# GDMCF/GDMCF

Measured on AMD Instinct MI355X. Metric: training users/sec, higher is better.
Workload: dtype f32; 1 GPU; yelp-shape synthetic rows, batch=400/GPU, dims=[1000], T=5, noise_scale=0.01, linear-var, mean_type=x0, reweight, AdamW lr=1e-5 (BASELINE configs[1]); n_items=34395, global_batch=400, parallelism=dp1, batch_rows=device CSR rows (CsrBatch)

## Files before the change

### gdmcf_amd/_lib.py

```python
import ctypes
import os
import re
from ctypes import c_char_p, c_double, c_float, c_int, c_int64, c_size_t, c_uint64, c_void_p

_HERE = os.path.dirname(os.path.abspath(__file__))
LIB_PATH = os.path.join(_HERE, "csrc", "libgdmcf_hip.so")
HEADER_PATH = os.path.normpath(os.path.join(_HERE, "..", "include", "gdmcf_hip.h"))

P = c_void_p
_CTYPES = {"int": c_int, "int64_t": c_int64, "uint64_t": c_uint64, "size_t": c_size_t, "float": c_float, "double": c_double}


def _uncomment(text):
    return re.sub(r"/\*.*?\*/", " ", text, flags=re.S)


def _code(text):
    return re.sub(r'^[ \t]*(#.*|extern\s+"C"\s*\{|\})[ \t]*$', "", _uncomment(text), flags=re.M)


def _ctype(ctype, where):
    words = re.sub(r"\bconst\b", " ", ctype).replace("*", " * ").split()
    if "*" in words:
        return c_char_p if words == ["char", "*"] else c_void_p
    if " ".join(words) not in _CTYPES:
        raise ImportError(f"gdmcf_hip.h: no ctypes type for '{' '.join(ctype.split())}' in the declaration of {where}")
    return _CTYPES[" ".join(words)]


def _declarator(decl, where):
    m = re.fullmatch(r"\s*(.*[\s*])(\w+)\s*", decl, flags=re.S)
    if not m:
        raise ImportError(f"gdmcf_hip.h: cannot read '{decl.strip()}' in the declaration of {where}")
    return m.groups()


def parse_functions(text):
    code = _code(text)
    out = {}
    for ret, name, params in re.findall(r"([\w\s*]+?)\b(gdmcf_\w+)\s*\(([^()]*)\)\s*;", code):
        params = [] if params.strip() in ("", "void") else params.split(",")
        out[name] = (_ctype(ret, name), [_ctype(_declarator(p, name)[0], name) for p in params])
    mentioned = re.findall(r"(gdmcf_\w+)\s*\(", code)
    if len(mentioned) != len(out):
        raise ImportError(f"gdmcf_hip.h: {len(mentioned)} gdmcf_*( but {len(out)} declarations read; unreadable: "
                          f"{sorted(set(mentioned) - set(out)) or 'none, a name is repeated'}")
    return out


def parse_constants(text):
    text = _uncomment(text)
    out = {n: int(v) for n, v in re.findall(r"^\s*#\s*define\s+(GDMCF_\w+)\s+\(?\s*(-?\d+)\s*\)?\s*$", text, flags=re.M)}
    for body in re.findall(r"\benum\s*\{([^}]*)\}", text):
        for member in filter(str.strip, body.split(",")):
            m = re.fullmatch(r"\s*(\w+)\s*=\s*(-?\d+)\s*", member)
            if not m:
                raise ImportError(f"gdmcf_hip.h: enum member '{member.strip()}' is not `NAME = integer`")
            out[m.group(1)] = int(m.group(2))
    return out


def parse_structs(text):
    out = {}
    for name, body in re.findall(r"\btypedef\s+struct\s+(\w+)\s*\{([^}]*)\}\s*\1\s*;", _code(text)):
        out[name] = []
        for line in filter(str.strip, body.split(";")):
            first, *more = line.split(",")
            ctype, member = _declarator(first, "struct " + name)
            if more and "*" in line:
                raise ImportError(f"gdmcf_hip.h: struct {name}: '{line.strip()}' must declare one pointer member per line")
            out[name] += [(m.strip(), _ctype(ctype, "struct " + name)) for m in [member] + more]
    return out


try:
    with open(HEADER_PATH) as _f:
        _HEADER = _f.read()
except OSError as e:
    raise ImportError(f"{HEADER_PATH} is missing: gdmcf_amd._lib derives its ctypes binding from the C header, which sits "
                      "beside the package in the source tree.") from e
_SIGNATURES = parse_functions(_HEADER)
EXPORTED_SYMBOLS = tuple(_SIGNATURES)
CONSTANTS = parse_constants(_HEADER)
GDMCF_OK, E_SHAPE, E_ARG, E_UNSUPPORTED, E_HIP, E_WORKSPACE, N_TABLES = (
    CONSTANTS["GDMCF_" + n] for n in ("OK", "E_SHAPE", "E_ARG", "E_UNSUPPORTED", "E_HIP", "E_WORKSPACE", "N_TABLES"))
TABLE_NAMES = (
    "betas", "alphas_cumprod", "alphas_cumprod_prev", "alphas_cumprod_next", "sqrt_alphas_cumprod",
    "sqrt_one_minus_alphas_cumprod", "log_one_minus_alphas_cumprod", "sqrt_recip_alphas_cumprod",
    "sqrt_recipm1_alphas_cumprod", "posterior_variance", "posterior_log_variance_clipped",
    "posterior_mean_coef1", "posterior_mean_coef2",
)


class GdDwAdamw(ctypes.Structure):
    _fields_ = parse_structs(_HEADER)["GdDwAdamw"]


_lib = None


def load():
    global _lib
    if _lib is not None:
        return _lib
    if not os.path.exists(LIB_PATH):
        raise ImportError(
            f"{LIB_PATH} is missing: build it with `python -m gdmcf_amd.build` (hipcc, gfx950). "
            "gdmcf_amd has no CPU / PyTorch fallback.")
    lib = ctypes.CDLL(LIB_PATH)
    for name, (res, args) in _SIGNATURES.items():
        fn = getattr(lib, name)
        fn.restype = res
        fn.argtypes = args
    if lib.gdmcf_version() != 1:
        raise ImportError("libgdmcf_hip.so ABI version mismatch; rebuild with `python -m gdmcf_amd.build --force`")
    _lib = lib
    return lib


_EXC = {E_SHAPE: AssertionError, E_ARG: ValueError, E_UNSUPPORTED: NotImplementedError, E_HIP: RuntimeError,
        E_WORKSPACE: RuntimeError}


def check(rc):
    if rc != GDMCF_OK:
        msg = load().gdmcf_last_error().decode(errors="replace")
        raise _EXC.get(rc, RuntimeError)(msg or f"gdmcf error {rc}")


def ptr(t):
    return None if t is None else t.data_ptr()


def require_gpu(t, what):
    if not t.is_cuda:
        raise RuntimeError(f"gdmcf_amd: {what} must live on the MI355X (got device '{t.device}'); "
                           "the HIP path has no CPU fallback")


def shadow_info(data_ptr):
    p16 = ctypes.c_void_p()
    rows, cols, ld = ctypes.c_int64(), ctypes.c_int64(), ctypes.c_int64()
    if not load().gdmcf_bf16_shadow_info(data_ptr, ctypes.byref(p16), ctypes.byref(rows), ctypes.byref(cols), ctypes.byref(ld)):
        return None
    return int(p16.value), int(rows.value), int(cols.value), int(ld.value)


def stream_ptr():
    import torch
    return torch.cuda.current_stream().cuda_stream


def philox_randn(shape, device, seed, offset, stream_id=4, out=None):
    import torch
    rows, cols = int(shape[0]), int(shape[1])
    if out is None:
        out = torch.empty(rows, cols, dtype=torch.float32, device=device)
    require_gpu(out, "philox_randn output")
    check(load().gdmcf_randn_f32(out.data_ptr(), out.stride(0), rows, cols, int(stream_id), int(seed) & (2 ** 64 - 1),
                                 int(offset) & (2 ** 64 - 1), stream_ptr()))
    return out


def schedule_tables(kind, noise_scale, noise_min, noise_max, steps, beta_fixed=True):
    import numpy as np
    out = np.zeros((N_TABLES, steps), dtype=np.float64)
    rc = load().gdmcf_schedule_build(kind, float(noise_scale), float(noise_min), float(noise_max), int(steps),
                                     int(bool(beta_fixed)), out.ctypes.data_as(c_void_p))
    check(rc)
    return out


class Bf16Shadow:

    def __init__(self, t, sync=True):
        import weakref

        import torch
        require_gpu(t, "bf16 shadow source")
        if t.dim() != 2 or t.dtype != torch.float32 or t.stride(1) != 1:
            raise RuntimeError("gdmcf_amd: a bf16 shadow needs a 2-D float32 tensor with unit column stride")
        self.rows, self.cols = t.shape
        self.ptr = t.data_ptr()
        self.ld = t.stride(0)
        self.buf = torch.zeros((self.rows + 63) // 64 * 64, (self.cols + 63) // 64 * 64, dtype=torch.bfloat16,
                               device=t.device)
        self._lib = load()
        self._fin = weakref.finalize(self, self._lib.gdmcf_bf16_shadow_clear, self.ptr)
        self.register()
        if sync:
            self.sync()

    def register(self):
        check(self._lib.gdmcf_bf16_shadow_set(self.ptr, self.buf.data_ptr(), self.rows, self.cols, self.buf.stride(0)))

    def unregister(self):
        self._lib.gdmcf_bf16_shadow_clear(self.ptr)

    def sync(self):
        check(self._lib.gdmcf_bf16_shadow_sync(self.ptr, self.ld, stream_ptr()))

    def close(self):
        self._fin()
```

### gdmcf_amd/build.py

```python
import concurrent.futures
import hashlib
import os
import re
import subprocess
import sys

CSRC = os.path.join(os.path.dirname(os.path.abspath(__file__)), "csrc")
SOURCES = ["capi.hip", "dp_exchange.hip", "gemm_f32.hip", "gemm_bf16.hip", "gemm_split.hip", "gemm_small.hip", "gemm_dr.hip", "gemm_dr_tn.hip", "gemm_dr_fat.hip", "gemm_dr_kn.hip", "prep_input.hip", "noise.hip", "loss_tail.hip", "adamw.hip", "rows.hip", "reduce.hip", "linear.hip", "topk.hip", "spmm_csr.hip", "rank_metrics.hip", "spmm_bundle.hip", "score_topk.hip", "score_rank.hip", "bpr.hip", "cat.hip", "gather_fwd.hip", "ntxent.hip", "latent_step.hip", "cand_scores.hip", "rank.hip"]
HEADERS = ["common.h", "draws.h", "rank_order.h", "score_product.h", "spmm.h", "gemm_dr.h", "gemm_epilogue.h", os.path.join("..", "..", "include", "gdmcf_hip.h")]
LIB = os.path.join(CSRC, "libgdmcf_hip.so")
ASM_LINT = ("gemm_dr_tn.hip", "gemm_split.hip")
STORE_LINT = ("gemm_f32.hip", "gemm_bf16.hip", "gemm_dr_fat.hip", "gemm_dr_kn.hip", "score_topk.hip", "score_rank.hip", "latent_step.hip", "bpr.hip")
NO_SPILL = ("gemm_f32.hip", "gemm_bf16.hip", "gemm_split.hip", "gemm_dr_tn.hip", "score_topk.hip", "score_rank.hip", "cat.hip", "gather_fwd.hip", "ntxent.hip", "latent_step.hip", "cand_scores.hip", "bpr.hip")
FLAGS = ["--offload-arch=gfx950", "-O3", "-std=c++17", "-fPIC", "-Wall", "-Wno-unused-function"]


def _hipcc():
    for c in (os.environ.get("HIPCC"), "/opt/rocm/bin/hipcc", "hipcc"):
        if c and (os.path.isabs(c) and os.path.exists(c) or not os.path.isabs(c)):
            return c
    raise RuntimeError("hipcc not found")


def _digest():
    h = hashlib.sha256()
    for f in SOURCES + HEADERS:
        with open(os.path.join(CSRC, f), "rb") as fh:
            h.update(fh.read())
    h.update(" ".join(FLAGS).encode())
    return h.hexdigest()


_REG = re.compile(r"\bv(\d+)\b|\bv\[(\d+):(\d+)\]")


def _regs(text):
    out = set()
    for m in _REG.finditer(text):
        if m.group(1) is not None:
            out.add(int(m.group(1)))
        else:
            out.update(range(int(m.group(2)), int(m.group(3)) + 1))
    return out


_SREG = re.compile(r"\bs(\d+)\b|\bs\[(\d+):(\d+)\]")


def _sregs(text):
    out = set()
    for m in _SREG.finditer(text):
        if m.group(1) is not None:
            out.add(int(m.group(1)))
        else:
            out.update(range(int(m.group(2)), int(m.group(3)) + 1))
    return out


def lint_ring_registers(asm_text, kernel_prefix="dr_tn_kernel"):
    bad, seen = [], 0
    for m in re.finditer(r"^(\S*%s\S*):[^\n]*\n(.*?)\n\s*s_endpgm" % kernel_prefix, asm_text, flags=re.S | re.M):
        name, body = m.group(1), m.group(2)
        seen += 1
        lines = [ln.split(";")[0].strip() for ln in body.splitlines()]
        lines = [ln for ln in lines if ln and not ln.endswith(":") and not ln.startswith(".")]
        ring = set()
        for ln in lines:
            if ln.startswith("buffer_load_dwordx4"):
                ring |= _regs(ln.split(",")[0])
        if not ring:
            bad.append(f"{name}: no asm ring loads found (lint out of date?)")
            continue
        first = next(i for i, ln in enumerate(lines) if ln.startswith("buffer_load_dwordx4"))
        drains = [i for i, ln in enumerate(lines) if ln.startswith("s_waitcnt") and "vmcnt(0)" in ln]
        last = drains[-1] if drains and drains[-1] > first else len(lines)
        for ln in lines[first:last]:
            mnem, _, ops = ln.partition(" ")
            parts = [o.strip() for o in ops.split(",")]
            if mnem.startswith("buffer_load_dwordx4"):
                if _regs(",".join(parts[1:])) & ring:
                    bad.append(f"{name}: ring register used as an address: {ln}")
            elif mnem.startswith("v_mfma"):
                if (_regs(parts[0]) | _regs(parts[3] if len(parts) > 3 else "")) & ring:
                    bad.append(f"{name}: MFMA accumulator inside the operand ring: {ln}")
            elif mnem.startswith(("v_mov", "v_pk_mov", "v_accvgpr", "scratch_", "v_swap")):
                if _regs(ops) & ring:
                    bad.append(f"{name}: copy or spill of a ring register: {ln}")
    if not seen:
        bad.append(f"no function named *{kernel_prefix}* in the assembly (lint out of date?)")
    return bad


_COPY = ("v_mov", "v_pk_mov", "v_accvgpr", "scratch_", "v_swap")
_VMEM = ("buffer_", "global_", "flat_", "scratch_")


def lint_vmcnt(asm_text, only=None):
    bad, nk = [], 0
    for m in re.finditer(r"^(_Z\S+):[^\n]*\n(.*?)\n\s*s_endpgm", asm_text, flags=re.S | re.M):
        name, body = m.group(1), m.group(2)
        if only and only not in name:
            continue
        ins, in_asm = [], False
        for ln in body.splitlines():
            t = ln.strip()
            if t.startswith(";;#ASMSTART"):
                in_asm = True
                continue
            if t.startswith(";;#ASMEND"):
                in_asm = False
                continue
            c = t.split(";")[0].strip()
            if not c or (c.startswith(".") and not c.endswith(":")):
                continue
            ins.append((c, in_asm))
        if not any(a and "load_dword" in c.split()[0] for c, a in ins):
            continue
        nk += 1
        leaders, labels = {0}, {}
        for k, (c, a) in enumerate(ins):
            if c.endswith(":"):
                labels[c[:-1]] = k
                leaders.add(k)
            elif c.startswith(("s_cbranch", "s_branch")):
                leaders.add(k + 1)
        starts = sorted(x for x in leaders if x < len(ins))
        blocks = [(st, starts[i + 1] if i + 1 < len(starts) else len(ins)) for i, st in enumerate(starts)]
        blk_of = {st: i for i, (st, en) in enumerate(blocks)}
        succ = []
        for bi, (st, en) in enumerate(blocks):
            mn, _, ops = ins[en - 1][0].partition(" ")
            nxt = []
            if mn.startswith(("s_cbranch", "s_branch")) and labels.get(ops.strip()) is not None:
                nxt.append(blk_of[labels[ops.strip()]])
            if not mn.startswith("s_branch") and bi + 1 < len(blocks):
                nxt.append(bi + 1)
            succ.append(nxt)
        found = {}

        def transfer(bi, st_in, report):
            st = dict(st_in)
            fresh = {}
            for k in range(*blocks[bi]):
                ln, a = ins[k]
                if ln.endswith(":"):
                    continue
                mnem, _, ops = ln.partition(" ")
                parts = [o.strip() for o in ops.split(",")]
                if a and mnem.startswith(_VMEM):
                    hot = _sregs(ops) & fresh.keys()
                    if hot and report:
                        found.setdefault(f"s{min(hot)} written by a VALU instruction < 5 wait states before this asm load reads it: {ln}", k)
                step = int(ops) + 1 if mnem == "s_nop" and ops.strip().isdigit() else 1
                fresh = {r: w - step for r, w in fresh.items() if w - step > 0}
                if mnem.startswith("v_") and parts and re.fullmatch(r"s\d+|s\[\d+:\d+\]", parts[0]):
                    for r in _sregs(parts[0]):
                        fresh[r] = 5
                if mnem == "s_waitcnt":
                    mm = re.search(r"vmcnt\((\d+)\)", ops)
                    if mm:
                        st = {r: rk for r, rk in st.items() if rk < int(mm.group(1))}
                    continue
                asm_load = a and "load_dword" in mnem
                touched = _regs(",".join(parts[1:]) if asm_load else ops) & st.keys()
                if touched and report:
                    what = "used as an address" if asm_load else ("copied / spilled" if mnem.startswith(_COPY) else "used")
                    found.setdefault(f"register v{min(touched)} {what} before a counted wait covers its load: {ln}", k)
                if mnem.startswith(_VMEM):
                    st = {r: min(rk + 1, 64) for r, rk in st.items()}
                    if asm_load:
                        for r in _regs(parts[0]):
                            st[r] = 0
            return st

        state = [None] * len(blocks)
        state[0] = {}
        work = [0]
        while work:
            bi = work.pop()
            out = transfer(bi, state[bi], False)
            for sj in succ[bi]:
                if state[sj] is None:
                    state[sj] = dict(out)
                    work.append(sj)
                else:
                    changed = False
                    for r, rk in out.items():
                        if state[sj].get(r, 65) > rk:
                            state[sj][r] = rk
                            changed = True
                    if changed:
                        work.append(sj)
        for bi in range(len(blocks)):
            if state[bi] is not None:
                transfer(bi, state[bi], True)
        bad += [f"{name}: {msg}" for msg, k in sorted(found.items(), key=lambda kv: kv[1])]
    if not nk:
        bad.append("no kernel with inline-asm loads in the assembly (lint out of date?)")
    return bad


def lint_store_data(asm_text):
    bad = []
    for m in re.finditer(r"^(_Z\S+):[^\n]*\n(.*?)\n\s*s_endpgm", asm_text, flags=re.S | re.M):
        name, body = m.group(1), m.group(2)
        lines = [ln.split(";")[0].strip() for ln in body.splitlines()]
        lines = [ln for ln in lines if ln and not ln.startswith(".") and not ln.endswith(":")]
        for k, ln in enumerate(lines):
            mnem, _, ops = ln.partition(" ")
            if not re.match(r"(buffer|global|flat|scratch)_store_dwordx[34]$", mnem):
                continue
            parts = [o.strip() for o in ops.split(",")]
            data = _regs(parts[1] if mnem.startswith(("global", "flat", "scratch")) else parts[0])
            left = 2
            for nxt in lines[k + 1:k + 8]:
                nm, _, nops = nxt.partition(" ")
                if nm == "s_nop":
                    left -= int(nops.strip() or 0) + 1
                else:
                    nparts = [o.strip() for o in nops.split(",")]
                    if nm.startswith("v_") and nparts and _regs(nparts[0]) & data and left > 0:
                        bad.append(f"{name}: data register of `{ln}` rewritten {2 - left} wait state(s) later by `{nxt}`")
                        break
                    left -= 1
                if left <= 0:
                    break
    return bad


def lint_fat_dma(asm_text, kernel="dr_fat_kernel"):
    bad, n_dma = [], 0
    for m in re.finditer(r"^(_Z\S*%s\S*):[^\n]*\n(.*?)\n\s*s_endpgm" % kernel, asm_text, flags=re.S | re.M):
        name, body = m.group(1), m.group(2)
        lines = [ln.split(";")[0].strip() for ln in body.splitlines()]
        lines = [ln for ln in lines if ln and (not ln.startswith(".") or ln.endswith(":"))]
        if not any(ln.startswith("buffer_load_dwordx4") and ln.endswith(" lds") for ln in lines):
            continue
        n_dma += 1
        pending = None
        for ln in lines:
            if ln.startswith("buffer_load_dwordx4") and ln.endswith(" lds"):
                pending = ln
            elif ln.startswith("s_waitcnt") and re.search(r"vmcnt\(0\)", ln):
                pending = None
            elif ln.startswith("ds_read_b128") and pending:
                bad.append(f"{name}: `{ln}` follows `{pending}` with no s_waitcnt vmcnt(0) in between")
                break
        loops, label, blk = 0, None, []
        for ln in lines + ["end:"]:
            if not ln.endswith(":"):
                blk.append(ln)
                continue
            if label and any(i.startswith("v_mfma") for i in blk) and any(
                    i.startswith(("s_cbranch", "s_branch")) and i.split()[-1] == label for i in blk):
                loops += 1
                moved = [i for i in blk if i.startswith(("scratch_", "v_accvgpr", "v_mov"))]
                if moved:
                    bad.append(f"{name}: {len(moved)} spill / move instruction(s) in the k loop, e.g. `{moved[0]}`")
            label, blk = ln[:-1], []
        if not loops:
            bad.append(f"{name}: no k loop found (lint out of date?)")
    if not n_dma:
        bad.append(f"no *{kernel}* with `buffer_load_dwordx4 ... lds` in the assembly (lint out of date?)")
    return bad


def build(force=False, verbose=True):
    stamp = os.path.join(CSRC, ".build_stamp")
    dig = _digest()
    if not force and os.path.exists(LIB) and os.path.exists(stamp) and open(stamp).read() == dig:
        return LIB
    hipcc = _hipcc()
    objs = []

    def compile_one(src):
        obj = os.path.join(CSRC, src.replace(".hip", ".o"))
        cmd = [hipcc] + FLAGS + ["-c", os.path.join(CSRC, src), "-o", obj]
        guarded = src in NO_SPILL
        if guarded:
            cmd.append("-Rpass-analysis=kernel-resource-usage")
        r = subprocess.run(cmd, capture_output=True, text=True)
        if r.returncode != 0:
            raise RuntimeError(f"hipcc failed for {src}:\n{r.stderr}")
        err = r.stderr
        if guarded:
            name, bad = None, []
            for line in err.splitlines():
                if "Function Name:" in line:
                    name = line.split("Function Name:")[1].split()[0]
                elif "VGPRs Spill:" in line and int(line.split("VGPRs Spill:")[1].split()[0]) > 0:
                    bad.append(name)
            if bad:
                raise RuntimeError(f"{src}: register spills in {len(bad)} kernel(s) with uncounted asm loads, e.g. {bad[0]}")
            err = err if ("warning:" in err or "error:" in err) else ""
        if verbose and err.strip():
            print(err, file=sys.stderr)
        if src in ASM_LINT or src in STORE_LINT:
            asm = os.path.join(CSRC, src.replace(".hip", ".lint.s"))
            r2 = subprocess.run([hipcc] + FLAGS + ["-S", "--cuda-device-only", os.path.join(CSRC, src), "-o", asm],
                                capture_output=True, text=True)
            if r2.returncode != 0:
                raise RuntimeError(f"hipcc -S failed for {src}:\n{r2.stderr}")
            text = open(asm).read()
            os.remove(asm)
            bad = lint_store_data(text)
            if src in ASM_LINT:
                bad += lint_vmcnt(text)
            if src == "gemm_dr_tn.hip":
                bad += lint_ring_registers(text)
            if src == "gemm_dr_fat.hip":
                bad += lint_fat_dma(text)
            if bad:
                raise RuntimeError(f"{src}: ISA lint failed (lint_store_data / lint_vmcnt / lint_ring_registers / lint_fat_dma):\n  " + "\n  ".join(bad[:12]))
        return obj

    with concurrent.futures.ThreadPoolExecutor(max_workers=min(8, len(SOURCES))) as ex:
        objs = list(ex.map(compile_one, SOURCES))
    cmd = [hipcc, "--offload-arch=gfx950", "-shared", "-fPIC", "-o", LIB] + objs
    r = subprocess.run(cmd, capture_output=True, text=True)
    if r.returncode != 0:
        raise RuntimeError(f"link failed:\n{r.stderr}")
    with open(stamp, "w") as fh:
        fh.write(dig)
    if verbose:
        print(f"built {LIB}")
    return LIB


if __name__ == "__main__":
    build(force="--force" in sys.argv)
```

### gdmcf_amd/csrc/gemm_dr_kn.hip

```cpp
#include "gemm_dr.h"

namespace {

#ifndef GD_KN_EVERY
#define GD_KN_EVERY 4
#endif
template <int NL>
__global__ __launch_bounds__(256, 1) void dr_kn_kernel(const DrArgs d) {
    constexpr int TMB = 5;
    const GdGemm& g = d.g;
    const int lane = threadIdx.x & 63;
    const int wave = __builtin_amdgcn_readfirstlane(threadIdx.x >> 6);
    const int r = lane & 15, q = lane >> 4;
    const int nblk = gridDim.x, per = nblk >> 3;
    const int wl = ((nblk & 7) == 0 ? ((int)(blockIdx.x & 7) * per + (int)(blockIdx.x >> 3)) : (int)blockIdx.x) * 4 + wave;
    const int n_waves = nblk * 4;
    const int ntiles = d.tiles_m * d.tiles_n;
    const int CPS = d.ksp;
    const int total_chunks = (g.K + 15) >> 4;
    const int ntasks = ntiles * g.splits;
    const __amdgpu_buffer_rsrc_t srdA = __builtin_amdgcn_make_buffer_rsrc(const_cast<float*>(g.A), 0, (int)(((int64_t)(g.M - 1) * g.lda + g.K) * 4), 0x00020000);
    const __amdgpu_buffer_rsrc_t srdB = __builtin_amdgcn_make_buffer_rsrc(const_cast<float*>(g.B), 0, (int)(((int64_t)(g.K - 1) * g.ldb + g.N) * 4), 0x00020000);
    const uint32_t ldb16 = (uint32_t)g.ldb * 64u;
    for (int task = wl; task < ntasks; task += n_waves) {
        const int split = task / ntiles, tile = task - split * ntiles;
        const int tm = tile % d.tiles_m, tn = tile / d.tiles_m;
        const int m0 = tm * (16 * TMB), n0 = tn * (64 * NL);
        const int c_lo = split * CPS;
        uint32_t offA[TMB], offB[4][NL];
#pragma unroll
        for (int a = 0; a < TMB; ++a) offA[a] = (uint32_t)(((int64_t)min(m0 + 16 * a + r, g.M - 1) * g.lda + 4 * q) * 4);
#pragma unroll
        for (int s = 0; s < 4; ++s)
#pragma unroll
            for (int l = 0; l < NL; ++l) {
                const int n = n0 + 64 * l + 4 * r;
                offB[s][l] = n < g.N ? (uint32_t)(((int64_t)(4 * q + s) * g.ldb + n) * 4) : 0x80000000u;
            }
        f32x4 acc[TMB][NL][4];
#pragma unroll
        for (int a = 0; a < TMB; ++a)
#pragma unroll
            for (int l = 0; l < NL; ++l)
#pragma unroll
                for (int e = 0; e < 4; ++e) acc[a][l][e] = f32x4{0.f, 0.f, 0.f, 0.f};
        f32x4 xa[2][TMB], xb[2][4][NL];
        {
            const uint32_t ka = (uint32_t)c_lo * 64u, kb = (uint32_t)c_lo * ldb16;
#pragma unroll
            for (int a = 0; a < TMB; ++a) xa[0][a] = __builtin_bit_cast(f32x4, __builtin_amdgcn_raw_buffer_load_b128(srdA, offA[a], ka, 0));
#pragma unroll
            for (int s = 0; s < 4; ++s)
#pragma unroll
                for (int l = 0; l < NL; ++l)
                    xb[0][s][l] = __builtin_bit_cast(f32x4, __builtin_amdgcn_raw_buffer_load_b128(srdB, offB[s][l], kb, 0));
        }
#define GD_KN_CHUNK(PAR, c)                                                                                            \
        {                                                                                                              \
            const bool more = (c) + 1 < c_lo + CPS && (c) + 1 < total_chunks;                                          \
            const uint32_t ka = more ? (uint32_t)((c) + 1) * 64u : 0x80000000u;                                        \
            const uint32_t kb = more ? (uint32_t)((c) + 1) * ldb16 : 0x80000000u;                                      \
            if ((c) * 16 + 15 >= g.K) {  \
                _Pragma("unroll") for (int e = 0; e < 4; ++e) {                                                        \
                    const bool keep = (c) * 16 + 4 * q + e < g.K;                                                      \
                    _Pragma("unroll") for (int a = 0; a < TMB; ++a) xa[PAR][a][e] = keep ? xa[PAR][a][e] : 0.f;        \
                }                                                                                                      \
            }                                                                                                          \
                    \
            _Pragma("unroll") for (int a = 0; a < TMB; ++a) asm volatile("" : "+v"(xa[PAR][a]));                       \
            _Pragma("unroll") for (int s = 0; s < 4; ++s)                                                              \
                _Pragma("unroll") for (int l = 0; l < NL; ++l) asm volatile("" : "+v"(xb[PAR][s][l]));                 \
            __builtin_amdgcn_sched_barrier(0);                                                                         \
            _Pragma("unroll") for (int s = 0; s < 4; ++s) {                                                            \
                _Pragma("unroll") for (int n = 0; n < TMB * NL * 4; ++n) {                                             \
                    const int a = n / (NL * 4), l = (n / 4) % NL, e = n % 4;                                           \
                    acc[a][l][e] = __builtin_amdgcn_mfma_f32_16x16x4f32(xa[PAR][a][s], xb[PAR][s][l][e], acc[a][l][e], 0, 0, 0); \
                    const int idx = s * (TMB * NL * 4) + n;                                                            \
                    if (idx % GD_KN_EVERY == 2 && idx / GD_KN_EVERY < TMB + 4 * NL) {                                  \
                        const int ld = idx / GD_KN_EVERY;                                                              \
                        __builtin_amdgcn_sched_barrier(0);                                                             \
                        if (ld < TMB)                                                                                  \
                            xa[(PAR) ^ 1][ld] = __builtin_bit_cast(f32x4, __builtin_amdgcn_raw_buffer_load_b128(srdA, offA[ld], ka, 0)); \
                        else                                                                                           \
                            xb[(PAR) ^ 1][(ld - TMB) / NL][(ld - TMB) % NL] = __builtin_bit_cast(                      \
                                f32x4, __builtin_amdgcn_raw_buffer_load_b128(srdB, offB[(ld - TMB) / NL][(ld - TMB) % NL], kb, 0)); \
                        __builtin_amdgcn_sched_barrier(0);                                                             \
                    }                                                                                                  \
                }                                                                                                      \
                __builtin_amdgcn_sched_barrier(0);                                                                     \
            }                                                                                                          \
        }
        for (int c = c_lo; c < c_lo + CPS && c < total_chunks; c += 2) {
            GD_KN_CHUNK(0, c);
            GD_KN_CHUNK(1, c + 1);
        }
#undef GD_KN_CHUNK
        float* __restrict__ slab = g.C + (int64_t)split * g.slab_stride;
#pragma unroll
        for (int a = 0; a < TMB; ++a)
#pragma unroll
            for (int t = 0; t < 4; ++t) {
                const int m = m0 + 16 * a + 4 * q + t;
                if (m >= g.M) continue;
#pragma unroll
                for (int l = 0; l < NL; ++l) {
                    const int n = n0 + 64 * l + 4 * r;
                    const f32x4 v = {acc[a][l][0][t], acc[a][l][1][t], acc[a][l][2][t], acc[a][l][3][t]};
                    if (n + 3 < g.ldc) {
                        *reinterpret_cast<f32x4*>(slab + (int64_t)m * g.ldc + n) = v;
                    } else {
                        for (int e = 0; e < 4; ++e)
                            if (n + e < g.N) slab[(int64_t)m * g.ldc + n + e] = v[e];
                    }
                }
            }
    }
}

}

int gd_dr_kn_splits(int M, int N, int K) {
    if (!dr_routes().kn || M < 16 || N < 64 || K < 4096) return 0;
    const long tiles = (long)gd_cdiv(M, 80) * gd_cdiv(N, 128);
    if ((long)gd_cdiv(M, 80) * 80 * 100 > (long)M * 112) return 0;
    if ((long)gd_cdiv(N, 128) * 128 * 100 > (long)N * 112) return 0;
    const long slots = 4L * dr_cu_count();
    if (tiles > slots) return 0;
    int splits = (int)(slots / tiles);
    const int total_chunks = gd_cdiv(K, 16);
    if (splits > total_chunks / 8) splits = total_chunks / 8;
    if (splits < 2 || splits > 64) return splits > 64 ? 64 : 0;
    return splits;
}

int gd_dr_kn_launch(GdGemm& g, hipStream_t s) {
    if (!dr_routes().kn) return GD_DR_NOT_TAKEN;
    const int splits = gd_dr_kn_splits(g.M, g.N, g.K);
    const size_t need = (size_t)splits * g.M * g.ldc * sizeof(float);
    const bool ok = splits > 0 && g.ldc >= g.N && (g.ldc & 3) == 0 && g.ws_cap >= need && g.slab_stride >= (int64_t)g.M * g.ldc &&
                (int64_t)g.M * g.lda * 4 < ((int64_t)1 << 31) && (int64_t)g.K * g.ldb * 4 < ((int64_t)1 << 31) && g.lda >= g.K && g.ldb >= g.N &&
                (reinterpret_cast<uintptr_t>(g.B) & 15) == 0 && (g.ldb & 3) == 0 && (reinterpret_cast<uintptr_t>(g.C) & 15) == 0;
    if (!ok) return GD_DR_NOT_TAKEN;
    DrArgs d = {};
    const int n_cu = dr_cu_count();
    const int total_chunks = gd_cdiv(g.K, 16);
    const int cps = (gd_cdiv(total_chunks, splits) + 1) & ~1;
    d.tiles_m = gd_cdiv(g.M, 80);
    d.tiles_n = gd_cdiv(g.N, 128);
    d.ksp = cps;
    g.splits = gd_cdiv(total_chunks, cps);
    g.kchunk = cps * 16;
    g.tiles_m = d.tiles_m;
    g.tiles_n = d.tiles_n;
    d.g = g;
    {
        GdProfScope prof(g.prof_tag, 2.0 * g.M * g.N * g.K, s);
        hipLaunchKernelGGL((dr_kn_kernel<2>), dim3(n_cu), dim3(256), 0, s, d);
    }
    t_gd_last_gemm = 5;
    return gd_launch_status("gemm_dr_kn");
}
```

### gdmcf_amd/csrc/linear.hip

```cpp
#include <stdlib.h>

#include "common.h"

int gd_splitk_reduce(const float* slabs, int64_t slab_stride, int splits, int64_t ld_slab, int M, int N, int mode,
                     const float* bias, const float* rowscale, const float* aact, int64_t ldact, int act, float* out,
                     int64_t ldo, hipStream_t s);
int gd_colsum(const float* dZ, int64_t ld, const float* rs, int M, int N, float* db, hipStream_t s);
int gd_rowpart_reduce(const float* rowpart, int ld, int M, int nt, float* rowsum, hipStream_t s);

namespace {

static const int TARGET_WGS = getenv("GDMCF_TARGET_WGS") ? atoi(getenv("GDMCF_TARGET_WGS")) : 760;

thread_local int t_gemm_prec = GDMCF_GEMM_F32;

int pick_class(int M, int N, bool fused, int prec) {
    if (prec == GDMCF_GEMM_BF16 && M > 128) {
        const long pad = (long)gd_cdiv(M, 208) * 208;
        const long tiles = (pad / 208) * gd_cdiv(N, 256);
        const long rounds = (tiles + 255) / 256;
        if (pad * 10 <= (long)M * 11 && pad / 208 <= 2 && (!fused || tiles * 100 >= rounds * 256 * 85)) return 3;
    }
    if (prec == GDMCF_GEMM_F32X3 && M > 128 && N >= 128) {
        const long pad = (long)gd_cdiv(M, 208) * 208;
        if (pad * 10 <= (long)M * 11) return 4;
    }
    return gd_pick_shape_class(M, N);
}

int pick_class_dw(int M, int N, int prec, bool fused_adamw = false) {
    static const int forced = getenv("GDMCF_BF16_DW_CLASS") ? atoi(getenv("GDMCF_BF16_DW_CLASS")) : -1;
    if (prec == GDMCF_GEMM_BF16 && forced >= 0) return forced;
    if (prec == GDMCF_GEMM_BF16 && fused_adamw && M >= 160 && N >= 256) return 0;
    if (prec == GDMCF_GEMM_BF16 && M >= 416 && N >= 512) {
        const long tiles = (long)gd_cdiv(M, 208) * gd_cdiv(N, 256);
        const long rounds = (tiles + 255) / 256;
        if (tiles * 100 >= rounds * 256 * 85) return 3;
    }
    return gd_pick_shape_class(M, N);
}

void attach_result_shadow(GdGemm& g) {
    GdShadow c;
    if (g.bf16 == 1 && gd_shadow_lookup(g.C, &c) && c.rows == g.M && c.cols >= g.N) {
        g.C16 = c.p16;
        g.ldc16 = c.ld16;
    }
}

void attach_shadows(GdGemm& g, int layA, int layB) {
    if (g.bf16 != 1) return;
    GdShadow a, b;
    if (!gd_shadow_lookup(g.A, &a) || !gd_shadow_lookup(g.B, &b)) return;
    const bool okA = layA == GD_LAY_KC ? (a.rows == g.M && a.cols == g.K) : (a.rows == g.K && a.cols == g.M);
    const bool okB = layB == GD_LAY_KC ? (b.rows == g.N && b.cols == g.K) : (b.rows == g.K && b.cols == g.N);
    if (!okA || !okB) return;
    g.A16 = a.p16; g.lda16 = a.ld16;
    g.B16 = b.p16; g.ldb16 = b.ld16;
}

int pick_splits(int M, int N, int K, int cls, int prec) {
    const int bk = prec == GDMCF_GEMM_BF16 ? 64 : 32;
    const int tiles = gd_cdiv(M, gd_gemm_tile_m(cls)) * gd_cdiv(N, gd_gemm_tile_n(cls));
    int s = (cls >= 3 ? 256 : TARGET_WGS) / tiles;
    const int max_by_k = K / (8 * bk);
    if (s > max_by_k) s = max_by_k;
    if (s < 1) s = 1;
    if (s > 64) s = 64;
    return s;
}

inline int64_t round4(int64_t x) { return (x + 3) & ~(int64_t)3; }

float* bias_col_request(int a_scale_col, int64_t lda, const float* rowscale, int K, float* db) {
    static const int on = getenv("GDMCF_BIAS_COL") ? atoi(getenv("GDMCF_BIAS_COL")) : 1;
    if (!on || !a_scale_col || db == nullptr || t_gemm_prec != GDMCF_GEMM_F32 || lda <= K) return nullptr;
    return db;
}

int dw_adamw_setup(const GdDwAdamw& e, GdGemm& g, int& cls) {
    GD_CHECK_SHAPE(e.M > 0 && e.N > 0 && e.K > 0 && e.lddz >= e.N && e.lda >= e.K && e.ldw >= e.K, "linear_bwd_weight_adamw: bad shape");
    GD_CHECK_ARG(e.W && e.exp_avg && e.exp_avg_sq && e.step >= 1, "linear_bwd_weight_adamw: optimizer state missing");
    const int M = e.M, N = e.N, K = e.K;
    cls = pick_class_dw(N, K, t_gemm_prec, true);
    g = GdGemm{};
    g.bf16 = t_gemm_prec;
    g.A = e.dZ; g.lda = e.lddz; g.B = e.A; g.ldb = e.lda; g.M = N; g.N = K; g.K = M; g.splits = 1;
    g.m_fastest = gd_cdiv(N, gd_gemm_tile_m(cls)) <= gd_cdiv(K, gd_gemm_tile_n(cls));
    g.C = e.W; g.ldc = e.ldw; g.aux = e.exp_avg; g.aux2 = e.exp_avg_sq; g.prof_tag = 5;
    g.adam = gd_adam_hyper(e.lr, e.beta1, e.beta2, e.eps, e.weight_decay, e.step, e.grad_scale);
    g.adam_dev = t_gd_step_state ? &t_gd_step_state->hyper : nullptr;
    attach_result_shadow(g);
    attach_shadows(g, GD_LAY_MC, GD_LAY_MC);
    g.out2 = bias_col_request(e.a_scale_col, e.lda, e.rowscale, K, e.db);
    return GDMCF_OK;
}

int dw_adamw_finish(const GdDwAdamw& e, bool asked, const GdGemm& g, hipStream_t s) {
    if (asked && g.out2 == nullptr) return GDMCF_OK;
    if (e.db) return gd_colsum(e.dZ, e.lddz, e.rowscale, e.M, e.N, e.db, s);
    return GDMCF_OK;
}

}

extern "C" {

int gdmcf_gemm_precision(int mode) {
    const int prev = t_gemm_prec;
    if (mode == GDMCF_GEMM_F32 || mode == GDMCF_GEMM_BF16 || mode == GDMCF_GEMM_F32X3) t_gemm_prec = mode;
    return prev;
}

size_t gdmcf_linear_ws_bytes(int M, int N, int K) {
    if (M <= 0 || N <= 0 || K <= 0) return 0;
    size_t need = 0;
    for (int prec = GDMCF_GEMM_F32; prec <= GDMCF_GEMM_F32X3; ++prec) {
        const int cf = pick_class(M, N, false, prec), cb = pick_class(M, K, false, prec);
        size_t f = (size_t)pick_splits(M, N, K, cf, prec) * M * round4(N);
        if (prec == GDMCF_GEMM_F32) {
            const size_t fk = (size_t)gd_dr_kn_splits(M, N, K) * M * round4(N);
            f = f > fk ? f : fk;
            const size_t ff = (size_t)gd_dr_fat_slab_plan(M, N, K, nullptr, nullptr) * M * round4(N);
            f = f > ff ? f : ff;
        }
        size_t b = (size_t)pick_splits(M, K, N, cb, prec) * M * round4(K);
        if (prec == GDMCF_GEMM_F32) {
            const size_t bk = (size_t)gd_dr_kn_splits(M, K, N) * M * round4(K);
            b = b > bk ? b : bk;
        }
        need = need > f ? need : f;
        need = need > b ? need : b;
    }
    return need * sizeof(float) + 256;
}

int gdmcf_debug_fat_slab_plan(int M, int N, int K, int* nb, int* splits, int* cps) {
    int nb_ = 0, cps_ = 0;
    const int sp = (t_gemm_prec == GDMCF_GEMM_F32 && M > 0 && N > 0 && K > 0) ? gd_dr_fat_slab_plan(M, N, K, &nb_, &cps_) : 0;
    if (nb) *nb = nb_;
    if (splits) *splits = sp;
    if (cps) *cps = cps_;
    return sp > 0;
}

int gdmcf_loss_tiles(int N) { return gd_cdiv(N, 16); }

int gdmcf_linear_fwd_f32(const float* A, int64_t lda, const float* W, int64_t ldw, const float* bias, int act, int M,
                         int N, int K, float* C, int64_t ldc, void* ws, size_t ws_bytes, void* stream) {
    GD_CHECK_SHAPE(M > 0 && N > 0 && K > 0 && lda >= K && ldw >= K && ldc >= N, "linear_fwd: bad shape");
    GD_CHECK_ARG(act == 0 || act == 1, "linear_fwd: bad activation");
    hipStream_t s = (hipStream_t)stream;
    const int cls = pick_class(M, N, false, t_gemm_prec);
    const int splits = pick_splits(M, N, K, cls, t_gemm_prec);
    GdGemm g = {};
    g.bf16 = t_gemm_prec;
    g.A = A; g.lda = lda; g.B = W; g.ldb = ldw; g.M = M; g.N = N; g.K = K;
    g.m_fastest = gd_cdiv(M, gd_gemm_tile_m(cls)) <= gd_cdiv(N, gd_gemm_tile_n(cls));
    g.bias = bias; g.act = act; g.prof_tag = 1;
    if (splits == 1) {
        g.splits = 1; g.C = C; g.ldc = ldc;
        attach_result_shadow(g);
        attach_shadows(g, GD_LAY_KC, GD_LAY_KC);
        return gd_gemm_launch(GD_LAY_KC, GD_LAY_KC, GD_EPI_BIAS_ACT, cls, g, s);
    }
    const int64_t lds_ = round4(N);
    const size_t need = (size_t)splits * M * lds_ * sizeof(float);
    if (ws == nullptr || ws_bytes < need) {
        gdmcf_set_error("linear_fwd: workspace %zu < %zu bytes", ws_bytes, need);
        return GDMCF_E_WORKSPACE;
    }
    g.splits = splits; g.C = (float*)ws; g.ldc = lds_; g.slab_stride = (int64_t)M * lds_;
    g.ws_cap = ws_bytes;
    attach_shadows(g, GD_LAY_KC, GD_LAY_KC);
    int rc = gd_gemm_launch(GD_LAY_KC, GD_LAY_KC, GD_EPI_SLAB, cls, g, s);
    if (rc) return rc;
    const int real_splits = gd_cdiv(K, g.kchunk);
    return gd_splitk_reduce((const float*)ws, g.slab_stride, real_splits, lds_, M, N, 0, bias, nullptr, nullptr, 0,
                            act, C, ldc, s);
}

int gdmcf_linear_fwd_wt_f32(const float* A, int64_t lda, const float* Wt, int64_t ldwt, const float* bias, int act, int M, int N,
                            int K, float* C, int64_t ldc, void* ws, size_t ws_bytes, void* stream) {
    GD_CHECK_SHAPE(M > 0 && N > 0 && K > 0 && lda >= K && ldwt >= N && ldc >= N, "linear_fwd_wt: bad shape");
    GD_CHECK_ARG(act == 0 || act == 1, "linear_fwd_wt: bad activation");
    if (t_gemm_prec != GDMCF_GEMM_F32) {
        gdmcf_set_error("linear_fwd_wt: float32 GEMM mode only (the bf16 / f32x3 modes keep the weight in its own orientation)");
        return GDMCF_E_UNSUPPORTED;
    }
    hipStream_t s = (hipStream_t)stream;
    const int cls = pick_class(M, N, false, t_gemm_prec);
    const int splits = pick_splits(M, N, K, cls, t_gemm_prec);
    const int64_t lds_ = round4(N);
    const size_t need = (size_t)splits * M * lds_ * sizeof(float);
    if (ws == nullptr || ws_bytes < need) {
        gdmcf_set_error("linear_fwd_wt: workspace %zu < %zu bytes", ws_bytes, need);
        return GDMCF_E_WORKSPACE;
    }
    GdGemm g = {};
    g.A = A; g.lda = lda; g.B = Wt; g.ldb = ldwt; g.M = M; g.N = N; g.K = K;
    g.m_fastest = gd_cdiv(M, gd_gemm_tile_m(cls)) <= gd_cdiv(N, gd_gemm_tile_n(cls));
    g.splits = splits; g.C = (float*)ws; g.ldc = lds_; g.slab_stride = (int64_t)M * lds_; g.prof_tag = 1;
    g.ws_cap = ws_bytes;
    int rc = gd_gemm_launch(GD_LAY_KC, GD_LAY_MC, GD_EPI_SLAB, cls, g, s);
    if (rc) return rc;
    const int real_splits = gd_cdiv(K, g.kchunk);
    return gd_splitk_reduce((const float*)ws, g.slab_stride, real_splits, lds_, M, N, 0, bias, nullptr, nullptr, 0, act, C, ldc, s);
}

int gdmcf_linear_loss_fwd_f32(const float* A, int64_t lda, const float* W, int64_t ldw, const float* bias,
                              const float* target, int64_t ldt, const float* alpha, int M, int N, int K, float* out,
                              int64_t ldo, float* diff, int64_t ldd, float* rowpart, float* rowsum, void* stream) {
    GD_CHECK_SHAPE(M > 0 && N > 0 && K > 0 && lda >= K && ldw >= K && ldt >= N && ldd >= N, "linear_loss_fwd: bad shape");
    GD_CHECK_SHAPE(out == nullptr || ldo >= N, "linear_loss_fwd: ldo < N");
    hipStream_t s = (hipStream_t)stream;
    const int cls = pick_class(M, N, true, t_gemm_prec);
    GdGemm g = {};
    g.bf16 = t_gemm_prec;
    g.A = A; g.lda = lda; g.B = W; g.ldb = ldw; g.M = M; g.N = N; g.K = K; g.splits = 1;
    g.m_fastest = gd_cdiv(M, gd_gemm_tile_m(cls)) <= gd_cdiv(N, gd_gemm_tile_n(cls));
    g.bias = bias; g.aux = target; g.ldaux = ldt; g.r0 = alpha; g.out2 = out; g.ldout2 = ldo;
    g.prof_tag = 2;
    g.C = diff; g.ldc = ldd; g.rowpart = rowpart; g.ld_rowpart = gdmcf_loss_tiles(N);
    attach_result_shadow(g);
    attach_shadows(g, GD_LAY_KC, GD_LAY_KC);
    int rc = gd_gemm_launch(GD_LAY_KC, GD_LAY_KC, GD_EPI_LOSS, cls, g, s);
    if (rc) return rc;
    return gd_rowpart_reduce(rowpart, g.ld_rowpart, M, g.tiles_n, rowsum, s);
}

int gdmcf_linear_loss_fwd_bits_f32(const float* A, int64_t lda, const float* W, int64_t ldw, const float* bias,
                                   const uint32_t* target_bits, int64_t ldbits, const float* alpha, int M, int N, int K,
                                   float* out, int64_t ldo, float* diff, int64_t ldd, float* rowpart, float* rowsum,
                                   void* stream) {
    GD_CHECK_SHAPE(M > 0 && N > 0 && K > 0 && lda >= K && ldw >= K && ldd >= N, "linear_loss_fwd_bits: bad shape");
    GD_CHECK_SHAPE(out == nullptr || ldo >= N, "linear_loss_fwd_bits: ldo < N");
    GD_CHECK_ARG(target_bits && ldbits >= (N + 31) / 32, "linear_loss_fwd_bits: target bitmap missing / ldbits < ceil(N/32)");
    hipStream_t s = (hipStream_t)stream;
    const int cls = pick_class(M, N, true, t_gemm_prec);
    GdGemm g = {};
    g.bf16 = t_gemm_prec;
    g.A = A; g.lda = lda; g.B = W; g.ldb = ldw; g.M = M; g.N = N; g.K = K; g.splits = 1;
    g.m_fastest = gd_cdiv(M, gd_gemm_tile_m(cls)) <= gd_cdiv(N, gd_gemm_tile_n(cls));
    g.bias = bias; g.aux = nullptr; g.ldaux = 0; g.aux_bits = target_bits; g.ldbits = ldbits; g.r0 = alpha; g.out2 = out;
    g.ldout2 = ldo; g.prof_tag = 2;
    g.C = diff; g.ldc = ldd; g.rowpart = rowpart; g.ld_rowpart = gdmcf_loss_tiles(N);
    attach_result_shadow(g);
    attach_shadows(g, GD_LAY_KC, GD_LAY_KC);
    int rc = gd_gemm_launch(GD_LAY_KC, GD_LAY_KC, GD_EPI_LOSS, cls, g, s);
    if (rc) return rc;
    return gd_rowpart_reduce(rowpart, g.ld_rowpart, M, g.tiles_n, rowsum, s);
}

int gdmcf_linear_posterior_fwd_f32(const float* A, int64_t lda, const float* W, int64_t ldw, const float* bias,
                                   const float* x_t, int64_t ldxt, const float* c1, const float* c2, const float* r1,
                                   const float* r2, const float* sigma, const float* z, int64_t ldz, int M, int N,
                                   int K, float* x_next, int64_t ldxn, float* pred_out, int64_t ldp, void* stream) {
    GD_CHECK_SHAPE(M > 0 && N > 0 && K > 0 && lda >= K && ldw >= K && ldxt >= N && ldxn >= N, "linear_posterior_fwd: bad shape");
    GD_CHECK_ARG(c1 && c2, "linear_posterior_fwd: c1/c2 missing");
    GD_CHECK_ARG((r1 == nullptr) == (r2 == nullptr), "linear_posterior_fwd: r1/r2 must both be set or both NULL");
    GD_CHECK_ARG(z == nullptr || (sigma != nullptr && ldz >= N), "linear_posterior_fwd: sigma missing");
    hipStream_t s = (hipStream_t)stream;
    const int cls = pick_class(M, N, true, t_gemm_prec);
    GdGemm g = {};
    g.bf16 = t_gemm_prec;
    g.A = A; g.lda = lda; g.B = W; g.ldb = ldw; g.M = M; g.N = N; g.K = K; g.splits = 1;
    g.m_fastest = gd_cdiv(M, gd_gemm_tile_m(cls)) <= gd_cdiv(N, gd_gemm_tile_n(cls));
    g.bias = bias; g.aux = x_t; g.ldaux = ldxt; g.aux2 = z; g.ldaux2 = ldz;
    g.r0 = c1; g.r1 = c2; g.r2 = r1; g.r3 = r2; g.r4 = sigma;
    g.out2 = pred_out; g.ldout2 = ldp; g.C = x_next; g.ldc = ldxn; g.prof_tag = 3;
    attach_result_shadow(g);
    attach_shadows(g, GD_LAY_KC, GD_LAY_KC);
    return gd_gemm_launch(GD_LAY_KC, GD_LAY_KC, GD_EPI_POST, cls, g, s);
}

int gdmcf_linear_bwd_input_f32(const float* dZ, int64_t lddz, const float* W, int64_t ldw, const float* rowscale,
                               const float* Aact, int64_t ldact, int act, int M, int N, int K, float* dA,
                               int64_t ldda, void* ws, size_t ws_bytes, void* stream) {
    GD_CHECK_SHAPE(M > 0 && N > 0 && K > 0 && lddz >= N && ldw >= K && ldda >= K, "linear_bwd_input: bad shape");
    GD_CHECK_ARG(act == 0 || (act == 1 && Aact && ldact >= K), "linear_bwd_input: activation output missing");
    hipStream_t s = (hipStream_t)stream;
    const int cls = pick_class(M, K, false, t_gemm_prec);
    const int splits = pick_splits(M, K, N, cls, t_gemm_prec);
    const int64_t lds_ = round4(K);
    const size_t need = (size_t)splits * M * lds_ * sizeof(float);
    if (ws == nullptr || ws_bytes < need) {
        gdmcf_set_error("linear_bwd_input: workspace %zu < %zu bytes", ws_bytes, need);
        return GDMCF_E_WORKSPACE;
    }
    GdGemm g = {};
    g.bf16 = t_gemm_prec;
    g.A = dZ; g.lda = lddz; g.B = W; g.ldb = ldw; g.M = M; g.N = K; g.K = N;
    g.m_fastest = gd_cdiv(M, gd_gemm_tile_m(cls)) <= gd_cdiv(K, gd_gemm_tile_n(cls));
    g.splits = splits; g.C = (float*)ws; g.ldc = lds_; g.slab_stride = (int64_t)M * lds_; g.prof_tag = 4;
    g.ws_cap = ws_bytes;
    attach_shadows(g, GD_LAY_KC, GD_LAY_MC);
    int rc = gd_gemm_launch(GD_LAY_KC, GD_LAY_MC, GD_EPI_SLAB, cls, g, s);
    if (rc) return rc;
    const int real_splits = gd_cdiv(N, g.kchunk);
    return gd_splitk_reduce((const float*)ws, g.slab_stride, real_splits, lds_, M, K, 1, nullptr, rowscale, Aact,
                            ldact, act, dA, ldda, s);
}

int gdmcf_linear_bwd_weight_f32(const float* dZ, int64_t lddz, const float* A, int64_t lda, const float* rowscale,
                                int a_scale_col, int M, int N, int K, float* dW, int64_t lddw, float* db, int accumulate,
                                void* stream) {
    GD_CHECK_SHAPE(M > 0 && N > 0 && K > 0 && lddz >= N && lda >= K && lddw >= K, "linear_bwd_weight: bad shape");
    hipStream_t s = (hipStream_t)stream;
    const int cls = pick_class_dw(N, K, t_gemm_prec);
    GdGemm g = {};
    g.bf16 = t_gemm_prec;
    g.A = dZ; g.lda = lddz; g.B = A; g.ldb = lda; g.M = N; g.N = K; g.K = M; g.splits = 1;
    g.m_fastest = gd_cdiv(N, gd_gemm_tile_m(cls)) <= gd_cdiv(K, gd_gemm_tile_n(cls));
    g.C = dW; g.ldc = lddw; g.accumulate = accumulate; g.prof_tag = 5;
    attach_shadows(g, GD_LAY_MC, GD_LAY_MC);
    g.out2 = bias_col_request(a_scale_col, lda, rowscale, K, db);
    const bool asked = g.out2 != nullptr;
    int rc = gd_gemm_launch(GD_LAY_MC, GD_LAY_MC, GD_EPI_STORE, cls, g, s);
    if (rc) return rc;
    if (asked && g.out2 == nullptr) return GDMCF_OK;
    if (db) return gd_colsum(dZ, lddz, rowscale, M, N, db, s);
    return GDMCF_OK;
}

int gdmcf_linear_bwd_weight_adamw_f32(const float* dZ, int64_t lddz, const float* A, int64_t lda, const float* rowscale,
                                      int a_scale_col, int M, int N, int K, float* W, int64_t ldw, float* exp_avg, float* exp_avg_sq,
                                      float* db, float lr, float beta1, float beta2, float eps, float weight_decay,
                                      int step, float grad_scale, void* stream) {
    const GdDwAdamw e = {dZ, lddz, A, lda, rowscale, a_scale_col, M, N, K, W, ldw, exp_avg, exp_avg_sq, db,
                         lr, beta1, beta2, eps, weight_decay, step, grad_scale};
    GdGemm g;
    int cls;
    int rc = dw_adamw_setup(e, g, cls);
    if (rc) return rc;
    const bool asked = g.out2 != nullptr;
    rc = gd_gemm_launch(GD_LAY_MC, GD_LAY_MC, GD_EPI_ADAMW, cls, g, (hipStream_t)stream);
    if (rc) return rc;
    return dw_adamw_finish(e, asked, g, (hipStream_t)stream);
}

int gdmcf_linear_bwd_weight_adamw_multi_f32(const GdDwAdamw* list, int n, void* stream) {
    GD_CHECK_ARG(n >= 0 && (n == 0 || list), "linear_bwd_weight_adamw_multi: bad list");
    hipStream_t s = (hipStream_t)stream;
    constexpr int MAXN = 4;
    for (int i0 = 0; i0 < n; i0 += MAXN) {
        const int k = n - i0 < MAXN ? n - i0 : MAXN;
        GdGemm g[MAXN];
        bool asked[MAXN];
        int cls;
        for (int j = 0; j < k; ++j) {
            const int rc = dw_adamw_setup(list[i0 + j], g[j], cls);
            if (rc) return rc;
            asked[j] = g[j].out2 != nullptr;
        }
        int rc = gd_gemm_dr_adamw_multi(g, k, s);
        if (rc == GD_DR_NOT_TAKEN) {
            for (int j = 0; j < k; ++j) {
                const GdDwAdamw& e = list[i0 + j];
                rc = gdmcf_linear_bwd_weight_adamw_f32(e.dZ, e.lddz, e.A, e.lda, e.rowscale, e.a_scale_col, e.M, e.N, e.K, e.W,
                                                       e.ldw, e.exp_avg, e.exp_avg_sq, e.db, e.lr, e.beta1, e.beta2, e.eps,
                                                       e.weight_decay, e.step, e.grad_scale, stream);
                if (rc) return rc;
            }
            continue;
        }
        if (rc) return rc;
        for (int j = 0; j < k; ++j) {
            rc = dw_adamw_finish(list[i0 + j], asked[j], g[j], s);
            if (rc) return rc;
        }
    }
    return GDMCF_OK;
}

}
```

### gdmcf_amd/csrc/loss_tail.hip

```cpp
#include "draws.h"

namespace {

__device__ void lt_history_parallel(const int64_t* __restrict__ ts, const double* __restrict__ lu, int B, int T, int H,
                                    double* hist, int64_t* cnt, unsigned char* lds_raw) {
    double* old = reinterpret_cast<double*>(lds_raw);
    int* n_t = reinterpret_cast<int*>(old + (size_t)T * H);
    int* c0 = n_t + T;
    int* tsl = c0 + T;
    const int tid = threadIdx.x, nth = blockDim.x;
    for (int i = tid; i < T * H; i += nth) old[i] = hist[i];
    for (int t = tid; t < T; t += nth) {
        n_t[t] = 0;
        c0[t] = (int)cnt[t];
    }
    for (int b = tid; b < B; b += nth) tsl[b] = (int)ts[b];
    __syncthreads();
    for (int b = tid; b < B; b += nth) atomicAdd(&n_t[tsl[b]], 1);
    __syncthreads();
    for (int i = tid; i < T * H; i += nth) {
        const int t = i / H, j = i % H;
        const int drop = max(0, c0[t] + n_t[t] - H);
        if (j < c0[t] && j - drop >= 0) hist[(int64_t)t * H + (j - drop)] = old[i];
    }
    for (int b = tid; b < B; b += nth) {
        const int t = tsl[b];
        int rank = 0;
        for (int p = 0; p < b; ++p) rank += (tsl[p] == t);
        const int drop = max(0, c0[t] + n_t[t] - H);
        const int pos = c0[t] + rank - drop;
        if (pos >= 0) hist[(int64_t)t * H + pos] = lu[b];
    }
    for (int t = tid; t < T; t += nth) cnt[t] = (int64_t)min(H, c0[t] + n_t[t]);
}

__global__ __launch_bounds__(256) void row_loss_finish_kernel(const float* __restrict__ rowsum,
                                                              const float* __restrict__ rowdiv,
                                                              const float* __restrict__ alpha,
                                                              float* __restrict__ gradcoef,
                                                              const int64_t* __restrict__ ts,
                                                              const double* __restrict__ weight_t,
                                                              const double* __restrict__ pt, int B, int T, int H,
                                                              double* hist, int64_t* cnt, int update,
                                                              double* __restrict__ lu, double* __restrict__ loss,
                                                              double* __restrict__ loss_mean, float* __restrict__ rowscale_mean,
                                                              float inv_b) {
    extern __shared__ __attribute__((aligned(16))) unsigned char fin_lds[];
    double part = 0.0;
    for (int b = threadIdx.x; b < B; b += 256) {
        const float mse = rowsum[b] / rowdiv[b];
        const double l = weight_t[ts[b]] * (double)mse;
        lu[b] = l;
        const double lb = l / pt[b];
        loss[b] = lb;
        part += lb;
        if (gradcoef) {
            const float gc = (float)(2.0 * (alpha ? (double)alpha[b] : 1.0) * weight_t[ts[b]] / (pt[b] * (double)rowdiv[b]));
            gradcoef[b] = gc;
            if (rowscale_mean) rowscale_mean[b] = gc * inv_b;
        }
    }
    if (loss_mean) {
        double* s_part = reinterpret_cast<double*>(fin_lds);
        for (int o = 32; o > 0; o >>= 1) part += __shfl_xor(part, o);
        if ((threadIdx.x & 63) == 0) s_part[threadIdx.x >> 6] = part;
        __syncthreads();
        if (threadIdx.x == 0) *loss_mean = (((s_part[0] + s_part[1]) + s_part[2]) + s_part[3]) / (double)B;
    }
    __syncthreads();
    if (update) lt_history_parallel(ts, lu, B, T, H, hist, cnt, fin_lds);
}

__global__ __launch_bounds__(256) void lt_history_update_kernel(const int64_t* ts, const double* lu, int B, int T,
                                                                int H, double* hist, int64_t* cnt) {
    extern __shared__ __attribute__((aligned(16))) unsigned char fin_lds[];
    lt_history_parallel(ts, lu, B, T, H, hist, cnt, fin_lds);
}

__global__ __launch_bounds__(256) void sample_timesteps_kernel(const double* __restrict__ hist,
                                                               const int64_t* __restrict__ cnt, int T, int H, int B,
                                                               double uniform_prob, uint64_t seed, uint64_t offset,
                                                               int64_t* __restrict__ ts, double* __restrict__ pt,
                                                               double* __restrict__ p_out, const GdStepState* step_state) {
    if (step_state) offset = step_state->ts_offset;
    extern __shared__ __attribute__((aligned(16))) unsigned char st_lds[];
    double* p = reinterpret_cast<double*>(st_lds);
    double* cdf = p + T;
    __shared__ int full;
    __shared__ double total;
    const int tid = threadIdx.x;
    if (tid == 0) full = 1;
    __syncthreads();
    for (int t = tid; t < T; t += 256)
        if (cnt[t] != H) full = 0;
    __syncthreads();
    const bool imp = (full != 0);
    if (imp) {
        for (int t = tid; t < T; t += 256) {
            double s = 0.0;
            for (int j = 0; j < H; ++j) {
                const double v = hist[(int64_t)t * H + j];
                s += v * v;
            }
            p[t] = sqrt(s / (double)H);
        }
        __syncthreads();
        if (tid == 0) {
            double s = 0.0;
            for (int t = 0; t < T; ++t) s += p[t];
            total = s;
        }
        __syncthreads();
        for (int t = tid; t < T; t += 256) {
            double v = p[t] / total;
            v *= 1.0 - uniform_prob;
            v += uniform_prob / (double)T;
            p[t] = v;
            if (p_out) p_out[t] = v;
        }
        __syncthreads();
        if (tid == 0) {
            double s = 0.0;
            for (int t = 0; t < T; ++t) {
                s += p[t];
                cdf[t] = s;
            }
        }
        __syncthreads();
    }
    for (int b = tid; b < B; b += 256) {
        const uint4 r = gd_philox_block((uint32_t)b, 0, GD_STREAM_TIMESTEPS, offset, gd_philox_key(seed));
        const double u = ((double)r.x * 4294967296.0 + (double)r.y) * (1.0 / 18446744073709551616.0);
        int t;
        if (imp) {
            const double x = u * cdf[T - 1];
            int lo = 0, hi = T - 1;
            while (lo < hi) {
                const int mid = (lo + hi) >> 1;
                if (cdf[mid] > x) hi = mid; else lo = mid + 1;
            }
            t = lo;
            pt[b] = p[t] * (double)T;
        } else {
            t = min((int)(u * (double)T), T - 1);
            pt[b] = 1.0;
        }
        ts[b] = t;
    }
}

size_t lt_lds_bytes(int T, int H, int B) { return (size_t)T * H * 8 + (size_t)T * 8 + (size_t)B * 4 + 16; }

template <class K>
bool gd_allow_big_lds(K* kernel, size_t lds, bool* done, const char* who) {
    if (*done || lds <= 48 * 1024) return true;
    *done = hipFuncSetAttribute(reinterpret_cast<const void*>(kernel), hipFuncAttributeMaxDynamicSharedMemorySize, 160 * 1024) == hipSuccess;
    if (!*done) gdmcf_set_error("%s: hipFuncSetAttribute failed", who);
    return *done;
}

}

extern "C" {

int gdmcf_row_loss_finish_f64(const float* rowsum, const float* rowdiv, const float* alpha, const int64_t* ts,
                              const double* weight_t, const double* pt, int B, int T, int H, double* Lt_history,
                              int64_t* Lt_count, int update_history, double* loss_unscaled, double* loss,
                              float* gradcoef, void* stream) {
    return gdmcf_row_loss_finish_mean_f64(rowsum, rowdiv, alpha, ts, weight_t, pt, B, T, H, Lt_history, Lt_count, update_history,
                                          loss_unscaled, loss, gradcoef, nullptr, nullptr, stream);
}

int gdmcf_row_loss_finish_mean_f64(const float* rowsum, const float* rowdiv, const float* alpha, const int64_t* ts,
                                   const double* weight_t, const double* pt, int B, int T, int H, double* Lt_history,
                                   int64_t* Lt_count, int update_history, double* loss_unscaled, double* loss,
                                   float* gradcoef, double* loss_mean, float* rowscale_mean, void* stream) {
    GD_CHECK_SHAPE(B > 0 && T > 0 && H > 0, "row_loss_finish: bad shape");
    GD_CHECK_ARG(rowsum && rowdiv && ts && weight_t && pt && loss_unscaled && loss, "row_loss_finish: null pointer");
    GD_CHECK_ARG(!update_history || (Lt_history && Lt_count), "row_loss_finish: update_history without the history");
    GD_CHECK_ARG(!rowscale_mean || gradcoef, "row_loss_finish: rowscale_mean needs gradcoef");
    const size_t lds = lt_lds_bytes(T, H, B);
    GD_CHECK_ARG(lds <= 150 * 1024, "row_loss_finish: T*H and B too large for the LDS-resident FIFO update (150 KiB)");
    static bool attr_set = false;
    if (!gd_allow_big_lds(row_loss_finish_kernel, lds, &attr_set, "row_loss_finish")) return GDMCF_E_HIP;
    hipLaunchKernelGGL(row_loss_finish_kernel, dim3(1), dim3(256), lds, (hipStream_t)stream, rowsum, rowdiv, alpha,
                       gradcoef, ts, weight_t, pt, B, T, H, Lt_history, Lt_count, update_history, loss_unscaled, loss,
                       loss_mean, rowscale_mean, 1.0f / (float)B);
    return gd_launch_status("row_loss_finish");
}

int gdmcf_lt_history_update(const int64_t* ts, const double* loss_unscaled, int B, int T, int H, double* Lt_history,
                            int64_t* Lt_count, void* stream) {
    GD_CHECK_SHAPE(B > 0 && T > 0 && H > 0, "lt_history_update: bad shape");
    GD_CHECK_ARG(ts && loss_unscaled && Lt_history && Lt_count, "lt_history_update: null pointer");
    const size_t lds = lt_lds_bytes(T, H, B);
    GD_CHECK_ARG(lds <= 150 * 1024, "lt_history_update: T*H and B too large for the LDS-resident FIFO update (150 KiB)");
    static bool attr_set = false;
    if (!gd_allow_big_lds(lt_history_update_kernel, lds, &attr_set, "lt_history_update")) return GDMCF_E_HIP;
    hipLaunchKernelGGL(lt_history_update_kernel, dim3(1), dim3(256), lds, (hipStream_t)stream, ts, loss_unscaled, B, T,
                       H, Lt_history, Lt_count);
    return gd_launch_status("lt_history_update");
}

int gdmcf_sample_timesteps(const double* Lt_history, const int64_t* Lt_count, int T, int H, int B,
                           double uniform_prob, uint64_t seed, uint64_t offset, int64_t* ts, double* pt, double* p_out,
                           void* stream) {
    GD_CHECK_SHAPE(B > 0 && T > 0 && H > 0, "sample_timesteps: bad shape");
    GD_CHECK_OFFSET(offset, "sample_timesteps");
    GD_CHECK_ARG(T <= 4096, "sample_timesteps: T > 4096 unsupported");
    hipLaunchKernelGGL(sample_timesteps_kernel, dim3(1), dim3(256), (size_t)T * 16, (hipStream_t)stream, Lt_history,
                       Lt_count, T, H, B, uniform_prob, seed, offset, ts, pt, p_out, t_gd_step_state);
    return gd_launch_status("sample_timesteps");
}

}
```

### gdmcf_amd/csrc/reduce.hip

```cpp
#include "common.h"

namespace {

__global__ __launch_bounds__(256) void splitk_reduce_kernel(const float* __restrict__ slabs, int64_t slab_stride,
                                                            int splits, int64_t ld_slab, int M, int N, int mode,
                                                            const float* __restrict__ bias,
                                                            const float* __restrict__ rowscale,
                                                            const float* __restrict__ aact, int64_t ldact, int act,
                                                            float* __restrict__ out, int64_t ldo,
                                                            unsigned short* __restrict__ out16, int64_t ldo16, int vec) {
    const int m = blockIdx.y;
    const int n0 = (blockIdx.x * 256 + threadIdx.x) * 4;
    if (n0 >= N) return;
    float sv[4] = {0.f, 0.f, 0.f, 0.f};
    const float* p = slabs + (int64_t)m * ld_slab + n0;
    if (vec && n0 + 3 < N) {
        for (int k0 = 0; k0 < splits; k0 += 8) {
            f32x4 t[8];
#pragma unroll
            for (int u = 0; u < 8; ++u)
                t[u] = (k0 + u < splits) ? *reinterpret_cast<const f32x4*>(p + (int64_t)(k0 + u) * slab_stride)
                                         : f32x4{0.f, 0.f, 0.f, 0.f};
#pragma unroll
            for (int u = 0; u < 8; ++u)
                if (k0 + u < splits) { sv[0] += t[u].x; sv[1] += t[u].y; sv[2] += t[u].z; sv[3] += t[u].w; }
        }
    } else {
        for (int k = 0; k < splits; ++k)
            for (int j = 0; j < 4; ++j)
                if (n0 + j < N) sv[j] += p[(int64_t)k * slab_stride + j];
    }
    const float rs = (mode != 0 && rowscale) ? rowscale[m] : 1.f;
#pragma unroll
    for (int j = 0; j < 4; ++j) {
        const int n = n0 + j;
        if (n >= N) break;
        float s = sv[j];
        if (mode == 0) {
            if (bias) s += bias[n];
            if (act == 1) s = tanhf(s);
        } else {
            if (rowscale) s *= rs;
            if (act == 1) {
                const float h = aact[(int64_t)m * ldact + n];
                s *= (1.f - h * h);
            }
        }
        out[(int64_t)m * ldo + n] = s;
        if (out16) out16[(int64_t)m * ldo16 + n] = gd_bf16_bits(s);
    }
}

__global__ __launch_bounds__(256) void rowscale_kernel(const float* __restrict__ A, int64_t lda,
                                                       const float* __restrict__ rs, int M, int K,
                                                       float* __restrict__ out, int64_t ldo,
                                                       unsigned short* __restrict__ out16, int64_t ldo16, int bias_col) {
    const int m = blockIdx.y, k = (blockIdx.x * 256 + threadIdx.x) * 4;
    if (bias_col && blockIdx.x == 0 && threadIdx.x == 0) out[(int64_t)m * ldo + K] = rs[m];
    if (k >= K) return;
    const float r = rs[m];
    const float* a = A + (int64_t)m * lda + k;
    float* o = out + (int64_t)m * ldo + k;
    float v[4];
    if (k + 3 < K) {
        const f32x4 t = *reinterpret_cast<const f32x4_u4*>(a);
        v[0] = t.x * r; v[1] = t.y * r; v[2] = t.z * r; v[3] = t.w * r;
        *reinterpret_cast<f32x4_u4*>(o) = f32x4{v[0], v[1], v[2], v[3]};
    } else {
        for (int j = 0; j < 4; ++j)
            if (k + j < K) o[j] = v[j] = a[j] * r;
    }
    if (out16)
        for (int j = 0; j < 4; ++j)
            if (k + j < K) out16[(int64_t)m * ldo16 + k + j] = gd_bf16_bits(v[j]);
}

__global__ __launch_bounds__(256) void colsum_kernel(const float* __restrict__ dZ, int64_t ld,
                                                     const float* __restrict__ rs, int M, int N,
                                                     float* __restrict__ db) {
    __shared__ float part[4][64];
    const int lane = threadIdx.x & 63, wave = threadIdx.x >> 6;
    const int n = blockIdx.x * 64 + lane;
    const int nc = min(n, N - 1);
    float s = 0.f;
    int m = wave;
    for (; m + 28 < M; m += 32) {
        float v[8];
#pragma unroll
        for (int j = 0; j < 8; ++j) v[j] = dZ[(int64_t)(m + 4 * j) * ld + nc] * (rs ? rs[m + 4 * j] : 1.f);
#pragma unroll
        for (int j = 0; j < 8; ++j) s += v[j];
    }
    for (; m < M; m += 4) s += dZ[(int64_t)m * ld + nc] * (rs ? rs[m] : 1.f);
    part[wave][lane] = s;
    __syncthreads();
    if (wave == 0 && n < N) db[n] = ((part[0][lane] + part[1][lane]) + part[2][lane]) + part[3][lane];
}

__global__ __launch_bounds__(256) void rowpart_reduce_kernel(const float* __restrict__ rowpart, int ld, int M, int nt,
                                                             float* __restrict__ rowsum) {
    const int m = blockIdx.x * 4 + (threadIdx.x >> 6), lane = threadIdx.x & 63;
    if (m >= M) return;
    float s = 0.f;
    for (int j = lane; j < nt; j += 64) s += rowpart[(int64_t)m * ld + j];
    for (int o = 32; o > 0; o >>= 1) s += __shfl_xor(s, o);
    if (lane == 0) rowsum[m] = s;
}

typedef __bf16 gd_bf16x2 __attribute__((ext_vector_type(2)));
__device__ __forceinline__ unsigned gd_pack_bf16(float lo, float hi) {
    gd_bf16x2 v;
    v[0] = (__bf16)lo;
    v[1] = (__bf16)hi;
    return __builtin_bit_cast(unsigned, v);
}
typedef unsigned int gd_u32x4 __attribute__((ext_vector_type(4)));

__global__ __launch_bounds__(256) void cast_bf16_kernel(const float* __restrict__ src, int64_t ld, unsigned short* __restrict__ dst,
                                                        int64_t ld16, int64_t rows, int64_t cols) {
    const int64_t groups = (cols + 7) / 8;
    const int64_t total = rows * groups;
    for (int64_t u = (int64_t)blockIdx.x * blockDim.x + threadIdx.x; u < total; u += (int64_t)gridDim.x * blockDim.x) {
        const int64_t r = u / groups, c = (u - r * groups) * 8;
        const float* p = src + r * ld + c;
        float e[8];
#pragma unroll
        for (int i = 0; i < 8; ++i) e[i] = (c + i < cols) ? p[i] : 0.f;
        gd_u32x4 w;
        w.x = gd_pack_bf16(e[0], e[1]);
        w.y = gd_pack_bf16(e[2], e[3]);
        w.z = gd_pack_bf16(e[4], e[5]);
        w.w = gd_pack_bf16(e[6], e[7]);
        *reinterpret_cast<gd_u32x4*>(dst + r * ld16 + c) = w;
    }
}
}

extern "C" {

int gdmcf_rowscale_f32(const float* A, int64_t lda, const float* rowscale, int M, int K, float* out, int64_t ldo,
                       void* stream) {
    GD_CHECK_SHAPE(M > 0 && K > 0 && lda >= K && ldo >= K, "rowscale: bad shape");
    GdShadow sh;
    const bool has16 = gd_shadow_lookup(out, &sh) && sh.rows == M && sh.cols == K;
    const int bias_col = ldo > K;
    hipLaunchKernelGGL(rowscale_kernel, dim3(gd_cdiv(K, 1024), M), dim3(256), 0, (hipStream_t)stream, A, lda,
                       rowscale, M, K, out, ldo, has16 ? (unsigned short*)sh.p16 : nullptr, has16 ? sh.ld16 : 0, bias_col);
    return gd_launch_status("rowscale");
}

}

int gd_splitk_reduce(const float* slabs, int64_t slab_stride, int splits, int64_t ld_slab, int M, int N, int mode,
                     const float* bias, const float* rowscale, const float* aact, int64_t ldact, int act, float* out,
                     int64_t ldo, hipStream_t s) {
    GdShadow sh;
    const bool has16 = gd_shadow_lookup(out, &sh) && sh.rows == M && sh.cols == N;
    const int vec = (ld_slab % 4 == 0) && (slab_stride % 4 == 0) && gd_aligned16(slabs);
    hipLaunchKernelGGL(splitk_reduce_kernel, dim3(gd_cdiv(N, 1024), M), dim3(256), 0, s, slabs, slab_stride,
                       splits, ld_slab, M, N, mode, bias, rowscale, aact, ldact, act, out, ldo,
                       has16 ? (unsigned short*)sh.p16 : nullptr, has16 ? sh.ld16 : 0, vec);
    return gd_launch_status("splitk_reduce");
}

int gd_colsum(const float* dZ, int64_t ld, const float* rs, int M, int N, float* db, hipStream_t s) {
    hipLaunchKernelGGL(colsum_kernel, dim3(gd_cdiv(N, 64)), dim3(256), 0, s, dZ, ld, rs, M, N, db);
    return gd_launch_status("colsum");
}

int gd_rowpart_reduce(const float* rowpart, int ld, int M, int nt, float* rowsum, hipStream_t s) {
    hipLaunchKernelGGL(rowpart_reduce_kernel, dim3(gd_cdiv(M, 4)), dim3(256), 0, s, rowpart, ld, M, nt, rowsum);
    return gd_launch_status("rowpart_reduce");
}

int gd_cast_bf16(const float* src, int64_t ld, void* dst, int64_t ld16, int64_t rows, int64_t cols, hipStream_t s) {
    const int64_t total = rows * ((cols + 7) / 8);
    const int64_t blocks = (total + 255) / 256;
    hipLaunchKernelGGL(cast_bf16_kernel, dim3((unsigned)(blocks < 16384 ? blocks : 16384)), dim3(256), 0, s, src, ld,
                       (unsigned short*)dst, ld16, rows, cols);
    return gd_launch_status("cast_bf16");
}
```

### gdmcf_amd/engine.py

```python

import ctypes
import os

import torch

from . import _lib
from . import engine_core as core
from .engine_core import EngineBase, _Bufs, _ceil64, with_precision


class DenoiserEngine(EngineBase):
    def __init__(self, model):
        super().__init__(model)
        self._wshadow = {}
        self.input_grad_first = False
        self.weight_waiters = {}
        self.static_grads = False
        self._grad_bufs = {}
        self._gemm_side = os.environ.get("GDMCF_GEMM_SIDE", "0") == "1"
        self._side2 = None
        self._side2_used = False
        self._wt_on = os.environ.get("GDMCF_FWD_WT", "1") == "1"

    def _grad_like(self, p):
        if not self.static_grads:
            return torch.empty_like(p)
        g = self._grad_bufs.get(id(p))
        if g is None or g.shape != p.shape or g.device != p.device:
            g = self._grad_bufs[id(p)] = torch.empty_like(p)
        return g

    def _use_weight(self, w):
        fn = self.weight_waiters.pop(id(w), None) if self.weight_waiters else None
        if fn is not None:
            fn()
            rec = self._wshadow.get(id(w))
            if rec is not None and rec[1] != w._version:
                rec[0].sync()
                rec[1] = w._version

    def flush_weight_waiters(self):
        while self.weight_waiters:
            self.weight_waiters.popitem()[1]()

    def _shadows_on(self, bufs, layers):
        if self.gemm_dtype != "bf16":
            if bufs.shadows is not None:
                for sh in bufs.shadows:
                    sh.close()
                bufs.shadows = None
                bufs.sh_xin2 = None
            for sh, _ in self._wshadow.values():
                sh.close()
            self._wshadow = {}
            return
        if bufs.shadows is None:
            I, E = self.I, self.E
            mk = lambda t, cols: _lib.Bf16Shadow(t[:, :cols], sync=False)
            sh = [mk(bufs.xin, I + E), mk(bufs.diff, I)]
            for (w, _, _), a, d in zip(layers[:-1], bufs.acts, bufs.dzs):
                sh += [mk(a, w.shape[0]), mk(d, w.shape[0])]
            sh.append(mk(bufs.hs, layers[-1][0].shape[1]))
            bufs.shadows = sh
            bufs.sh_xin = sh[0]
        live = {id(w) for w, _, _ in layers}
        for key in [k for k in self._wshadow if k not in live]:
            self._wshadow.pop(key)[0].close()
        for w, _, _ in layers:
            rec = self._wshadow.get(id(w))
            if rec is None or rec[0].ptr != w.data_ptr():
                self._use_weight(w)
                if rec is not None:
                    rec[0].close()
                self._wshadow[id(w)] = [_lib.Bf16Shadow(w.detach()), w._version]
            elif id(w) in self.weight_waiters:
                continue
            elif rec[1] != w._version:
                rec[0].sync()
                rec[1] = w._version

    def _layers(self):
        layers = self.model.layer_list()
        self._check_params(layers)
        return layers

    def buffers(self, B, device):
        key = (B, str(device))
        b = self._bufs.get(key)
        if b is not None:
            return b
        layers = self.model.layer_list()
        f32 = dict(dtype=torch.float32, device=device)
        b = _Bufs()
        b.ldk = _ceil64(self.I + self.E)
        b.xin = torch.zeros(B, b.ldk, **f32)
        b.xin2 = None
        b.acts = [torch.zeros(B, _ceil64(w.shape[0]), **f32) for (w, _, _) in layers[:-1]]
        b.dzs = [torch.zeros(B, _ceil64(w.shape[0]), **f32) for (w, _, _) in layers[:-1]]
        b.hs = torch.zeros(B, _ceil64(layers[-1][0].shape[1]), **f32)
        b.shadows = None
        self._shared_buffers(b, B, device, layers[-1][0].shape[0], layers[0][0].shape[0], [w for w, _, _ in layers])
        self._bufs[key] = b
        return b

    def _prep(self, bufs, x, ts, ca, cb, noise, drop_mask, training, xt_out=None, xin=None):
        xin = bufs.xin if xin is None else xin
        keepalive = self._prep_input(bufs, x, self.I, xin, ts, ca, cb, noise, drop_mask, training, xt_out=xt_out)
        if xin is bufs.xin:
            bufs.xin_ones = True
        return keepalive

    def _train_input(self, bufs, spec, xt_out):
        return self._prep(bufs, spec["x_start"], spec["ts"], spec["ca"], spec["cb"], spec["noise"], spec["drop_mask"],
                          self.model.training, xt_out=xt_out)

    def _prep_csr(self, bufs, batch, ts, ca, cb, noise, drop_mask, training):
        m = self.model
        B, I = batch.shape
        if getattr(bufs, "x0bits", None) is None:
            bufs.x0bits = torch.zeros(B, (I + 31) // 32, dtype=torch.int32, device=batch.device)
        self.offset += 1
        keepalive = core.prep_input_csr(self.lib, batch, ts, ca, cb, noise, drop_mask, float(m.drop.p), training, self.seed,
                                        self.offset, m.emb_layer, self.E, bufs.xin, bufs.temb, bufs.x0bits, _lib.stream_ptr())
        bufs.xin_ones = True
        return keepalive

    def _train_input_csr(self, bufs, spec):
        return self._prep_csr(bufs, spec["csr"], spec["ts"], spec["ca"], spec["cb"], spec["noise"], spec["drop_mask"],
                              self.model.training)

    def _hidden_forward(self, bufs, layers, B, xin=None, frozen=False, csr=None):
        lib, st = self.lib, _lib.stream_ptr()
        A = bufs.xin if xin is None else xin
        for li, (w, bias, act) in enumerate(layers[:-1]):
            N, K = w.shape
            out = bufs.acts[li]
            self._use_weight(w)
            if li == 0 and csr is not None:
                self._gather_first_layer(bufs, csr, w, bias, act, A, B, out, st)
            elif frozen and self._wt_on and self.gemm_dtype == "f32" and K >= 4096 and w.numel() >= (1 << 20):
                wt = self._transposed(w)
                _lib.check(lib.gdmcf_linear_fwd_wt_f32(A.data_ptr(), A.stride(0), wt.data_ptr(), wt.stride(0), bias.data_ptr(), act, B, N, K,
                                                       out.data_ptr(), out.stride(0), bufs.ws.data_ptr(), bufs.ws_bytes, st))
            else:
                core.linear_fwd(lib, bufs, A, w, bias, act, B, N, K, out, st)
            A = out
        return A

    @with_precision
    def train_forward(self, spec):
        x0, ts = spec["x_start"], spec["ts"]
        csr = spec.get("csr")
        B, dev = (csr.shape[0], csr.device) if csr is not None else (x0.shape[0], x0.device)
        layers = self._layers()
        bufs = self.buffers(B, dev)
        self._shadows_on(bufs, layers)
        lib, st = self.lib, _lib.stream_ptr()
        self.version += 1
        eps_mode = spec["eps_mode"]
        xt_out = None
        if eps_mode:
            if bufs.xt is None:
                bufs.xt = torch.zeros(B, bufs.ldi, dtype=torch.float32, device=dev)
            xt_out = bufs.xt
        if csr is not None:
            keepalive = self._train_input_csr(bufs, spec)
        else:
            keepalive = self._train_input(bufs, spec, xt_out)
        x0c = keepalive[0]
        alpha = None
        if eps_mode:
            target, alpha, rowdiv = self._eps_target(bufs, spec, ts, x0c, keepalive[1])
        else:
            target = x0c
            rowdiv = bufs.rowdiv_mse
        A = self._hidden_forward(bufs, layers, B)
        w, bias, _ = layers[-1]
        N, K = w.shape
        self._use_weight(w)
        if csr is not None:
            core.loss_layer_bits(lib, bufs, A, w, bias, bufs.x0bits, None, B, N, K, st)
        else:
            core.loss_layer(lib, bufs, A, w, bias, target, alpha, B, N, K, st)
        loss, self.last_loss_mean = core.loss_tail(lib, bufs, spec, B, rowdiv, alpha, st, mean=True)
        self._saved = dict(kind="train", B=B, bufs=bufs, layers=layers, keepalive=(keepalive, target, alpha, rowdiv, spec["pt"]))
        return loss

    @with_precision
    def train_backward(self, gloss):
        sv = self._saved
        if sv is None or sv.get("kind") != "train":
            raise RuntimeError("gdmcf_amd: train_backward without a preceding training_losses")
        bufs = sv["bufs"]
        if isinstance(gloss, float) and gloss == 1.0 / sv["B"] and getattr(bufs, "rowscale_mean", None) is not None:
            rowscale = bufs.rowscale_mean
        else:
            rowscale = self._rowscale_of(bufs, gloss)
        return self._backward(sv, bufs.diff, rowscale)

    @with_precision
    def forward_plain(self, x, timesteps, training, drop_mask=None):
        self.flush_weight_waiters()
        B, dev = x.shape[0], x.device
        layers = self._layers()
        bufs = self.buffers(B, dev)
        self._shadows_on(bufs, layers)
        lib, st = self.lib, _lib.stream_ptr()
        self.version += 1
        ts = timesteps.to(device=dev, dtype=torch.int64).contiguous()
        keepalive = self._prep(bufs, x, ts, None, None, None, drop_mask, training)
        A = self._hidden_forward(bufs, layers, B)
        w, bias, act = layers[-1]
        N, K = w.shape
        out = torch.empty(B, N, dtype=torch.float32, device=dev)
        core.linear_fwd(lib, bufs, A, w, bias, act, B, N, K, out, st)
        self._saved = dict(kind="plain", B=B, bufs=bufs, layers=layers, keepalive=(keepalive, ts))
        return out

    @with_precision
    def backward_plain(self, gout):
        sv = self._saved
        g = gout.to(torch.float32)
        if g.stride(-1) != 1:
            g = g.contiguous()
        return self._backward(sv, g, None)

    def _backward(self, sv, dz_last, rowscale):
        lib, st = self.lib, _lib.stream_ptr()
        bufs, layers, B = sv["bufs"], sv["layers"], sv["B"]
        m = self.model
        L = len(layers)
        grads_w = [None] * L
        grads_b = [None] * L
        dWe = dbe = None
        fused = self.fused_opt if self.grad_sink is None else None
        dz, rs = dz_last, rowscale
        dw_queue = [] if (fused is not None and self.gemm_dtype == "f32" and os.environ.get("GDMCF_DW_MULTI", "1") != "0") else None

        def input_grad(li, w, A_prev):
            nonlocal dWe, dbe
            N, K = w.shape
            if li > 0:
                dprev = bufs.dzs[li - 1]
                self._input_grad(bufs, B, w, N, K, dz, rs, A_prev, layers[li - 1][2], dprev, st)
                return dprev
            dWe = self._grad_like(m.emb_layer.weight)
            dbe = self._grad_like(m.emb_layer.bias)
            core.emb_bwd(lib, bufs, dz, w, self.I, self.E, B, N, dWe, dbe, st)
            return None

        def weight_grad(li, w, bias, A_prev):
            db = self._grad_like(bias)
            scol = int(rs is None and li == 0 and getattr(bufs, "xin_ones", False) and A_prev.stride(0) > w.shape[1])
            A_use, scol = self._row_scaled(bufs, B, w.shape[1], A_prev, rs, scol, st)
            fs = fused.fused_state(w) if fused is not None else None
            dW = self._grad_like(w) if fs is None else None
            if fs is None and self._gemm_side and self.grad_sink is None and li == L - 1 and L > 1:
                if self._side2 is None:
                    self._side2 = torch.cuda.Stream()
                self._side2.wait_stream(torch.cuda.current_stream())
                with torch.cuda.stream(self._side2):
                    self._weight_grad(bufs, B, w, dz, rs, A_use, scol, dW, db, None, _lib.stream_ptr())
                self._side2_used = True
            else:
                self._weight_grad(bufs, B, w, dz, rs, A_use, scol, dW, db, fs, st, queue=dw_queue)
            grads_w[li], grads_b[li] = dW, db
            if self.grad_sink is not None:
                self.grad_sink(w, dW)
                self.grad_sink(bias, db)
                grads_w[li] = grads_b[li] = None

        for li in range(L - 1, -1, -1):
            w, bias, _ = layers[li]
            A_prev = bufs.acts[li - 1] if li > 0 else bufs.xin
            if fused is not None or self.input_grad_first:
                nxt = input_grad(li, w, A_prev)
                weight_grad(li, w, bias, A_prev)
            else:
                weight_grad(li, w, bias, A_prev)
                nxt = input_grad(li, w, A_prev)
            dz, rs = nxt, None
        if dw_queue:
            arr = (_lib.GdDwAdamw * len(dw_queue))(*[e for e, _ in dw_queue])
            _lib.check(lib.gdmcf_linear_bwd_weight_adamw_multi_f32(ctypes.addressof(arr), len(dw_queue), st))
            for _, w in dw_queue:
                torch.autograd.graph.increment_version(w)
        if self._side2_used:
            torch.cuda.current_stream().wait_stream(self._side2)
            self._side2_used = False
        if self.grad_sink is not None:
            self.grad_sink(m.emb_layer.weight, dWe)
            self.grad_sink(m.emb_layer.bias, dbe)
            dWe = dbe = None
        out = [dWe, dbe]
        for li in range(L):
            out += [grads_w[li], grads_b[li]]
        return out

    @with_precision
    def p_sample_loop(self, x_start, steps, T, tabs32, eps_mode, sampling_noise, noise0=None, step_noise=None,
                      capture=None, draw_noise=None, latent=False, stop=False, eps=None):
        m, lib = self.model, self.lib
        if draw_noise is None:
            def draw_noise(like):
                self.offset += 1
                return _lib.philox_randn(like.shape, like.device, self.seed, self.offset, 7)
        self.flush_weight_waiters()
        B, dev, I = x_start.shape[0], x_start.device, self.I
        from .data_utils import CsrBatch
        csr = x_start if isinstance(x_start, CsrBatch) else None
        if csr is not None and (steps != 0 or m.norm or self.gemm_dtype != "f32" or csr.csr.values is not None):
            raise RuntimeError("gdmcf_amd: the reverse loop takes CSR rows only for steps == 0, binary rows, norm=False and "
                               "float32 products (GaussianDiffusion.p_sample densifies the rest)")
        layers = self._layers()
        bufs = self.buffers(B, dev)
        self._shadows_on(bufs, layers)
        st = _lib.stream_ptr()
        self.version += 1
        if latent:
            if (eps_mode and eps is None) or sampling_noise or capture is not None or m.norm or self.gemm_dtype != "f32":
                raise RuntimeError("gdmcf_amd: the latent reverse loop takes the x0 target without sampling noise, capture or "
                                   "F.normalize, in float32 products (GaussianDiffusion._latent_reverse_ok)")
            return self._latent_loop(bufs, layers, x_start, csr, steps, T, tabs32, noise0, stop=stop, eps=eps if eps_mode else None)
        if bufs.xin2 is None:
            bufs.xin2 = torch.zeros_like(bufs.xin)
        if self.gemm_dtype == "bf16" and getattr(bufs, "sh_xin2", None) is None:
            bufs.sh_xin2 = _lib.Bf16Shadow(bufs.xin2[:, : I + self.E], sync=False)
            bufs.shadows.append(bufs.sh_xin2)
        norm = bool(m.norm)
        keep = []
        t_vec = torch.full((B,), max(steps - 1, 0), dtype=torch.int64, device=dev)
        ca = cb = None
        if steps > 0:
            ca, cb = tabs32["sqrt_ab"], tabs32["sqrt_1mab"]
        w, bias, _ = layers[-1]
        N, K = w.shape
        out = None

        stabs = core.step_tables(tabs32, T, B, ("c1", "c2", "r1", "r2", "sigma"), bufs.tab_cache)
        if getattr(bufs, "step_ts", None) is None or bufs.step_ts.shape[0] != T:
            bufs.step_ts = torch.arange(T, dtype=torch.int64, device=dev)[:, None].expand(T, B).contiguous()
        step_ts = bufs.step_ts

        def posterior(i, n, A, xt, xn):
            c1, c2 = stabs["c1"][i], stabs["c2"][i]
            r1 = r2 = sg = z = None
            if eps_mode:
                r1, r2 = stabs["r1"][i], stabs["r2"][i]
            if sampling_noise and i != 0:
                sg = stabs["sigma"][i]
                z = step_noise[n] if step_noise is not None else draw_noise(xt[:, :I])
                z = z.contiguous()
            pred = torch.empty(B, I, dtype=torch.float32, device=dev) if capture is not None else None
            core.posterior_fwd(lib, A, w, bias, xt, c1, c2, r1, r2, sg, z, B, N, K, xn, pred, st)
            keep.append((c1, c2, r1, r2, sg, z))
            if capture is not None:
                capture.setdefault("pred_xstart", []).append(pred)
                capture.setdefault("mean", []).append(xn[:, :I].clone())

        if not norm:
            cur, nxt = bufs.xin, bufs.xin2
            if csr is not None:
                keep.append(self._prep_csr(bufs, csr, t_vec, None, None, None, None, False))
            else:
                keep.append(self._prep(bufs, x_start, t_vec, ca, cb, noise0, None, False, xin=cur))
            bufs.xin_ones = False
            for n, i in enumerate(range(T - 1, -1, -1)):
                ts = step_ts[i]
                _lib.check(lib.gdmcf_dnn_emb_cols_f32(ts.data_ptr(), m.emb_layer.weight.data_ptr(),
                                                      m.emb_layer.bias.data_ptr(), self.E, B, I, cur.data_ptr(),
                                                      cur.stride(0), bufs.temb.data_ptr(), st))
                keep.append(ts)
                A = self._hidden_forward(bufs, layers, B, xin=cur, frozen=True, csr=csr if n == 0 else None)
                out = torch.empty(B, I, dtype=torch.float32, device=dev) if i == 0 else None
                posterior(i, n, A, cur, out if out is not None else nxt)
                cur, nxt = nxt, cur
        else:
            if bufs.xt is None:
                bufs.xt = torch.zeros(B, bufs.ldi, dtype=torch.float32, device=dev)
            xt = bufs.xt
            keep.append(self._prep(bufs, x_start, t_vec, ca, cb, noise0, None, False, xt_out=xt, xin=bufs.xin2))
            for n, i in enumerate(range(T - 1, -1, -1)):
                ts = step_ts[i]
                keep.append(self._prep(bufs, xt[:, :I], ts, None, None, None, None, False, xin=bufs.xin))
                A = self._hidden_forward(bufs, layers, B, xin=bufs.xin, frozen=True)
                out = torch.empty(B, I, dtype=torch.float32, device=dev) if i == 0 else None
                xn = out if out is not None else (bufs.diff if xt is bufs.xt else bufs.xt)
                posterior(i, n, A, xt, xn)
                xt = xn
        self._saved = None
        del keep
        return out

    def _latent_begin(self, bufs, layers, T, B, tabs32):
        for wl, _, _ in layers:
            self._use_weight(wl)
        (w1, b1, _), (w, bias, _), emb = layers[0], layers[-1], self.model.emb_layer
        ops = self._latent_operands(w1, b1, w, w.shape[1], bias, T, (w1, b1, w, bias, emb.weight, emb.bias))
        ld = _ceil64(w1.shape[0])
        if getattr(bufs, "lat_p", None) is None:
            bufs.lat_p = torch.zeros(B, ld, dtype=torch.float32, device=w1.device)
            bufs.lat_h = torch.zeros_like(bufs.lat_p)
        return ops, core.step_tables(tabs32, T, B, ("c1", "c2"), bufs.tab_cache), bufs.lat_p, ld

    def _latent_run(self, bufs, layers, ops, tabs, T, B, pre, p, e, x_T, **kw):
        (_, _, act1), (w, bias, _), lib, st = layers[0], layers[-1], self.lib, _lib.stream_ptr()

        def middle(n, i, A):
            for li in range(1, len(layers) - 1):
                wl, bl, al = layers[li]
                core.linear_fwd(lib, bufs, A, wl, bl, al, B, wl.shape[0], wl.shape[1], bufs.acts[li], st)
                A = bufs.acts[li]
            return A

        return self._latent_reverse(bufs, ops, T, B, w.shape[1], act1, pre, p, (bufs.acts[0], bufs.lat_h),
                                    middle if len(layers) > 2 else None, e, tabs["c1"], tabs["c2"], w, bias, x_T, **kw)

    def _latent_loop(self, bufs, layers, x_start, csr, steps, T, tabs32, noise0, stop=False, eps=None):
        lib, st, I = self.lib, _lib.stream_ptr(), self.I
        B, dev = x_start.shape[0], x_start.device
        w1 = layers[0][0]
        h1 = w1.shape[0]
        ops, tabs, p, _ = self._latent_begin(bufs, layers, T, B, tabs32)
        t_vec = torch.full((B,), max(steps - 1, 0), dtype=torch.int64, device=dev)
        if csr is not None:
            if stop:
                keep, self.offset = None, self.offset + 1
            else:
                keep = self._prep_csr(bufs, csr, t_vec, None, None, None, None, False)
            wt = self._transposed(w1)
            core.gather_fwd(lib, None, None, csr, wt, I, None, None, 0, None, 0, B, h1, p, st)
        else:
            ca, cb = (tabs32["sqrt_ab"], tabs32["sqrt_1mab"]) if steps > 0 else (None, None)
            keep = self._prep(bufs, x_start, t_vec, ca, cb, noise0, None, False, xin=bufs.xin)
            core.linear_fwd(lib, bufs, (bufs.xin.data_ptr(), bufs.xin.stride(0)), w1, None, 0, B, h1, I, p, st)
        bufs.xin_ones = False
        x0 = self._latent_run(bufs, layers, ops, tabs, T, B, p, p, ops.e, bufs.xin, stop=stop, eps=eps)
        self._saved = None
        del keep
        return x0
```

### gdmcf_amd/engine_core.py

```python
import collections
import functools

import torch

from . import _lib


def _ceil64(n):
    return (int(n) + 63) // 64 * 64


class _Bufs:
    pass


_GEMM_MODES = {k: _lib.CONSTANTS["GDMCF_GEMM_" + k.upper()] for k in ("f32", "bf16", "f32x3")}


def with_precision(fn):
    @functools.wraps(fn)
    def wrapped(self, *a, **kw):
        prev = self.lib.gdmcf_gemm_precision(_GEMM_MODES[self.gemm_dtype])
        try:
            return fn(self, *a, **kw)
        finally:
            self.lib.gdmcf_gemm_precision(prev)
    return wrapped


def _pl(a):
    if type(a) is tuple:
        return a
    return (None, 0) if a is None else (a.data_ptr(), a.stride(0))


def _f32_rows(t):
    return t if t.dtype == torch.float32 and t.stride(-1) == 1 else t.float().contiguous()


def _prep_modes(B, ca, noise, drop_mask, drop_p, training):
    noise_mode = 0
    if ca is not None:
        noise_mode = 1 if noise is not None else 2
        if noise is not None:
            noise = _f32_rows(noise)
    drop_mode, keep = 0, None
    if drop_mask is not None:
        drop_mode = 1
        keep = drop_mask.reshape(B, -1)
        keep = (keep if keep.dtype == torch.uint8 else (keep != 0).to(torch.uint8)).contiguous()
    elif training and drop_p > 0.0:
        drop_mode = 2
    return noise_mode, noise, drop_mode, keep


def prep_input(lib, x, I, ts, ca, cb, noise, drop_mask, drop_p, training, seed, offset, norm, emb, E, xin, xt_out, temb,
               rownorm, st):
    B = x.shape[0]
    x = _f32_rows(x)
    noise_mode, noise, drop_mode, keep = _prep_modes(B, ca, noise, drop_mask, drop_p, training)
    (nz, ldn), (kp, ldkp), (xi, ldx), (xo, ldxo) = _pl(noise), _pl(keep), _pl(xin), _pl(xt_out)
    _lib.check(lib.gdmcf_dnn_prep_input_f32(
        x.data_ptr(), x.stride(0), _lib.ptr(ts), _lib.ptr(ca), _lib.ptr(cb), noise_mode, nz, ldn, drop_mode, kp, ldkp, drop_p,
        seed, offset, int(bool(norm)), emb.weight.data_ptr() if emb is not None else None,
        emb.bias.data_ptr() if emb is not None else None, E, B, I, xi, ldx, xo, ldxo, _lib.ptr(temb), _lib.ptr(rownorm), st))
    return x, noise, keep


def prep_input_csr(lib, batch, ts, ca, cb, noise, drop_mask, drop_p, training, seed, offset, emb, E, xin, temb, x0bits, st):
    B, I = batch.shape
    noise_mode, noise, drop_mode, keep = _prep_modes(B, ca, noise, drop_mask, drop_p, training)
    (nz, ldn), (kp, ldkp) = _pl(noise), _pl(keep)
    c = batch.csr
    _lib.check(lib.gdmcf_dnn_prep_input_csr_f32(
        c.indptr.data_ptr(), c.indices.data_ptr(), batch.row_ids.data_ptr(), _lib.ptr(ts), _lib.ptr(ca), _lib.ptr(cb),
        noise_mode, nz, ldn, drop_mode, kp, ldkp, drop_p, seed, offset, emb.weight.data_ptr(), emb.bias.data_ptr(), E, B, I,
        xin.data_ptr(), xin.stride(0), temb.data_ptr(), x0bits.data_ptr(), x0bits.stride(0), st))
    return batch, noise, keep


def onehot_prep_input_csr(lib, batch, ts_U, discrete, sampled, seed, offset_noise, ts, drop_mask, drop_p, training,
                          offset_prep, emb, E, xin, temb, st, sampled_out=None, x0bits=None):
    B, I = batch.shape
    _, _, drop_mode, keep = _prep_modes(B, None, None, drop_mask, drop_p, training)
    (sp, lds), (kp, ldkp), (so, ldso), (xb, ldb) = _pl(sampled), _pl(keep), _pl(sampled_out), _pl(x0bits)
    c = batch.csr
    _lib.check(lib.gdmcf_onehot_prep_input_csr_f32(
        c.indptr.data_ptr(), c.indices.data_ptr(), batch.row_ids.data_ptr(), _lib.ptr(ts_U), float(discrete), sp, lds, seed,
        offset_noise, so, ldso, _lib.ptr(ts), drop_mode, kp, ldkp, drop_p, offset_prep,
        emb.weight.data_ptr() if emb is not None else None, emb.bias.data_ptr() if emb is not None else None, E, B, I,
        xin.data_ptr(), xin.stride(0), _lib.ptr(temb), xb, ldb, st))
    return batch, sampled, keep


def cat_prep_input_csr(lib, batch, ts_U, discrete, sampled, seed, offset_noise, ts, ca, cb, noise, drop_mask, drop_p, training,
                       offset_prep, cat, emb, E, xin, xt, temb, x0bits, clsbits, st):
    B, I = batch.shape
    noise_mode, noise, drop_mode, keep = _prep_modes(B, ca, noise, drop_mask, drop_p, training)
    (sp, lds), (nz, ldn), (kp, ldkp) = _pl(sampled), _pl(noise), _pl(keep)
    c = batch.csr
    _lib.check(lib.gdmcf_cat_prep_input_csr_f32(
        c.indptr.data_ptr(), c.indices.data_ptr(), batch.row_ids.data_ptr(), _lib.ptr(ts_U), float(discrete), sp, lds,
        offset_noise, ts.data_ptr(), _lib.ptr(ca), _lib.ptr(cb), noise_mode, nz, ldn, drop_mode, kp, ldkp, drop_p, seed,
        offset_prep, cat.weight.data_ptr(), cat.bias.data_ptr(), emb.weight.data_ptr(), emb.bias.data_ptr(), E, B, I,
        xin.data_ptr(), xin.stride(0), xt.data_ptr(), xt.stride(0), temb.data_ptr(), x0bits.data_ptr(), x0bits.stride(0),
        clsbits.data_ptr(), clsbits.stride(0), st))
    return batch, noise, keep, drop_mode


def cat_grad_bits(lib, dxin, xt, x0bits, clsbits, drop_mode, keep, drop_p, seed, offset, B, I, ws, ws_bytes, gw, gb, st):
    (kp, ldkp) = _pl(keep)
    _lib.check(lib.gdmcf_cat_grad_bits_f32(
        dxin.data_ptr(), dxin.stride(0), xt.data_ptr(), xt.stride(0), x0bits.data_ptr(), x0bits.stride(0), clsbits.data_ptr(),
        clsbits.stride(0), drop_mode, kp, ldkp, drop_p, seed, offset, B, I, ws.data_ptr(), ws_bytes, gw.data_ptr(), gb.data_ptr(),
        st))


def linear_fwd(lib, bufs, A, W, bias, act, B, N, K, out, st):
    (a, lda), (w, ldw), (o, ldo) = _pl(A), _pl(W), _pl(out)
    _lib.check(lib.gdmcf_linear_fwd_f32(a, lda, w, ldw, _lib.ptr(bias), act, B, N, K, o, ldo, bufs.ws.data_ptr(),
                                        bufs.ws_bytes, st))


def gather_fwd(lib, pre, base, batch, table, I, a, tblE, E, bias, act, B, N, out, st):
    (p, ldp), (tb, ldt), (ap, lda), (te, ldte), (o, ldo) = _pl(pre), _pl(table), _pl(a), _pl(tblE), _pl(out)
    c = batch.csr if batch is not None else None
    if c is None:
        tb, ldt = None, 0
    if E == 0:
        ap, lda, te, ldte = None, 0, None, 0
    _lib.check(lib.gdmcf_gather_fwd_f32(
        p, ldp, _lib.ptr(base), c.indptr.data_ptr() if c is not None else None, c.indices.data_ptr() if c is not None else None,
        batch.row_ids.data_ptr() if c is not None else None, tb, ldt, I, ap, lda, te, ldte, E, _lib.ptr(bias), act, B, N, o, ldo, st))


def latent_step(lib, A, M, v, p_cur, c1, c2, e, act, B, N, K, p_next, h_next, st):
    (a, lda), (m, ldm), (pc, ldpc), (pn, ldpn), (h, ldh) = _pl(A), _pl(M), _pl(p_cur), _pl(p_next), _pl(h_next)
    _lib.check(lib.gdmcf_latent_step_f32(a, lda, m, ldm, _lib.ptr(v), pc, ldpc, c1.data_ptr(), c2.data_ptr(), _lib.ptr(e), act,
                                         B, N, K, pn, ldpn, h, ldh, None, 0, st))


def latent_step_ex(lib, A, M, v, p_cur, c1, c2, r, e, act, B, N, K, p_next, h_next, acc, st):
    (a, lda), (m, ldm), (pc, ldpc), (pn, ldpn), (h, ldh), (rp, ldr) = _pl(A), _pl(M), _pl(p_cur), _pl(p_next), _pl(h_next), _pl(r)
    (qc, ldqc), (qn, ldqn) = (_pl(acc[0]), _pl(acc[3])) if acc is not None else ((None, 0), (None, 0))
    qa, qb = (acc[1].data_ptr(), acc[2].data_ptr()) if acc is not None else (None, None)
    _lib.check(lib.gdmcf_latent_step_ex_f32(a, lda, m, ldm, _lib.ptr(v), pc, ldpc, c1.data_ptr(), c2.data_ptr(), rp, ldr, _lib.ptr(e),
                                            act, B, N, K, pn, ldpn, h, ldh, qc, ldqc, qa, qb, qn, ldqn, None, 0, st))


def latent_acc(lib, q_cur, qa, A, qb, B, K, q_next, st):
    (qc, ldqc), (a, lda), (qn, ldqn) = _pl(q_cur), _pl(A), _pl(q_next)
    _lib.check(lib.gdmcf_latent_acc_f32(qc, ldqc, qa.data_ptr(), a, lda, qb.data_ptr(), B, K, qn, ldqn, st))


def cand_scores(lib, A, W, I, K, bias, scale, cand, ldcand, B, C, mask_ptrs, rows, out, st):
    (a, lda), (w, ldw), (o, ldo) = _pl(A), _pl(W), _pl(out)
    _lib.check(lib.gdmcf_cand_scores_f32(a, lda, w, ldw, I, K, _lib.ptr(bias), _lib.ptr(scale), cand.data_ptr(), ldcand, B, C,
                                         *mask_ptrs, _lib.ptr(rows), o, ldo, st))


def cand_pick(lib, dense, B, I, scale, cand, ldcand, C, mask_ptrs, rows, out, st):
    (d, ldd), (o, ldo) = _pl(dense), _pl(out)
    _lib.check(lib.gdmcf_cand_pick_f32(d, ldd, B, I, _lib.ptr(scale), cand.data_ptr(), ldcand, C, *mask_ptrs, _lib.ptr(rows), o,
                                       ldo, st))


def step_tables(tabs32, T, B, names, cache=None):
    key = (id(tabs32), int(T), int(B))
    rec = cache.get(names) if cache is not None else None
    if rec is None or rec[0] != key:
        rec = (key, {k: tabs32[k][:T, None].expand(T, B).contiguous() for k in names if k in tabs32})
        if cache is not None:
            cache[names] = rec
    return rec[1]


LatentProduct = collections.namedtuple("LatentProduct", "A second K bias scale")


class EpsTables:

    def __init__(self, c1, c2, r1, r2, T):
        import numpy as np
        c1, c2, r1, r2 = (np.asarray(t, dtype=np.float64)[:T] for t in (c1, c2, r1, r2))
        g, d = c1 * r1 + c2, c1 * r2
        G, D = 1.0, 0.0
        with np.errstate(all="ignore"):
            for t in range(T - 1, -1, -1):
                G, D = g[t] * G, g[t] * D + d[t]
            qa, qb = g.copy(), d.copy()
            qa[T - 1] = 0.0
            qa[0], qb[0] = qa[0] / D, qb[0] / D
        self.g, self.d, self.qa, self.qb = (t.astype(np.float32) for t in (g, d, qa, qb))
        self.G, self.D = float(np.float32(G)), float(np.float32(D))
        self.ok = bool(all(np.isfinite(t).all() for t in (self.g, self.d, self.qa, self.qb)) and np.isfinite(self.G)
                       and np.isfinite(self.D) and self.D > 0)
        self._dev = {}

    def on(self, device, B):
        rec, key = self._dev, (str(device), int(B))
        if key not in rec:
            def tab(a):
                return torch.from_numpy(a).to(device)[:, None].expand(len(a), B).contiguous()
            f = dict(dtype=torch.float32, device=device)
            rec[key] = dict(neg_d=tab(-self.d), g=tab(self.g), qa=tab(self.qa), qb=tab(self.qb), G=torch.full((B,), self.G, **f),
                            D=torch.full((B,), self.D, **f), one=torch.ones(B, **f), zero=torch.zeros(B, **f))
            rec[key]["qa0_neg"], rec[key]["qb0_neg"] = -rec[key]["qa"][0], -rec[key]["qb"][0]
        return rec[key]


def linear_bwd_input(lib, bufs, dz, W, rs, A_prev, act_prev, B, N, K, d_prev, st):
    (z, ldz), (w, ldw), (a, lda), (d, ldd) = _pl(dz), _pl(W), _pl(A_prev), _pl(d_prev)
    _lib.check(lib.gdmcf_linear_bwd_input_f32(z, ldz, w, ldw, _lib.ptr(rs), a, lda, act_prev, B, N, K, d, ldd,
                                              bufs.ws.data_ptr(), bufs.ws_bytes, st))


def linear_bwd_weight(lib, dz, A, rs, scol, B, N, K, dW, db, st):
    (z, ldz), (a, lda) = _pl(dz), _pl(A)
    _lib.check(lib.gdmcf_linear_bwd_weight_f32(z, ldz, a, lda, _lib.ptr(rs), scol, B, N, K, dW.data_ptr(), dW.stride(0),
                                               _lib.ptr(db), 0, st))


def adamw_args(fs, w):
    if fs["exp_avg"].stride() != w.stride() or fs["exp_avg_sq"].stride() != w.stride():
        raise RuntimeError("gdmcf_amd: the moments of a fused weight must share its leading dimension")
    return (fs["exp_avg"].data_ptr(), fs["exp_avg_sq"].data_ptr(), fs["lr"], fs["beta1"], fs["beta2"], fs["eps"],
            fs["weight_decay"], fs["step"], fs["grad_scale"])


def dw_adamw_args(dz, A, rs, scol, B, N, K, w, db, fs):
    (z, ldz), (a, lda) = _pl(dz), _pl(A)
    ad = adamw_args(fs, w)
    return (z, ldz, a, lda, _lib.ptr(rs), scol, B, N, K, w.data_ptr(), w.stride(0), ad[0], ad[1], _lib.ptr(db)) + ad[2:]


def linear_bwd_weight_adamw(lib, args, st):
    _lib.check(lib.gdmcf_linear_bwd_weight_adamw_f32(*args, st))


def rowscale(lib, A, rs, B, K, out, st):
    (a, lda), (o, ldo) = _pl(A), _pl(out)
    _lib.check(lib.gdmcf_rowscale_f32(a, lda, rs.data_ptr(), B, K, o, ldo, st))


def emb_bwd(lib, bufs, dz, W, I_cols, E, B, N, dWe, dbe, st):
    (z, ldz), (w, ldw) = _pl(dz), _pl(W)
    _lib.check(lib.gdmcf_emb_bwd_f32(z, ldz, w, ldw, I_cols, E, bufs.temb.data_ptr(), B, N, bufs.demb.data_ptr(),
                                     dWe.data_ptr(), dbe.data_ptr(), st))


def loss_layer(lib, bufs, A, W, bias, target, alpha, B, N, K, st):
    (a, lda), (w, ldw) = _pl(A), _pl(W)
    _lib.check(lib.gdmcf_linear_loss_fwd_f32(a, lda, w, ldw, _lib.ptr(bias), target.data_ptr(), target.stride(0),
                                             _lib.ptr(alpha), B, N, K, None, 0, bufs.diff.data_ptr(), bufs.ldi,
                                             bufs.rowpart.data_ptr(), bufs.rowsum.data_ptr(), st))


def loss_layer_bits(lib, bufs, A, W, bias, x0bits, alpha, B, N, K, st):
    (a, lda), (w, ldw) = _pl(A), _pl(W)
    _lib.check(lib.gdmcf_linear_loss_fwd_bits_f32(a, lda, w, ldw, _lib.ptr(bias), x0bits.data_ptr(), x0bits.stride(0),
                                                  _lib.ptr(alpha), B, N, K, None, 0, bufs.diff.data_ptr(), bufs.ldi,
                                                  bufs.rowpart.data_ptr(), bufs.rowsum.data_ptr(), st))


def loss_tail(lib, bufs, spec, B, rowdiv, alpha, st, mean=False):
    ts = spec["ts"]
    loss = torch.empty(B, dtype=torch.float64, device=ts.device)
    args = (bufs.rowsum.data_ptr(), rowdiv.data_ptr(), _lib.ptr(alpha), ts.data_ptr(), spec["weight_t"].data_ptr(),
            spec["pt"].data_ptr(), B, spec["T"], spec["H"], spec["Lt_history"].data_ptr(), spec["Lt_count"].data_ptr(),
            int(spec["update_history"]), bufs.lu.data_ptr(), loss.data_ptr(), bufs.gradcoef.data_ptr())
    if not mean:
        _lib.check(lib.gdmcf_row_loss_finish_f64(*args, st))
        return loss
    loss_mean = torch.empty((), dtype=torch.float64, device=ts.device)
    if getattr(bufs, "rowscale_mean", None) is None:
        bufs.rowscale_mean = torch.zeros(B, dtype=torch.float32, device=ts.device)
    _lib.check(lib.gdmcf_row_loss_finish_mean_f64(*args, loss_mean.data_ptr(), bufs.rowscale_mean.data_ptr(), st))
    return loss, loss_mean


def posterior_fwd(lib, A, W, bias, x_t, c1, c2, r1, r2, sigma, z, B, N, K, x_next, pred, st):
    (a, lda), (w, ldw), (zp, ldz), (pp, ldp) = _pl(A), _pl(W), _pl(z), _pl(pred)
    _lib.check(lib.gdmcf_linear_posterior_fwd_f32(
        a, lda, w, ldw, _lib.ptr(bias), x_t.data_ptr(), x_t.stride(0), c1.data_ptr(), c2.data_ptr(), _lib.ptr(r1),
        _lib.ptr(r2), _lib.ptr(sigma), zp, ldz, B, N, K, x_next.data_ptr(), x_next.stride(0), pp, ldp, st))


class TrainLoss(torch.autograd.Function):

    @staticmethod
    def forward(ctx, eng, spec, *params):
        loss = eng.train_forward(spec)
        ctx.eng, ctx.version = eng, eng.version
        return loss

    @staticmethod
    def backward(ctx, gloss):
        eng = ctx.eng
        if ctx.version != eng.version:
            raise RuntimeError("gdmcf_amd: activations were overwritten by a later forward; "
                               "call backward before the next training_losses/forward")
        return (None, None, *eng.train_backward(gloss))


class EngineBase:
    supports_grad_sink = True

    def __init__(self, model):
        self.model = model
        self.lib = _lib.load()
        self.E = int(model.time_emb_dim)
        self.I = int(model.in_dims[0])
        self.version = 0
        self.seed = int(torch.initial_seed()) & 0xFFFFFFFFFFFFFFFF
        self.offset = 0
        self._bufs = {}
        self._saved = None
        self._wt = {}
        self._latent = None
        self.grad_sink = None
        self.fused_opt = None

    @property
    def gemm_dtype(self):
        return getattr(self.model, "gemm_dtype", "f32")

    def manual_seed(self, seed):
        self.seed = int(seed) & 0xFFFFFFFFFFFFFFFF
        self.offset = 0

    def _check_params(self, layers):
        what = type(self.model).__name__ + " parameters"
        for w, b, _ in layers:
            _lib.require_gpu(w, what)
            if not (w.stride(1) == 1 and w.stride(0) >= w.shape[1] and b.is_contiguous() and w.dtype == torch.float32):
                raise RuntimeError(f"gdmcf_amd: {what} must be float32 with unit column stride")

    def _transposed(self, w):
        rec = self._wt.get(id(w))
        if rec is None or rec[0] is not w or rec[1] != w._version or rec[2].device != w.device:
            n, k = w.shape
            buf = torch.zeros(k, (n + 31) // 32 * 32, dtype=torch.float32, device=w.device)
            buf[:, :n].copy_(w.detach().t())
            rec = self._wt[id(w)] = (w, w._version, buf)
        return rec[2]

    def _emb_table(self, w, bias, I_cols, T, st):
        m, lib, E, h, dev = self.model, self.lib, self.E, w.shape[0], w.device
        f32 = dict(dtype=torch.float32, device=dev)
        e = torch.zeros(T, _ceil64(h), **f32)
        if E == 0:
            e[:, :h].copy_(bias.detach()[None, :].expand(T, h))
            return e, None
        ew, eb = m.emb_layer.weight, m.emb_layer.bias
        xs = torch.zeros(T, _ceil64(4 + E), **f32)
        ts = torch.arange(T, dtype=torch.int64, device=dev)
        temb = torch.zeros(T, E, **f32)
        _lib.check(lib.gdmcf_dnn_emb_cols_f32(ts.data_ptr(), ew.data_ptr(), eb.data_ptr(), E, T, 4, xs.data_ptr(), xs.stride(0),
                                              temb.data_ptr(), st))
        we_t = torch.zeros(E, (h + 3) // 4 * 4, **f32)
        we_t[:, :h].copy_(w.detach()[:, I_cols:I_cols + E].t())
        gather_fwd(lib, None, None, None, None, I_cols, (xs.data_ptr() + 16, xs.stride(0)), we_t, E, bias, 0, T, h, e, st)
        return e, (xs, ts, temb, we_t)

    def _latent_operands(self, w1, bias1, second, K, b_out, T, entering, tables=()):
        lib, st = self.lib, _lib.stream_ptr()
        key = tuple((t.data_ptr(), t._version, str(t.device)) for t in entering) + (int(T), int(K), b_out is None)
        if self._latent is not None and self._latent[0] == key:
            return self._latent[1]
        h, I, dev = w1.shape[0], self.I, w1.device
        f32 = dict(dtype=torch.float32, device=dev)
        o, ws = _Bufs(), _Bufs()
        ws.ws_bytes = int(max(lib.gdmcf_linear_ws_bytes(h, I, K), lib.gdmcf_linear_ws_bytes(1, h, I)))
        ws.ws = torch.empty(max(ws.ws_bytes, 256), dtype=torch.uint8, device=dev)
        w1x = (w1.data_ptr(), w1.stride(0))
        o.M = torch.zeros(h, _ceil64(K), **f32)
        linear_bwd_input(lib, ws, w1x, second, None, None, 0, h, I, K, o.M, st)
        o.v = o.neg_b = None
        if b_out is not None:
            o.v = torch.zeros(h, **f32)
            linear_fwd(lib, ws, (b_out.data_ptr(), I), w1x, None, 0, 1, h, I, (o.v.data_ptr(), h), st)
            o.neg_b = -b_out.detach()
        ones = torch.ones(I, **f32)
        o.S = torch.zeros(h, **f32)
        linear_fwd(lib, ws, (ones.data_ptr(), I), w1x, None, 0, 1, h, I, (o.S.data_ptr(), h), st)
        o.keep_S = ones
        o.e, o.keep = self._emb_table(w1, bias1, I, T, st)
        o.tabs = [self._emb_table(w, b, cols, T, st) for w, b, cols in tables]
        self._latent = (key, o)
        return o

    def _latent_reverse(self, bufs, ops, T, B, K, act, pre, p, hpair, small, e, c1, c2, second, b_out, x_T, stop=False, eps=None,
                        r=None, c1_of=None, before_step=None):
        lib, st, I, dev, h = self.lib, _lib.stream_ptr(), self.I, p.device, ops.M.shape[0]
        s1, s2, Q = c1, c2, None
        if eps is not None:
            et = eps.on(dev, B)
            s1, s2, qa, qb = et["neg_d"], et["g"], et["qa"], et["qb"]
            if getattr(bufs, "lat_q", None) is None:
                bufs.lat_q = torch.zeros(B, _ceil64(K), dtype=torch.float32, device=dev)
            Q = bufs.lat_q
        if c1_of is not None:
            s1 = c1_of(s1)
        plain = r is None and Q is None
        hcur, hnxt = hpair
        gather_fwd(lib, pre, None, None, None, I, None, None, 0, e[T - 1], act, B, h, hcur, st)
        for n, i in enumerate(range(T - 1, -1, -1)):
            if before_step is not None:
                before_step(n, i)
            A = small(n, i, hcur) if small is not None else hcur
            if i == 0:
                break
            if plain:
                latent_step(lib, A, ops.M, ops.v, p, s1[i], s2[i], e[i - 1], act, B, h, K, p, hnxt, st)
            else:
                latent_step_ex(lib, A, ops.M, ops.v, p, s1[i], s2[i], r, e[i - 1], act, B, h, K, p, hnxt,
                               (Q, qa[i], qb[i], Q) if Q is not None else None, st)
            hcur, hnxt = hnxt, hcur
        if eps is not None:
            qa0, qb0 = (et["qa0_neg"], et["qb0_neg"]) if stop else (qa[0], qb[0])
            latent_acc(lib, Q, qa0, A, qb0, B, K, Q, st)
            if stop:
                return LatentProduct(Q, second, K, ops.neg_b, et["D"])
        elif stop:
            return LatentProduct(A, second, K, b_out, c1[0])
        x0 = torch.empty(B, I, dtype=torch.float32, device=dev)
        if eps is not None:
            posterior_fwd(lib, Q, second, b_out, x_T, et["one"], et["zero"], et["G"], et["D"], None, None, B, I, K, x0, None, st)
        else:
            posterior_fwd(lib, A, second, b_out, x_T, c1[0], c2[0], None, None, None, None, B, I, K, x0, None, st)
        return x0

    @with_precision
    def score_product(self, A, second, K, b_out, B, device):
        bufs = self.buffers(B, device)
        if getattr(bufs, "scores", None) is None:
            bufs.scores = torch.empty(B, self.I, dtype=torch.float32, device=device)
        self._grow_workspace(bufs, B, device, [(self.I, K)])
        linear_fwd(self.lib, bufs, A, second, b_out, 0, B, self.I, K, bufs.scores, _lib.stream_ptr())
        return bufs.scores

    def _gather_first_layer(self, bufs, batch, w, bias, act, xin, B, out, st):
        N, I, E = w.shape[0], self.I, self.E
        wt = self._transposed(w)
        emb_cols = (xin.data_ptr() + 4 * I, xin.stride(0))
        gather_fwd(self.lib, None, None, batch, wt, I, emb_cols, (wt.data_ptr() + 4 * I * wt.stride(0), wt.stride(0)), E, bias, act,
                   B, N, out, st)

    def _shared_buffers(self, b, B, device, n_loss, n_first, weights):
        lib, I, E = self.lib, self.I, self.E
        f32 = dict(dtype=torch.float32, device=device)
        b.temb = torch.zeros(B, max(E, 1), **f32)
        b.rownorm = torch.zeros(B, **f32)
        b.ldi = _ceil64(I)
        b.diff = torch.zeros(B, b.ldi, **f32)
        b.xt = None
        b.rowpart = torch.zeros(B, lib.gdmcf_loss_tiles(n_loss), **f32)
        b.rowsum = torch.zeros(B, **f32)
        b.gradcoef = torch.zeros(B, **f32)
        b.rowdiv_mse = torch.full((B,), float(I), **f32)
        b.lu = torch.zeros(B, dtype=torch.float64, device=device)
        b.demb = torch.zeros((B + n_first) * max(E, 1), **f32)
        b.ws_bytes = 0
        b.tab_cache = {}
        self._grow_workspace(b, B, device, [w.shape for w in weights])

    def _grow_workspace(self, b, B, device, shapes):
        ws = max([b.ws_bytes] + [self.lib.gdmcf_linear_ws_bytes(B, n, k) for n, k in shapes])
        if ws > b.ws_bytes or getattr(b, "ws", None) is None:
            b.ws_bytes = int(ws)
            b.ws = torch.empty(max(ws, 256), dtype=torch.uint8, device=device)

    def _prep_input(self, bufs, x, I, xin, ts, ca, cb, noise, drop_mask, training, xt_out=None):
        m = self.model
        self.offset += 1
        return prep_input(self.lib, x, I, ts, ca, cb, noise, drop_mask, float(m.drop.p), training, self.seed, self.offset,
                          m.norm, m.emb_layer, self.E, xin, xt_out, bufs.temb, bufs.rownorm, _lib.stream_ptr())

    def _eps_target(self, bufs, spec, ts, x0, noise):
        B, dev = ts.shape[0], ts.device
        x0 = _f32_rows(x0)
        target = noise if spec.get("noise_owned", False) else torch.empty(B, self.I, dtype=torch.float32, device=dev)
        alpha = torch.empty(B, dtype=torch.float32, device=dev)
        rowdiv = torch.empty(B, dtype=torch.float32, device=dev)
        _lib.check(self.lib.gdmcf_eps_target_f32(
            noise.data_ptr(), noise.stride(0), bufs.xt.data_ptr(), bufs.xt.stride(0), x0.data_ptr(), x0.stride(0), ts.data_ptr(),
            spec["r1_0"].data_ptr(), spec["r2_0"].data_ptr(), int(bool(spec.get("t0_likelihood", True))), B, self.I,
            target.data_ptr(), target.stride(0), alpha.data_ptr(), rowdiv.data_ptr(), _lib.stream_ptr()))
        return target, alpha, rowdiv

    def _rowscale_of(self, bufs, gloss):
        if isinstance(gloss, float):
            return bufs.gradcoef * gloss
        return (gloss.to(torch.float32) * bufs.gradcoef).contiguous()

    def _fused_state(self, w):
        fused = self.fused_opt if self.grad_sink is None else None
        return fused.fused_state(w) if fused is not None else None

    def _row_scaled(self, bufs, B, K, A, rs, scol, st):
        if rs is None:
            return A, scol
        rowscale(self.lib, A, rs, B, K, bufs.hs, st)
        return bufs.hs, int(bufs.hs.stride(0) > K)

    def _weight_grad(self, bufs, B, w, dz, rs, A, scol, dW, db, fs, st, queue=None):
        N, K = w.shape
        if fs is None:
            linear_bwd_weight(self.lib, dz, A, rs, scol, B, N, K, dW, db, st)
            return
        args = dw_adamw_args(dz, A, rs, scol, B, N, K, w, db, fs)
        if queue is not None:
            queue.append((_lib.GdDwAdamw(*args), w))
            return
        linear_bwd_weight_adamw(self.lib, args, st)
        if not (self.gemm_dtype == "bf16" and _lib.shadow_info(w.data_ptr()) is not None):
            torch.autograd.graph.increment_version(w)

    def _input_grad(self, bufs, B, W, N, K, dz, rs, A_prev, act_prev, d_prev, st):
        linear_bwd_input(self.lib, bufs, dz, W, rs, A_prev, act_prev, B, N, K, d_prev, st)
```

### gdmcf_amd/graph.py

```python
import ctypes

import torch

from . import _lib
from .DNN import DNN
from .data_utils import CsrBatch
from .gaussian_diffusion import ModelMeanType
from .parallel import DataParallelStep


class GraphedTrainStep:
    def __init__(self, diffusion, model, optimizer, csr, batch_size, reweight=True, warmup=3, table_steps=8192, group=None,
                 force_exchange=False):
        dist = torch.distributed
        multi = dist.is_available() and dist.is_initialized() and (dist.get_world_size(group) > 1 or force_exchange)
        self._no_capture = None
        if multi and dist.get_backend(group) != "nccl":
            self._no_capture = ("NotImplementedError: a captured gradient exchange needs the nccl (RCCL) backend; backend "
                                f"'{dist.get_backend(group)}' stages its collectives through the host")
        if not isinstance(model, DNN) or model.norm or diffusion.mean_type != ModelMeanType.START_X:
            raise NotImplementedError("GraphedTrainStep: plain DNN denoiser without F.normalize, x0 target")
        if getattr(diffusion, "CatOneHot", False) or diffusion.rng != "philox" or diffusion.noise_scale == 0.0:
            raise NotImplementedError("GraphedTrainStep: continuous diffusion with in-kernel Philox randomness")
        if len(optimizer.param_groups) != 1 or not hasattr(optimizer, "grad_scale"):
            raise NotImplementedError("GraphedTrainStep: a gdmcf_amd.FusedAdamW, one parameter group")
        if csr.values is not None:
            raise NotImplementedError("GraphedTrainStep: interaction values must all be 1 (rows stay sparse)")
        self.diffusion, self.model, self.optimizer, self.reweight = diffusion, model, optimizer, reweight
        self.lib = _lib.load()
        dev = csr.device
        self.ids = torch.zeros(batch_size, dtype=torch.int64, device=dev)
        self.batch = CsrBatch(csr, self.ids)
        assert self.batch.row_ids.data_ptr() == self.ids.data_ptr()
        self.eng = model.engine
        self.eng.static_grads = True
        self.step = DataParallelStep(diffusion, model, optimizer, group=group, force_exchange=bool(force_exchange) and multi)
        self.warmup, self.calls, self.graph, self.loss = int(warmup), 0, None, None
        self.capture_error = None
        self.table_steps = int(table_steps)
        self._state = None
        self._upload_state()

    def _host_counters(self):
        steps = {int(st.get("step", 0)) for st in self.optimizer.state.values() if "step" in st} or {0}
        if len(steps) != 1:
            raise RuntimeError("GraphedTrainStep: all parameters must share the optimizer step count")
        return int(self.eng.offset), int(getattr(self.diffusion, "_ts_calls", 0)), steps.pop()

    def _upload_state(self, counters=None):
        lib, dev = self.lib, self.ids.device
        prep, ts, step = counters if counters is not None else self._host_counters()
        g = self.optimizer.param_groups[0]
        self._hyper = self._hyper_now()
        hb, sb = lib.gdmcf_adam_hyper_bytes(), lib.gdmcf_graph_state_bytes()
        host_tab = (ctypes.c_ubyte * (hb * self.table_steps))()
        _lib.check(lib.gdmcf_adam_hyper_fill(host_tab, self.table_steps, g["lr"], g["betas"][0], g["betas"][1], g["eps"],
                                             g["weight_decay"], step + 1, float(self.optimizer.grad_scale)))
        self._table = torch.frombuffer(host_tab, dtype=torch.uint8).clone().to(dev)
        host_st = (ctypes.c_ubyte * sb)()
        _lib.check(lib.gdmcf_graph_state_init(host_st, prep, ts, step, step + 1, self.table_steps, self._table.data_ptr()))
        new = torch.frombuffer(host_st, dtype=torch.uint8).clone().to(dev)
        if getattr(self, "_state", None) is None:
            self._state = new
        else:
            self._state.copy_(new)
        self._table_end = step + self.table_steps
        self._dev_step = step

    def _hyper_now(self):
        g = self.optimizer.param_groups[0]
        return (float(g["lr"]), float(g["betas"][0]), float(g["betas"][1]), float(g["eps"]), float(g["weight_decay"]),
                float(self.optimizer.grad_scale))

    def _read_state(self):
        torch.cuda.synchronize()
        raw = self._state.cpu().numpy().tobytes()
        prep, ts = int.from_bytes(raw[0:8], "little"), int.from_bytes(raw[8:16], "little")
        step = int.from_bytes(raw[16:24], "little", signed=True)
        return prep, ts, step

    def _body(self):
        _lib.check(self.lib.gdmcf_graph_state_tick(self._state.data_ptr(), _lib.stream_ptr()))
        return self.step(self.batch, self.reweight)

    def __call__(self, row_ids):
        if row_ids.numel() != self.ids.numel():
            raise ValueError("GraphedTrainStep: every batch must have the captured batch size")
        self.ids.copy_(row_ids, non_blocking=True)
        self.calls += 1
        if self._hyper_now() != self._hyper or self._dev_step + 1 > self._table_end:
            self._upload_state(self._read_state())
        if self.graph is None or self.graph is False:
            self.lib.gdmcf_graph_state_bind(self._state.data_ptr())
            try:
                if self.calls <= self.warmup or self.graph is False:
                    self._dev_step += 1
                    return self._body().clone()
                if self._no_capture is not None:
                    self.graph, self.capture_error = False, self._no_capture
                    self._dev_step += 1
                    return self._body().clone()
                self.lib.gdmcf_prof_enable(0)
                g = torch.cuda.CUDAGraph()
                try:
                    torch.cuda.synchronize()
                    if self.step.exchange:
                        import time
                        time.sleep(0.35)
                    with torch.cuda.graph(g, capture_error_mode="thread_local" if self.step.exchange else "global"):
                        self.loss = self._body()
                    self.graph = g
                except Exception as exc:
                    self.graph, self.capture_error = False, f"{type(exc).__name__}: {exc}"[:300]
                    torch.cuda.synchronize()
                    self._dev_step += 1
                    return self._body().clone()
            finally:
                self.lib.gdmcf_graph_state_bind(None)
        self.graph.replay()
        self._bump_versions()
        self._dev_step += 1
        return self.loss.clone()

    def _bump_versions(self):
        for p in self.model.parameters():
            torch.autograd.graph.increment_version(p)

    def close(self):
        if self._state is None:
            return
        prep, ts, step = self._read_state()
        self.eng.offset = prep
        if self.reweight:
            self.diffusion._ts_calls = ts
        for st in self.optimizer.state.values():
            if "step" in st:
                st["step"] = step
        self.eng.static_grads = False
        self._bump_versions()
        self.graph, self._state = None, None

    def __enter__(self):
        return self

    def __exit__(self, *exc):
        self.close()
        return False
```

### gdmcf_amd/parallel.py

```python
import functools

import torch
import torch.distributed as dist


def _host_staged(group):
    return dist.get_backend(group) == "gloo"


def _all_reduce(t, group, async_op=False):
    if t.is_cuda and _host_staged(group):
        h = t.cpu()
        dist.all_reduce(h, op=dist.ReduceOp.SUM, group=group)
        t.copy_(h)
        return None
    return dist.all_reduce(t, op=dist.ReduceOp.SUM, group=group, async_op=async_op)


def all_gather_rows(local, n_total, group=None):
    world = dist.get_world_size(group)
    if local.is_cuda and _host_staged(group):
        h = local.cpu()
        parts = [torch.empty_like(h) for _ in range(world)]
        dist.all_gather(parts, h, group=group)
        return torch.cat(parts)[:n_total].to(local.device)
    out = torch.empty(world * local.shape[0], local.shape[1], dtype=local.dtype, device=local.device)
    dist.all_gather_into_tensor(out, local.contiguous(), group=group)
    return out[:n_total]


def reduce_scatter_rows(rows, group=None):
    world, rank = dist.get_world_size(group), dist.get_rank(group)
    n = rows.shape[0] // world
    if rows.is_cuda and _host_staged(group):
        h = rows.cpu()
        dist.all_reduce(h, op=dist.ReduceOp.SUM, group=group)
        return h[rank * n:(rank + 1) * n].to(rows.device), None
    if _host_staged(group):
        h = rows.clone()
        dist.all_reduce(h, op=dist.ReduceOp.SUM, group=group)
        return h[rank * n:(rank + 1) * n].contiguous(), None
    out = torch.empty(n, rows.shape[1], dtype=rows.dtype, device=rows.device)
    return out, dist.reduce_scatter_tensor(out, rows, op=dist.ReduceOp.SUM, group=group, async_op=True)


def all_gather_rows_inplace(full, group=None):
    world, rank = dist.get_world_size(group), dist.get_rank(group)
    n = full.shape[0] // world
    mine = full[rank * n:(rank + 1) * n]
    if _host_staged(group):
        h = mine.cpu() if mine.is_cuda else mine.clone()
        parts = [torch.empty_like(h) for _ in range(world)]
        dist.all_gather(parts, h, group=group)
        full.copy_(torch.cat(parts).to(full.device))
        return None
    return dist.all_gather_into_tensor(full, mine, group=group, async_op=True)


def allreduce_grads(params, group=None, bucket_bytes=256 << 20, force=False):
    if not dist.is_initialized() or (dist.get_world_size(group) == 1 and not force):
        return
    small, handles = [], []
    for p in params:
        if p.grad is None:
            continue
        g = p.grad
        if g.numel() * g.element_size() >= (1 << 20):
            handles.append(_all_reduce(g, group, async_op=True))
        else:
            small.append(g)
    if small:
        flat = torch.cat([g.reshape(-1) for g in small])
        _all_reduce(flat, group)
        off = 0
        for g in small:
            g.copy_(flat[off:off + g.numel()].view_as(g))
            off += g.numel()
    for h in handles:
        if h is not None:
            h.wait()


def gather_history_inputs(ts, loss_unscaled, group=None, force=False):
    if not dist.is_initialized() or (dist.get_world_size(group) == 1 and not force):
        return ts, loss_unscaled
    world = dist.get_world_size(group)
    dev = ts.device
    if ts.is_cuda and _host_staged(group):
        ts, loss_unscaled = ts.cpu(), loss_unscaled.cpu()
    ts_all = [torch.empty_like(ts) for _ in range(world)]
    lu_all = [torch.empty_like(loss_unscaled) for _ in range(world)]
    dist.all_gather(ts_all, ts.contiguous(), group=group)
    dist.all_gather(lu_all, loss_unscaled.contiguous(), group=group)
    return torch.cat(ts_all).to(dev), torch.cat(lu_all).to(dev)


def broadcast_parameters(model, group=None, src=0, force=False):
    if dist.is_initialized() and (dist.get_world_size(group) > 1 or force):
        for p in model.parameters():
            if p.is_cuda and _host_staged(group):
                h = p.data.cpu()
                dist.broadcast(h, src=src, group=group)
                p.data.copy_(h)
            else:
                dist.broadcast(p.data, src=src, group=group)
            torch.autograd.graph.increment_version(p)


class DataParallelStep:

    def __init__(self, diffusion, model, optimizer, group=None, overlap=True, early_update=False, direct_backward=True,
                 shard_optimizer=False, force_exchange=False, defer_gather=True):
        self.diffusion, self.model, self.optimizer, self.group = diffusion, model, optimizer, group
        self.direct_backward = direct_backward
        self.defer_gather = bool(defer_gather)
        self.shard_optimizer = (bool(shard_optimizer) and overlap and hasattr(optimizer, "step_rows")
                                and getattr(model.engine, "supports_grad_sink", False))
        self._sharded = []
        self.world = dist.get_world_size(group) if dist.is_initialized() else 1
        self._handles, self._small = [], []
        self.exchange = self.world > 1 or (bool(force_exchange) and dist.is_initialized())
        if self.exchange:
            diffusion.update_history = False
            optimizer.grad_scale = 1.0 / self.world
            if hasattr(optimizer, "unfuse") and (hasattr(model, "layer_list") or hasattr(model, "fusable_weights")):
                optimizer.unfuse(model)
            model.engine.fused_opt = None
            if hasattr(optimizer, "_fused_ids"):
                optimizer._fused_ids = set()
            broadcast_parameters(model, group, force=True)
            if overlap and getattr(model.engine, "supports_grad_sink", False):
                model.engine.grad_sink = self._sink
            if getattr(model.engine, "supports_grad_sink", False):
                model.register_state_dict_pre_hook(lambda *a, **k: self.flush())
        elif (early_update and hasattr(optimizer, "step_subset") and getattr(model.engine, "fused_opt", None) is None
              and next(model.parameters()).is_cuda):
            self._side = torch.cuda.Stream()
            self._side_busy = False
            model.engine.grad_sink = self._sink_local
            model.engine.input_grad_first = True

    def _sink(self, param, grad):
        if (self.shard_optimizer and param.grad is None and grad.dim() == 2 and grad.is_contiguous()
                and grad.numel() * grad.element_size() >= (1 << 20) and grad.shape[0] >= self.world):
            n_eq = grad.shape[0] // self.world * self.world
            shard, h = reduce_scatter_rows(grad[:n_eq], self.group)
            tail = grad[n_eq:]
            h2 = _all_reduce(tail, self.group, async_op=True) if tail.numel() else None
            self._sharded.append((param, grad, shard, h, tail, h2, n_eq))
            return
        param.grad = grad if param.grad is None else param.grad.add_(grad)
        g = param.grad
        if g.numel() * g.element_size() >= (1 << 20):
            self._handles.append((param, _all_reduce(g, self.group, async_op=True)))
        else:
            self._small.append(g)

    def set_shard_optimizer(self, flag):
        flag = (bool(flag) and hasattr(self.optimizer, "step_rows") and self.exchange
                and getattr(self.model.engine, "grad_sink", None) is not None)
        if self.shard_optimizer and not flag:
            self.gather_optimizer_state()
        self.shard_optimizer = flag
        return flag

    def gather_optimizer_state(self):
        if not (self.shard_optimizer and self.exchange):
            return
        self.flush()
        for p in self.model.parameters():
            st = self.optimizer.state.get(p)
            if st and p.dim() == 2 and p.numel() * 4 >= (1 << 20) and p.shape[0] >= self.world:
                n_eq = p.shape[0] // self.world * self.world
                for key in ("exp_avg", "exp_avg_sq"):
                    h = all_gather_rows_inplace(st[key][:n_eq], self.group)
                    if h is not None:
                        h.wait()

    def _sink_local(self, param, grad):
        param.grad = grad if param.grad is None else param.grad.add_(grad)
        if param.grad.numel() * param.grad.element_size() < (1 << 20):
            return
        self.optimizer._init_state(param)
        done = torch.cuda.Event()
        done.record()
        self._side.wait_event(done)
        with torch.cuda.stream(self._side):
            self.optimizer.step_subset([param])
        self._side_busy = True

    def _finish_exchange(self):
        import ctypes
        from . import _lib
        lib, st = _lib.load(), _lib.stream_ptr()
        d = self.diffusion
        ts, lu = d.last_ts, d.last_loss_unscaled
        B, dev = ts.numel(), ts.device
        rank = dist.get_rank(self.group)
        small = self._small
        for i, g in enumerate(small):
            if g.dtype != torch.float32 or not g.is_contiguous():
                raise RuntimeError("DataParallelStep: small gradients must be contiguous float32")
        n = len(small)
        if n > 16:
            raise RuntimeError("DataParallelStep: more than 16 small gradient tensors")
        ptrs = (ctypes.c_void_p * max(n, 1))(*[g.data_ptr() for g in small])
        counts = (ctypes.c_int64 * max(n, 1))(*[g.numel() for g in small])
        n_small = sum(g.numel() for g in small)
        flat = torch.empty(n_small + self.world * B * 2, dtype=torch.float64, device=dev)
        ts = ts if ts.dtype == torch.int64 and ts.is_contiguous() else ts.to(torch.int64).contiguous()
        lu = lu if lu.dtype == torch.float64 and lu.is_contiguous() else lu.double().contiguous()
        _lib.check(lib.gdmcf_dp_pack_f64(ptrs, counts, n, ts.data_ptr(), lu.data_ptr(), B, rank, self.world,
                                         flat.data_ptr(), st))
        hflat = _all_reduce(flat, self.group, async_op=True) if self._sharded else None
        pending = []
        for param, grad, shard, h, tail, h2, n_eq in self._sharded:
            if h is not None:
                h.wait()
            nr = n_eq // self.world
            self.optimizer.step_rows(param, shard, rank * nr)
            if tail.numel():
                if h2 is not None:
                    h2.wait()
                self.optimizer.step_rows(param, tail, n_eq)
            pending.append((param, n_eq))
        self._gathers = [(param, all_gather_rows_inplace(param.data[:n_eq], self.group)) for param, n_eq in reversed(pending)]
        had_sharded, self._sharded = bool(self._sharded), []
        early = hasattr(self.optimizer, "step_subset")
        for k, (param, h) in enumerate(self._handles):
            if h is not None:
                h.wait()
            if early and k + 1 < len(self._handles):
                self.optimizer.step_subset([param])
        if not had_sharded:
            _all_reduce(flat, self.group)
        elif hflat is not None:
            hflat.wait()
        ts_all = torch.empty(self.world * B, dtype=torch.int64, device=dev)
        lu_all = torch.empty(self.world * B, dtype=torch.float64, device=dev)
        _lib.check(lib.gdmcf_dp_unpack_f64(flat.data_ptr(), ptrs, counts, n, B, self.world, ts_all.data_ptr(),
                                           lu_all.data_ptr(), st))
        self._handles, self._small = [], []
        return ts_all, lu_all

    def __call__(self, batch, reweight=True, **rand):
        from . import _lib
        self.optimizer.zero_grad()
        eng = getattr(self.model, "engine", None)
        if self.direct_backward and eng is not None:
            with torch.no_grad():
                losses = self.diffusion.training_losses(self.model, batch, reweight, **rand)
            loss = getattr(eng, "last_loss_mean", None)
            if loss is None:
                loss = losses["loss"].mean()
            grads = eng.train_backward(1.0 / losses["loss"].numel())
            for p, g in zip(self.model.param_list(), grads):
                if g is not None:
                    p.grad = g if p.grad is None else p.grad.add_(g)
        else:
            losses = self.diffusion.training_losses(self.model, batch, reweight, **rand)
            loss = losses["loss"].mean()
            loss.backward()
            if getattr(eng, "last_loss_mean", None) is not None:
                loss = eng.last_loss_mean
        if self.exchange:
            d = self.diffusion
            if getattr(self.model.engine, "grad_sink", None) is not None:
                ts_all, lu_all = self._finish_exchange()
            else:
                allreduce_grads(self.model.parameters(), self.group, force=True)
                ts_all, lu_all = gather_history_inputs(d.last_ts, d.last_loss_unscaled, self.group, force=True)
            _lib.check(_lib.load().gdmcf_lt_history_update(ts_all.data_ptr(), lu_all.data_ptr(), ts_all.numel(),
                                                           d.steps, d.history_num_per_term, d.Lt_history.data_ptr(),
                                                           d.Lt_count.data_ptr(), _lib.stream_ptr()))
        if getattr(self, "_side_busy", False):
            torch.cuda.current_stream().wait_stream(self._side)
            self._side_busy = False
        self.optimizer.step()
        for param, h in getattr(self, "_gathers", []):
            if self.defer_gather and eng is not None and hasattr(eng, "weight_waiters"):
                eng.weight_waiters[id(param)] = functools.partial(self._arrived, param, h)
            else:
                self._arrived(param, h)
        self._gathers = []
        return loss.detach()

    @staticmethod
    def _arrived(param, h):
        if h is not None:
            h.wait()
        torch.autograd.graph.increment_version(param)

    def flush(self):
        eng = getattr(self.model, "engine", None)
        if eng is not None and hasattr(eng, "flush_weight_waiters"):
            eng.flush_weight_waiters()
```

### include/gdmcf_hip.h

```cpp
#ifndef GDMCF_HIP_H
#define GDMCF_HIP_H
#include <stddef.h>
#include <stdint.h>

#ifdef __cplusplus
extern "C" {
#endif

#define GDMCF_OK 0
#define GDMCF_E_SHAPE (-1)
#define GDMCF_E_ARG (-2)
#define GDMCF_E_UNSUPPORTED (-3)
#define GDMCF_E_HIP (-4)
#define GDMCF_E_WORKSPACE (-5)

int gdmcf_version(void);
const char* gdmcf_last_error(void);
int gdmcf_device_info(int* n_cu, int* wave_size, char* arch_host, int arch_len);
int gdmcf_debug_last_gemm(void);
int gdmcf_debug_fat_slab_plan(int M, int N, int K, int* nb, int* splits, int* cps);
int gdmcf_debug_dr_tn_plan(int M, int N, int K, int64_t lddz, int64_t lda, int64_t ldw, int bias_col, int fused, int* depth,
                           int* ksp, int* tiles_m, int* tiles_n, int* m_fastest, int* has_bias);

int gdmcf_prof_enable(int on);
int gdmcf_prof_collect(int cap, int* tags_host, float* ms_host, double* work_host);

#define GDMCF_N_TABLES 13
int gdmcf_schedule_build(int kind, double noise_scale, double noise_min, double noise_max, int T,
                         int beta_fixed, double* out_tables_host);

int gdmcf_densify_rows_f32(const int64_t* indptr, const int32_t* indices, const float* values,
                           const int64_t* row_ids, int B, int I, float* out, int64_t ldo, void* stream);

int gdmcf_dnn_prep_input_f32(const float* x, int64_t ldx, const int64_t* ts, const float* ca,
                             const float* cb, int noise_mode, const float* noise, int64_t ldn,
                             int drop_mode, const uint8_t* keep, int64_t ldkeep, float drop_p,
                             uint64_t seed, uint64_t offset, int normalize, const float* emb_w,
                             const float* emb_b, int E, int B, int I, float* xin, int64_t ldxin,
                             float* xt_out, int64_t ldxt, float* temb_out, float* rownorm_ws,
                             void* stream);
int gdmcf_dnn_prep_input_csr_f32(const int64_t* indptr, const int32_t* indices, const int64_t* rows, const int64_t* ts,
                                 const float* ca, const float* cb, int noise_mode, const float* noise, int64_t ldn,
                                 int drop_mode, const uint8_t* keep, int64_t ldkeep, float drop_p, uint64_t seed,
                                 uint64_t offset, const float* emb_w, const float* emb_b, int E, int B, int I, float* xin,
                                 int64_t ldxin, float* temb_out, uint32_t* bits_out, int64_t ldbits, void* stream);

int gdmcf_onehot_noise_f32(const float* x0, int64_t ldx, const int64_t* ts, int B, int I, float discrete,
                           const uint8_t* sampled, int64_t lds, uint64_t seed, uint64_t offset,
                           float* xU, int64_t ldu, uint8_t* sampled_out, int64_t ldso, void* stream);
int gdmcf_onehot_prep_input_csr_f32(const int64_t* indptr, const int32_t* indices, const int64_t* rows, const int64_t* ts_U,
                                    float discrete, const uint8_t* sampled, int64_t lds, uint64_t seed, uint64_t offset_noise,
                                    uint8_t* sampled_out, int64_t ldso, const int64_t* ts, int drop_mode, const uint8_t* keep,
                                    int64_t ldkeep, float drop_p, uint64_t offset_prep, const float* emb_w, const float* emb_b,
                                    int E, int B, int I, float* xin, int64_t ldxin, float* temb_out, uint32_t* bits_out,
                                    int64_t ldbits, void* stream);

int gdmcf_randn_f32(float* out, int64_t ld, int rows, int cols, int stream_id, uint64_t seed, uint64_t offset, void* stream);

int gdmcf_eps_target_f32(const float* noise, int64_t ldn, const float* xt, int64_t ldxt, const float* x0, int64_t ldx0,
                         const int64_t* ts, const float* r1, const float* r2, int t0_likelihood, int B, int I, float* target,
                         int64_t ldt, float* alpha, float* rowdiv, void* stream);

int gdmcf_graph_guided_step_u8(uint8_t* graph, int64_t ldg, const int64_t* ts, int B, int I, float discrete,
                               const uint8_t* sampled_in, int64_t lds, const uint8_t* pick_in, const float* degree_prob,
                               int user_guided, uint64_t seed, uint64_t offset, uint8_t* sampled_out, int64_t ldso,
                               uint8_t* pick_out, void* stream);

int gdmcf_dnn_emb_cols_f32(const int64_t* ts, const float* emb_w, const float* emb_b, int E, int B,
                           int I, float* xin, int64_t ldxin, float* temb_out, void* stream);

enum { GDMCF_GEMM_F32 = 0, GDMCF_GEMM_BF16 = 1, GDMCF_GEMM_F32X3 = 2 };
int gdmcf_gemm_precision(int mode);
int gdmcf_bf16_shadow_set(const float* f32, void* bf16, int64_t rows, int64_t cols, int64_t ld_bf16);
int gdmcf_bf16_shadow_clear(const float* f32 );
void* gdmcf_bf16_shadow_get(const float* f32);
int gdmcf_bf16_shadow_info(const float* f32, void** bf16, int64_t* rows, int64_t* cols, int64_t* ld_bf16);
int gdmcf_bf16_shadow_sync(const float* f32, int64_t ld, void* stream);
size_t gdmcf_linear_ws_bytes(int M, int N, int K);
int gdmcf_linear_fwd_f32(const float* A, int64_t lda, const float* W, int64_t ldw,
                         const float* bias, int act, int M, int N, int K, float* C, int64_t ldc,
                         void* ws, size_t ws_bytes, void* stream);
int gdmcf_linear_fwd_wt_f32(const float* A, int64_t lda, const float* Wt, int64_t ldwt,
                            const float* bias, int act, int M, int N, int K, float* C, int64_t ldc,
                            void* ws, size_t ws_bytes, void* stream);
int gdmcf_gather_fwd_f32(const float* pre, int64_t ldpre, const float* base, const int64_t* indptr, const int32_t* indices,
                         const int64_t* rows, const float* table, int64_t ldt, int I, const float* a, int64_t lda,
                         const float* tblE, int64_t ldte, int E, const float* bias, int act, int B, int N, float* out, int64_t ldo,
                         void* stream);
int gdmcf_latent_step_f32(const float* A, int64_t lda, const float* M, int64_t ldm, const float* v,
                          const float* p_cur, int64_t ldpc, const float* c1, const float* c2, const float* e, int act,
                          int B, int N, int K, float* p_next, int64_t ldpn, float* h_next, int64_t ldh,
                          void* ws, size_t ws_bytes, void* stream);
size_t gdmcf_latent_step_ws_bytes(int B, int N, int K);
int gdmcf_latent_step_ex_f32(const float* A, int64_t lda, const float* M, int64_t ldm, const float* v,
                             const float* p_cur, int64_t ldpc, const float* c1, const float* c2, const float* r, int64_t ldr,
                             const float* e, int act, int B, int N, int K, float* p_next, int64_t ldpn, float* h_next,
                             int64_t ldh, const float* q_cur, int64_t ldqc, const float* qa, const float* qb, float* q_next,
                             int64_t ldqn, void* ws, size_t ws_bytes, void* stream);
int gdmcf_latent_acc_f32(const float* q_cur, int64_t ldqc, const float* qa, const float* A, int64_t lda, const float* qb,
                         int B, int K, float* q_next, int64_t ldqn, void* stream);
int gdmcf_loss_tiles(int N);
int gdmcf_linear_loss_fwd_f32(const float* A, int64_t lda, const float* W, int64_t ldw,
                              const float* bias, const float* target, int64_t ldt,
                              const float* alpha, int M, int N, int K, float* out, int64_t ldo,
                              float* diff, int64_t ldd, float* rowpart, float* rowsum,
                              void* stream);
int gdmcf_linear_loss_fwd_bits_f32(const float* A, int64_t lda, const float* W, int64_t ldw, const float* bias,
                                   const uint32_t* target_bits, int64_t ldbits, const float* alpha, int M, int N, int K,
                                   float* out, int64_t ldo, float* diff, int64_t ldd, float* rowpart, float* rowsum,
                                   void* stream);
int gdmcf_linear_posterior_fwd_f32(const float* A, int64_t lda, const float* W, int64_t ldw,
                                   const float* bias, const float* x_t, int64_t ldxt,
                                   const float* c1, const float* c2, const float* r1,
                                   const float* r2, const float* sigma, const float* z,
                                   int64_t ldz, int M, int N, int K, float* x_next,
                                   int64_t ldxn, float* pred_out, int64_t ldp, void* stream);
int gdmcf_linear_bwd_input_f32(const float* dZ, int64_t lddz, const float* W, int64_t ldw,
                               const float* rowscale, const float* Aact, int64_t ldact, int act,
                               int M, int N, int K, float* dA, int64_t ldda, void* ws,
                               size_t ws_bytes, void* stream);
int gdmcf_linear_bwd_weight_f32(const float* dZ, int64_t lddz, const float* A, int64_t lda,
                                const float* rowscale, int a_scale_col, int M, int N, int K,
                                float* dW, int64_t lddw, float* db, int accumulate, void* stream);
int gdmcf_linear_bwd_weight_adamw_f32(const float* dZ, int64_t lddz, const float* A, int64_t lda,
                                      const float* rowscale, int a_scale_col, int M, int N, int K, float* W,
                                      int64_t ldw, float* exp_avg, float* exp_avg_sq, float* db, float lr,
                                      float beta1, float beta2, float eps, float weight_decay, int step,
                                      float grad_scale, void* stream);
typedef struct GdDwAdamw {
    const float* dZ;
    int64_t lddz;
    const float* A;
    int64_t lda;
    const float* rowscale;
    int a_scale_col, M, N, K;
    float* W;
    int64_t ldw;
    float* exp_avg;
    float* exp_avg_sq;
    float* db;
    float lr, beta1, beta2, eps, weight_decay;
    int step;
    float grad_scale;
} GdDwAdamw;
int gdmcf_linear_bwd_weight_adamw_multi_f32(const GdDwAdamw* list, int n, void* stream);
int gdmcf_rowscale_f32(const float* A, int64_t lda, const float* rowscale, int M, int K, float* out,
                       int64_t ldo, void* stream);
int gdmcf_row_norms_f32(const float* X, int64_t ld, int rows, int cols, float* norm, float* inv_norm,
                        void* stream);
int gdmcf_normalize_rows_bwd_f32(const float* dY, int64_t lddy, const float* Y, int64_t ldy,
                                 const float* inv_norm, int rows, int cols, float* dX, int64_t lddx,
                                 void* stream);
int gdmcf_tanh_bwd_f32(const float* dA, int64_t ldd, const float* A, int64_t lda, const float* extra,
                       int64_t lde, const float* scale, int M, int N, float* out, int64_t ldo,
                       void* stream);
int gdmcf_gather_rows_f32(const float* src, int64_t lds, const int64_t* index, int n, int cols, float* dst,
                          int64_t ldd, void* stream);
int gdmcf_scatter_add_rows_f32(const float* src, int64_t lds, const int64_t* index, int n, int cols,
                               float* dst, int64_t ldd, void* stream);
int gdmcf_normalize_rows_bwd_adamw_f32(const float* dY, int64_t lddy, const float* Y, int64_t ldy,
                                       const float* inv_norm, int rows, int cols, float* X, int64_t ldx,
                                       float* exp_avg, float* exp_avg_sq, float lr, float beta1, float beta2,
                                       float eps, float weight_decay, int step, float grad_scale, void* stream);
int gdmcf_scatter_rows_adamw_f32(const float* src, int64_t lds, const int64_t* index, int n, int rows, int cols,
                                 float* W, int64_t ldw, float* exp_avg, float* exp_avg_sq, float lr, float beta1,
                                 float beta2, float eps, float weight_decay, int step, float grad_scale,
                                 void* stream);
int gdmcf_emb_bwd_f32(const float* dZ1, int64_t lddz, const float* W1, int64_t ldw, int I, int E,
                      const float* temb, int M, int N, float* demb_ws, float* dWe, float* dbe,
                      void* stream);

int gdmcf_row_loss_finish_f64(const float* rowsum, const float* rowdiv, const float* alpha,
                              const int64_t* ts, const double* weight_t, const double* pt, int B,
                              int T, int H, double* Lt_history, int64_t* Lt_count,
                              int update_history, double* loss_unscaled, double* loss,
                              float* gradcoef, void* stream);
int gdmcf_row_loss_finish_mean_f64(const float* rowsum, const float* rowdiv, const float* alpha, const int64_t* ts,
                                   const double* weight_t, const double* pt, int B, int T, int H, double* Lt_history,
                                   int64_t* Lt_count, int update_history, double* loss_unscaled, double* loss,
                                   float* gradcoef, double* loss_mean, float* rowscale_mean, void* stream);
int gdmcf_lt_history_update(const int64_t* ts, const double* loss_unscaled, int B, int T, int H,
                            double* Lt_history, int64_t* Lt_count, void* stream);

int gdmcf_dp_pack_f64(const float* const* grads, const int64_t* counts, int n, const int64_t* ts,
                      const double* loss_unscaled, int B, int rank, int world, double* flat,
                      void* stream);
int gdmcf_dp_unpack_f64(const double* flat, float* const* grads, const int64_t* counts, int n, int B,
                        int world, int64_t* ts_all, double* loss_unscaled_all, void* stream);

int gdmcf_sample_timesteps(const double* Lt_history, const int64_t* Lt_count, int T, int H, int B,
                           double uniform_prob, uint64_t seed, uint64_t offset, int64_t* ts,
                           double* pt, double* p_out, void* stream);

int gdmcf_adamw_f32(const int64_t* table, int n_tensors, int total_blocks, float lr, float beta1,
                    float beta2, float eps, float weight_decay, int step, float grad_scale,
                    void* stream);
int gdmcf_adamw_bf16s_f32(const int64_t* table, const int64_t* shadow_table, int n_tensors, int total_blocks, float lr,
                          float beta1, float beta2, float eps, float weight_decay, int step, float grad_scale,
                          void* stream);

int gdmcf_topk_masked_f32(const float* pred, int64_t ldp, int B, int I, const int64_t* mask_indptr,
                          const int32_t* mask_indices, int k, int64_t* idx_out, float* val_out,
                          void* stream);
int gdmcf_topk_masked_rows_f32(const float* pred, int64_t ldp, int B, int I, const int64_t* indptr, const int32_t* indices,
                               const int64_t* indptr2, const int32_t* indices2, const int64_t* rows, const float* scale, int k,
                               int64_t* idx_out, float* val_out, void* stream);
int gdmcf_rank_targets_f32(const float* pred, int64_t ldp, int B, int I, const int64_t* indptr, const int32_t* indices,
                           const int64_t* indptr2, const int32_t* indices2, const int64_t* tgt_indptr, const int32_t* tgt_indices,
                           const int64_t* rows, int G, int32_t* rank_out, int64_t ldr, int32_t* n_live_out, void* stream);

int gdmcf_cand_scores_f32(const float* A, int64_t lda, const float* W, int64_t ldw, int I, int K, const float* bias,
                          const float* scale, const int64_t* cand, int64_t ldcand, int B, int C, const int64_t* indptr,
                          const int32_t* indices, const int64_t* indptr2, const int32_t* indices2, const int64_t* rows, float* out,
                          int64_t ldo, void* stream);
int gdmcf_cand_pick_f32(const float* dense, int64_t ldd, int B, int I, const float* scale, const int64_t* cand, int64_t ldcand,
                        int C, const int64_t* indptr, const int32_t* indices, const int64_t* indptr2, const int32_t* indices2,
                        const int64_t* rows, float* out, int64_t ldo, void* stream);

size_t gdmcf_score_topk_ws_bytes(int n_rows, int n_items, int d, int k);
int gdmcf_score_topk_f32(const float* user_emb, int64_t ldu, const int64_t* user_ids, int n_rows, const float* item_emb,
                         int64_t ldi, int n_items, int d, const int64_t* mask_indptr, const int32_t* mask_indices, int k,
                         int64_t* out_idx, float* out_val, void* ws, size_t ws_bytes, void* stream);

int gdmcf_debug_score_rank_plan(int n_rows, int n_items, int G, int* tile_rows, int* pass_targets, int* passes, int* slabs);
size_t gdmcf_score_rank_ws_bytes(int n_rows, int n_items, int d, int G);
int gdmcf_score_rank_f32(const float* user_emb, int64_t ldu, const int64_t* user_ids, int n_rows, const float* item_emb,
                         int64_t ldi, int n_items, int d, const int64_t* mask_indptr, const int32_t* mask_indices,
                         const int64_t* tgt_indptr, const int32_t* tgt_indices, int G, int32_t* rank_out, int64_t ldr,
                         int32_t* n_live_out, void* ws, size_t ws_bytes, void* stream);

int gdmcf_topn_metrics_f64(const int64_t* pred_idx, int64_t ldp, int U, const int64_t* gt_indptr, const int32_t* gt_indices,
                           const int* topN_host, int n_topn, double* out, void* stream);
int gdmcf_rank_metrics_f64(const int32_t* ranks, int64_t ldr, int U, int G, const int* topN_host, int n_topn, double* out,
                           void* stream);

int gdmcf_spmm_csr_f32(const int64_t* vbeg, const int64_t* vend, const int32_t* vrow, const int32_t* vslot,
                       int n_virtual, int n_short, const int32_t* lrow, const int32_t* lptr, int n_long, const int32_t* col,
                       const float* val, int n_rows, const float* X, int64_t ldx, int d, float* Y,
                       int64_t ldy, float* partial_ws, const float* const* addends_host, int n_add,
                       int64_t ld_add, float scale, double alg_bytes, void* stream);
int gdmcf_spmm_bundled_f32(const int32_t* wdesc, int n_waves, const int64_t* lbeg, const int32_t* llen, const int32_t* lrow,
                           const int32_t* lslot, int n_pieces, const int64_t* sbeg, const int32_t* slen, const int32_t* srow,
                           const int32_t* smax, int n_bundles, const int32_t* crow, const int32_t* cptr, int n_cut,
                           const int32_t* col, const float* val, int64_t nnz, int n_rows, int n_x_rows, const float* X,
                           int64_t ldx, int d, float* Y, int64_t ldy, float* partial_ws, const float* const* addends_host, int n_add, int64_t ld_add,
                           float scale, double alg_bytes, void* stream);
int gdmcf_spmm_stream_f32(const int32_t* wdesc, int n_waves, const int32_t* cw, int64_t n_entries, const int32_t* ud, int n_units,
                          const int32_t* crow, const int32_t* cptr, int n_cut, int n_rows, int n_x_rows, const float* X,
                          int64_t ldx, int d, float* Y, int64_t ldy, float* partial_ws, const float* const* addends_host,
                          int n_add, int64_t ld_add, float scale, double alg_bytes, void* stream);
int gdmcf_debug_spmm_stamps(int n_waves, long long* host_out);
int gdmcf_graph_state_bytes(void);
int gdmcf_adam_hyper_bytes(void);
int gdmcf_graph_state_init(void* state_host, uint64_t prep_offset, uint64_t ts_offset, int64_t adam_step, int64_t table_first,
                           int64_t table_len, const void* hyper_table_dev);
int gdmcf_adam_hyper_fill(void* out_host, int n, float lr, float beta1, float beta2, float eps, float weight_decay,
                          int64_t first_step, float grad_scale);
int gdmcf_graph_state_bind(const void* state_dev);
int gdmcf_graph_state_tick(void* state_dev, void* stream);
int gdmcf_scale_f32(const float* acc, int64_t n, float scale, float* out, void* stream);

int gdmcf_bpr_sample_f32(const int64_t* indptr, const int32_t* indices, const int64_t* users, int B, int n_users, int n_items,
                         uint64_t seed, uint64_t offset, int64_t* pos, int64_t* neg, int32_t* flag, void* stream);
int gdmcf_bpr_sample_pool_f32(const int64_t* indptr, const int32_t* indices, const int64_t* users, int B, int n_negs, int pool,
                              int n_users, int n_items, const float* M, int64_t ldm, int d, uint64_t seed, uint64_t offset,
                              int64_t* pos, int64_t* neg, int32_t* flag, void* stream);
int gdmcf_bpr_loss_f32(const float* M, int64_t ldm, const float* E0, int64_t lde, int d, const int64_t* users, const int64_t* pos,
                       const int64_t* neg, int B, int n_users, int n_items, float* coef, float* ws, float* mf, float* reg,
                       int32_t* flag, void* stream);
int gdmcf_bpr_grad_f32(int mode, const int32_t* order, const int64_t* users, const int64_t* pos, const int64_t* neg, int B,
                       int n_users, int n_items, const float* coef, const float* src, int64_t ld_src, int d, float* out,
                       int64_t ld_out, float scale, float* zero_rows, int64_t ld_zero, void* stream);

int gdmcf_cat_prep_input_f32(const float* x, int64_t ldx, const float* xU, int64_t ldu, const int64_t* ts, const float* ca,
                             const float* cb, int noise_mode, const float* noise, int64_t ldn, int drop_mode, const uint8_t* keep,
                             int64_t ldkeep, float drop_p, uint64_t seed, uint64_t offset, const float* cat_w, const float* cat_b,
                             const float* emb_w, const float* emb_b, int E, int B, int I, float* xin, int64_t ldxin, float* xt_out,
                             int64_t ldxt, float* temb_out, void* stream);
size_t gdmcf_cat_grad_ws_bytes(int B, int I);
int gdmcf_cat_grad_f32(const float* dxin, int64_t lddx, const float* xt, int64_t ldxt, const float* xU, int64_t ldu, int drop_mode,
                       const uint8_t* keep, int64_t ldkeep, float drop_p, uint64_t seed, uint64_t offset, int B, int I, void* ws,
                       size_t ws_bytes, float* grad_w, float* grad_b, void* stream);
int gdmcf_cat_prep_input_csr_f32(const int64_t* indptr, const int32_t* indices, const int64_t* rows, const int64_t* ts_U,
                                 float discrete, const uint8_t* sampled, int64_t lds, uint64_t offset_noise, const int64_t* ts,
                                 const float* ca, const float* cb, int noise_mode, const float* noise, int64_t ldn, int drop_mode,
                                 const uint8_t* keep, int64_t ldkeep, float drop_p, uint64_t seed, uint64_t offset_prep,
                                 const float* cat_w, const float* cat_b, const float* emb_w, const float* emb_b, int E, int B, int I,
                                 float* xin, int64_t ldxin, float* xt_out, int64_t ldxt, float* temb_out, uint32_t* x0bits_out,
                                 int64_t ldx0bits, uint32_t* clsbits_out, int64_t ldclsbits, void* stream);
int gdmcf_cat_grad_bits_f32(const float* dxin, int64_t lddx, const float* xt, int64_t ldxt, const uint32_t* x0bits, int64_t ldx0bits,
                            const uint32_t* clsbits, int64_t ldclsbits, int drop_mode, const uint8_t* keep, int64_t ldkeep,
                            float drop_p, uint64_t seed, uint64_t offset, int B, int I, void* ws, size_t ws_bytes, float* grad_w,
                            float* grad_b, void* stream);

size_t gdmcf_ntxent_ws_bytes(int B);
int gdmcf_ntxent_fwd_f32(const float* z1, int64_t ld1, const float* z2, int64_t ld2, int B, int d, float temperature, float eps,
                         void* ws, size_t ws_bytes, float* loss_out, void* stream);
int gdmcf_ntxent_bwd_f32(const float* z1, int64_t ld1, const float* z2, int64_t ld2, int B, int d, const void* ws, size_t ws_bytes,
                         const float* scale, float* dz1, int64_t lddz1, float* dz2, int64_t lddz2, void* stream);

#ifdef __cplusplus
}
#endif
#endif
```

Measured before the change: 323,400 users/s.

## Run loss tail on idle workgroup of input-gradient split-K GEMM

Defers the per-row loss finish (rowpart reduce, loss/gradcoef computation, Lt history FIFO update, row scaling of hidden activations) and runs it inside an otherwise idle workgroup of the dr_kn backward-input GEMM kernel. This removes several small serial kernel launches from the critical path by overlapping them with the GEMM. In exchange, the GEMM kernel now requests large dynamic LDS and carries an extra argument, and the weight-gradient path for the last layer reads precomputed scaled activations. It falls back to separate kernels when no idle workgroup exists.

```diff
diff --git a/gdmcf_amd/_lib.py b/gdmcf_amd/_lib.py
--- a/gdmcf_amd/_lib.py
+++ b/gdmcf_amd/_lib.py
@@ -96,6 +96,10 @@
     _fields_ = parse_structs(_HEADER)["GdDwAdamw"]
 
 
+class GdKnTail(ctypes.Structure):
+    _fields_ = parse_structs(_HEADER)["GdKnTail"]
+
+
 _lib = None
 
 
diff --git a/gdmcf_amd/build.py b/gdmcf_amd/build.py
--- a/gdmcf_amd/build.py
+++ b/gdmcf_amd/build.py
@@ -7,7 +7,7 @@
 
 CSRC = os.path.join(os.path.dirname(os.path.abspath(__file__)), "csrc")
 SOURCES = ["capi.hip", "dp_exchange.hip", "gemm_f32.hip", "gemm_bf16.hip", "gemm_split.hip", "gemm_small.hip", "gemm_dr.hip", "gemm_dr_tn.hip", "gemm_dr_fat.hip", "gemm_dr_kn.hip", "prep_input.hip", "noise.hip", "loss_tail.hip", "adamw.hip", "rows.hip", "reduce.hip", "linear.hip", "topk.hip", "spmm_csr.hip", "rank_metrics.hip", "spmm_bundle.hip", "score_topk.hip", "score_rank.hip", "bpr.hip", "cat.hip", "gather_fwd.hip", "ntxent.hip", "latent_step.hip", "cand_scores.hip", "rank.hip"]
-HEADERS = ["common.h", "draws.h", "rank_order.h", "score_product.h", "spmm.h", "gemm_dr.h", "gemm_epilogue.h", os.path.join("..", "..", "include", "gdmcf_hip.h")]
+HEADERS = ["common.h", "draws.h", "rank_order.h", "score_product.h", "spmm.h", "gemm_dr.h", "gemm_epilogue.h", "tail_job.h", os.path.join("..", "..", "include", "gdmcf_hip.h")]
 LIB = os.path.join(CSRC, "libgdmcf_hip.so")
 ASM_LINT = ("gemm_dr_tn.hip", "gemm_split.hip")
 STORE_LINT = ("gemm_f32.hip", "gemm_bf16.hip", "gemm_dr_fat.hip", "gemm_dr_kn.hip", "score_topk.hip", "score_rank.hip", "latent_step.hip", "bpr.hip")
diff --git a/gdmcf_amd/csrc/gemm_dr_kn.hip b/gdmcf_amd/csrc/gemm_dr_kn.hip
--- a/gdmcf_amd/csrc/gemm_dr_kn.hip
+++ b/gdmcf_amd/csrc/gemm_dr_kn.hip
@@ -1,4 +1,7 @@
+#include <stdlib.h>
+
 #include "gemm_dr.h"
+#include "tail_job.h"
 
 namespace {
 
@@ -6,19 +9,25 @@
 #define GD_KN_EVERY 4
 #endif
 template <int NL>
-__global__ __launch_bounds__(256, 1) void dr_kn_kernel(const DrArgs d) {
+__global__ __launch_bounds__(256, 1) void dr_kn_kernel(const DrArgs d, const GdTailJob job) {
     constexpr int TMB = 5;
     const GdGemm& g = d.g;
     const int lane = threadIdx.x & 63;
     const int wave = __builtin_amdgcn_readfirstlane(threadIdx.x >> 6);
     const int r = lane & 15, q = lane >> 4;
     const int nblk = gridDim.x, per = nblk >> 3;
-    const int wl = ((nblk & 7) == 0 ? ((int)(blockIdx.x & 7) * per + (int)(blockIdx.x >> 3)) : (int)blockIdx.x) * 4 + wave;
+    const int slot = (nblk & 7) == 0 ? ((int)(blockIdx.x & 7) * per + (int)(blockIdx.x >> 3)) : (int)blockIdx.x;
+    const int wl = slot * 4 + wave;
     const int n_waves = nblk * 4;
     const int ntiles = d.tiles_m * d.tiles_n;
     const int CPS = d.ksp;
     const int total_chunks = (g.K + 15) >> 4;
     const int ntasks = ntiles * g.splits;
+    if (job.on && slot == (ntasks + 3) >> 2) {
+        extern __shared__ __attribute__((aligned(16))) unsigned char kn_lds[];
+        gd_tail_job_run(job, kn_lds);
+        return;
+    }
     const __amdgpu_buffer_rsrc_t srdA = __builtin_amdgcn_make_buffer_rsrc(const_cast<float*>(g.A), 0, (int)(((int64_t)(g.M - 1) * g.lda + g.K) * 4), 0x00020000);
     const __amdgpu_buffer_rsrc_t srdB = __builtin_amdgcn_make_buffer_rsrc(const_cast<float*>(g.B), 0, (int)(((int64_t)(g.K - 1) * g.ldb + g.N) * 4), 0x00020000);
     const uint32_t ldb16 = (uint32_t)g.ldb * 64u;
@@ -133,7 +142,13 @@
     return splits;
 }
 
-int gd_dr_kn_launch(GdGemm& g, hipStream_t s) {
+static bool kn_idle_workgroup(int ntasks, int n_cu) { return gd_cdiv(ntasks, 4) < n_cu; }
+
+#ifndef GD_KN_TAIL_DEFAULT
+#define GD_KN_TAIL_DEFAULT 1
+#endif
+
+static int kn_launch(GdGemm& g, const GdTailJob* job, hipStream_t s) {
     if (!dr_routes().kn) return GD_DR_NOT_TAKEN;
     const int splits = gd_dr_kn_splits(g.M, g.N, g.K);
     const size_t need = (size_t)splits * g.M * g.ldc * sizeof(float);
@@ -145,18 +160,41 @@
     const int n_cu = dr_cu_count();
     const int total_chunks = gd_cdiv(g.K, 16);
     const int cps = (gd_cdiv(total_chunks, splits) + 1) & ~1;
+    const int real_splits = gd_cdiv(total_chunks, cps);
     d.tiles_m = gd_cdiv(g.M, 80);
     d.tiles_n = gd_cdiv(g.N, 128);
     d.ksp = cps;
-    g.splits = gd_cdiv(total_chunks, cps);
+    GdTailJob none = {};
+    size_t lds = 0;
+    if (job) {
+        const char* env = getenv("GDMCF_KN_TAIL");
+        const bool tail_on = env ? atoi(env) != 0 : GD_KN_TAIL_DEFAULT != 0;
+        lds = lt_lds_bytes(job->T, job->H, job->B);
+        if (!tail_on || !job->on || !kn_idle_workgroup(d.tiles_m * d.tiles_n * real_splits, n_cu) || lds > GD_LT_LDS_MAX)
+            return GD_DR_NOT_TAKEN;
+        static bool attr_set = false;
+        if (!gd_allow_big_lds(dr_kn_kernel<2>, lds, &attr_set, "gemm_dr_kn")) return GDMCF_E_HIP;
+    }
+    g.splits = real_splits;
     g.kchunk = cps * 16;
     g.tiles_m = d.tiles_m;
     g.tiles_n = d.tiles_n;
     d.g = g;
     {
         GdProfScope prof(g.prof_tag, 2.0 * g.M * g.N * g.K, s);
-        hipLaunchKernelGGL((dr_kn_kernel<2>), dim3(n_cu), dim3(256), 0, s, d);
+        hipLaunchKernelGGL((dr_kn_kernel<2>), dim3(n_cu), dim3(256), lds, s, d, job ? *job : none);
     }
     t_gd_last_gemm = 5;
     return gd_launch_status("gemm_dr_kn");
 }
+
+int gd_dr_kn_launch(GdGemm& g, hipStream_t s) { return kn_launch(g, nullptr, s); }
+int gd_dr_kn_launch_tail(GdGemm& g, const GdTailJob& job, hipStream_t s) { return kn_launch(g, &job, s); }
+
+int gdmcf_debug_kn_tail_rides(int M, int N, int K) {
+    const int splits = gd_dr_kn_splits(M, N, K);
+    if (splits <= 0) return 0;
+    const int total_chunks = gd_cdiv(K, 16);
+    const int cps = (gd_cdiv(total_chunks, splits) + 1) & ~1;
+    return kn_idle_workgroup(gd_cdiv(M, 80) * gd_cdiv(N, 128) * gd_cdiv(total_chunks, cps), dr_cu_count()) ? 1 : 0;
+}
diff --git a/gdmcf_amd/csrc/linear.hip b/gdmcf_amd/csrc/linear.hip
--- a/gdmcf_amd/csrc/linear.hip
+++ b/gdmcf_amd/csrc/linear.hip
@@ -1,6 +1,7 @@
 #include <stdlib.h>
 
 #include "common.h"
+#include "tail_job.h"
 
 int gd_splitk_reduce(const float* slabs, int64_t slab_stride, int splits, int64_t ld_slab, int M, int N, int mode,
                      const float* bias, const float* rowscale, const float* aact, int64_t ldact, int act, float* out,
@@ -13,6 +14,7 @@
 static const int TARGET_WGS = getenv("GDMCF_TARGET_WGS") ? atoi(getenv("GDMCF_TARGET_WGS")) : 760;
 
 thread_local int t_gemm_prec = GDMCF_GEMM_F32;
+thread_local int t_loss_parts = 0;
 
 int pick_class(int M, int N, bool fused, int prec) {
     if (prec == GDMCF_GEMM_BF16 && M > 128) {
@@ -226,6 +228,8 @@
     attach_shadows(g, GD_LAY_KC, GD_LAY_KC);
     int rc = gd_gemm_launch(GD_LAY_KC, GD_LAY_KC, GD_EPI_LOSS, cls, g, s);
     if (rc) return rc;
+    t_loss_parts = g.tiles_n;
+    if (rowsum == nullptr) return GDMCF_OK;
     return gd_rowpart_reduce(rowpart, g.ld_rowpart, M, g.tiles_n, rowsum, s);
 }
 
@@ -249,6 +253,8 @@
     attach_shadows(g, GD_LAY_KC, GD_LAY_KC);
     int rc = gd_gemm_launch(GD_LAY_KC, GD_LAY_KC, GD_EPI_LOSS, cls, g, s);
     if (rc) return rc;
+    t_loss_parts = g.tiles_n;
+    if (rowsum == nullptr) return GDMCF_OK;
     return gd_rowpart_reduce(rowpart, g.ld_rowpart, M, g.tiles_n, rowsum, s);
 }
 
@@ -300,6 +306,64 @@
     const int real_splits = gd_cdiv(N, g.kchunk);
     return gd_splitk_reduce((const float*)ws, g.slab_stride, real_splits, lds_, M, K, 1, nullptr, rowscale, Aact,
                             ldact, act, dA, ldda, s);
+}
+
+int gdmcf_loss_parts_last(void) { return t_loss_parts; }
+
+int gdmcf_kn_tail_run(const GdKnTail* tail, int M, void* stream) {
+    GD_CHECK_ARG(tail != nullptr, "kn_tail_run: tail missing");
+    const GdKnTail& t = *tail;
+    GD_CHECK_SHAPE(M > 0 && t.nt > 0 && t.ld_rowpart >= t.nt, "kn_tail_run: bad shape");
+    GD_CHECK_ARG(t.rowpart && t.rowsum, "kn_tail_run: null pointer");
+    int rc = gd_rowpart_reduce(t.rowpart, t.ld_rowpart, M, t.nt, t.rowsum, (hipStream_t)stream);
+    if (rc) return rc;
+    rc = gdmcf_row_loss_finish_mean_f64(t.rowsum, t.rowdiv, t.alpha, t.ts, t.weight_t, t.pt, M, t.T, t.H, t.Lt_history, t.Lt_count,
+                                        t.update_history, t.loss_unscaled, t.loss, t.gradcoef, t.loss_mean, t.rowscale_mean, stream);
+    if (rc) return rc;
+    return gdmcf_rowscale_f32(t.A, t.lda, t.rowscale, M, t.Ka, t.out, t.ldo, stream);
+}
+
+int gdmcf_linear_bwd_input_tail_f32(const float* dZ, int64_t lddz, const float* W, int64_t ldw, const float* rowscale,
+                                    const float* Aact, int64_t ldact, int act, int M, int N, int K, float* dA, int64_t ldda,
+                                    void* ws, size_t ws_bytes, const GdKnTail* tail, void* stream) {
+    GD_CHECK_SHAPE(M > 0 && N > 0 && K > 0 && lddz >= N && ldw >= K && ldda >= K, "linear_bwd_input_tail: bad shape");
+    GD_CHECK_ARG(act == 0 || (act == 1 && Aact && ldact >= K), "linear_bwd_input_tail: activation output missing");
+    GD_CHECK_ARG(tail != nullptr, "linear_bwd_input_tail: tail missing");
+    const GdKnTail& t = *tail;
+    GD_CHECK_SHAPE(t.nt > 0 && t.ld_rowpart >= t.nt && t.T > 0 && t.H > 0 && t.Ka > 0 && t.lda >= t.Ka && t.ldo >= t.Ka,
+                   "linear_bwd_input_tail: bad tail shape");
+    GD_CHECK_ARG(t.rowpart && t.rowsum && t.rowdiv && t.ts && t.weight_t && t.pt && t.loss_unscaled && t.loss && t.A && t.rowscale && t.out,
+                 "linear_bwd_input_tail: null pointer");
+    GD_CHECK_ARG(!t.update_history || (t.Lt_history && t.Lt_count), "linear_bwd_input_tail: update_history without the history");
+    GD_CHECK_ARG(!t.rowscale_mean || t.gradcoef, "linear_bwd_input_tail: rowscale_mean needs gradcoef");
+    GD_CHECK_ARG(lt_lds_bytes(t.T, t.H, M) <= GD_LT_LDS_MAX, "linear_bwd_input_tail: T*H and B too large for the LDS-resident FIFO update (150 KiB)");
+    hipStream_t s = (hipStream_t)stream;
+    const int64_t lds_ = round4(K);
+    if (t_gemm_prec == GDMCF_GEMM_F32 && ws != nullptr) {
+        GdGemm g = {};
+        g.A = dZ; g.lda = lddz; g.B = W; g.ldb = ldw; g.M = M; g.N = K; g.K = N;
+        g.C = (float*)ws; g.ldc = lds_; g.slab_stride = (int64_t)M * lds_; g.prof_tag = 4;
+        g.ws_cap = ws_bytes;
+        GdShadow sh;
+        const bool has16 = gd_shadow_lookup(t.out, &sh) && sh.rows == M && sh.cols == t.Ka;
+        GdTailJob j = {};
+        j.on = 1; j.B = M;
+        j.rowpart = t.rowpart; j.ld_rowpart = t.ld_rowpart; j.nt = t.nt; j.rowsum = t.rowsum;
+        j.rowdiv = t.rowdiv; j.alpha = t.alpha; j.gradcoef = t.gradcoef; j.ts = t.ts; j.weight_t = t.weight_t; j.pt = t.pt;
+        j.T = t.T; j.H = t.H; j.update = t.update_history; j.hist = t.Lt_history; j.cnt = t.Lt_count; j.lu = t.loss_unscaled;
+        j.loss = t.loss; j.loss_mean = t.loss_mean; j.rowscale_mean = t.rowscale_mean; j.inv_b = 1.0f / (float)M;
+        j.K = t.Ka; j.A = t.A; j.lda = t.lda; j.rs = t.rowscale; j.out = t.out; j.ldo = t.ldo;
+        j.out16 = has16 ? (unsigned short*)sh.p16 : nullptr; j.ldo16 = has16 ? sh.ld16 : 0; j.bias_col = t.ldo > t.Ka;
+        const int rc = gd_dr_kn_launch_tail(g, j, s);
+        if (rc != GD_DR_NOT_TAKEN) {
+            if (rc) return rc;
+            return gd_splitk_reduce((const float*)ws, g.slab_stride, gd_cdiv(N, g.kchunk), lds_, M, K, 1, nullptr, rowscale, Aact, ldact,
+                                    act, dA, ldda, s);
+        }
+    }
+    const int rc = gdmcf_kn_tail_run(tail, M, stream);
+    if (rc) return rc;
+    return gdmcf_linear_bwd_input_f32(dZ, lddz, W, ldw, rowscale, Aact, ldact, act, M, N, K, dA, ldda, ws, ws_bytes, stream);
 }
 
 int gdmcf_linear_bwd_weight_f32(const float* dZ, int64_t lddz, const float* A, int64_t lda, const float* rowscale,
diff --git a/gdmcf_amd/csrc/loss_tail.hip b/gdmcf_amd/csrc/loss_tail.hip
--- a/gdmcf_amd/csrc/loss_tail.hip
+++ b/gdmcf_amd/csrc/loss_tail.hip
@@ -1,38 +1,7 @@
 #include "draws.h"
+#include "tail_job.h"
 
 namespace {
-
-__device__ void lt_history_parallel(const int64_t* __restrict__ ts, const double* __restrict__ lu, int B, int T, int H,
-                                    double* hist, int64_t* cnt, unsigned char* lds_raw) {
-    double* old = reinterpret_cast<double*>(lds_raw);
-    int* n_t = reinterpret_cast<int*>(old + (size_t)T * H);
-    int* c0 = n_t + T;
-    int* tsl = c0 + T;
-    const int tid = threadIdx.x, nth = blockDim.x;
-    for (int i = tid; i < T * H; i += nth) old[i] = hist[i];
-    for (int t = tid; t < T; t += nth) {
-        n_t[t] = 0;
-        c0[t] = (int)cnt[t];
-    }
-    for (int b = tid; b < B; b += nth) tsl[b] = (int)ts[b];
-    __syncthreads();
-    for (int b = tid; b < B; b += nth) atomicAdd(&n_t[tsl[b]], 1);
-    __syncthreads();
-    for (int i = tid; i < T * H; i += nth) {
-        const int t = i / H, j = i % H;
-        const int drop = max(0, c0[t] + n_t[t] - H);
-        if (j < c0[t] && j - drop >= 0) hist[(int64_t)t * H + (j - drop)] = old[i];
-    }
-    for (int b = tid; b < B; b += nth) {
-        const int t = tsl[b];
-        int rank = 0;
-        for (int p = 0; p < b; ++p) rank += (tsl[p] == t);
-        const int drop = max(0, c0[t] + n_t[t] - H);
-        const int pos = c0[t] + rank - drop;
-        if (pos >= 0) hist[(int64_t)t * H + pos] = lu[b];
-    }
-    for (int t = tid; t < T; t += nth) cnt[t] = (int64_t)min(H, c0[t] + n_t[t]);
-}
 
 __global__ __launch_bounds__(256) void row_loss_finish_kernel(const float* __restrict__ rowsum,
                                                               const float* __restrict__ rowdiv,
@@ -46,29 +15,8 @@
                                                               double* __restrict__ loss_mean, float* __restrict__ rowscale_mean,
                                                               float inv_b) {
     extern __shared__ __attribute__((aligned(16))) unsigned char fin_lds[];
-    double part = 0.0;
-    for (int b = threadIdx.x; b < B; b += 256) {
-        const float mse = rowsum[b] / rowdiv[b];
-        const double l = weight_t[ts[b]] * (double)mse;
-        lu[b] = l;
-        const double lb = l / pt[b];
-        loss[b] = lb;
-        part += lb;
-        if (gradcoef) {
-            const float gc = (float)(2.0 * (alpha ? (double)alpha[b] : 1.0) * weight_t[ts[b]] / (pt[b] * (double)rowdiv[b]));
-            gradcoef[b] = gc;
-            if (rowscale_mean) rowscale_mean[b] = gc * inv_b;
-        }
-    }
-    if (loss_mean) {
-        double* s_part = reinterpret_cast<double*>(fin_lds);
-        for (int o = 32; o > 0; o >>= 1) part += __shfl_xor(part, o);
-        if ((threadIdx.x & 63) == 0) s_part[threadIdx.x >> 6] = part;
-        __syncthreads();
-        if (threadIdx.x == 0) *loss_mean = (((s_part[0] + s_part[1]) + s_part[2]) + s_part[3]) / (double)B;
-    }
-    __syncthreads();
-    if (update) lt_history_parallel(ts, lu, B, T, H, hist, cnt, fin_lds);
+    gd_row_loss_finish_block(rowsum, rowdiv, alpha, gradcoef, ts, weight_t, pt, B, T, H, hist, cnt, update, lu, loss, loss_mean,
+                             rowscale_mean, inv_b, fin_lds);
 }
 
 __global__ __launch_bounds__(256) void lt_history_update_kernel(const int64_t* ts, const double* lu, int B, int T,
@@ -149,16 +97,6 @@
     }
 }
 
-size_t lt_lds_bytes(int T, int H, int B) { return (size_t)T * H * 8 + (size_t)T * 8 + (size_t)B * 4 + 16; }
-
-template <class K>
-bool gd_allow_big_lds(K* kernel, size_t lds, bool* done, const char* who) {
-    if (*done || lds <= 48 * 1024) return true;
-    *done = hipFuncSetAttribute(reinterpret_cast<const void*>(kernel), hipFuncAttributeMaxDynamicSharedMemorySize, 160 * 1024) == hipSuccess;
-    if (!*done) gdmcf_set_error("%s: hipFuncSetAttribute failed", who);
-    return *done;
-}
-
 }
 
 extern "C" {
@@ -180,7 +118,7 @@
     GD_CHECK_ARG(!update_history || (Lt_history && Lt_count), "row_loss_finish: update_history without the history");
     GD_CHECK_ARG(!rowscale_mean || gradcoef, "row_loss_finish: rowscale_mean needs gradcoef");
     const size_t lds = lt_lds_bytes(T, H, B);
-    GD_CHECK_ARG(lds <= 150 * 1024, "row_loss_finish: T*H and B too large for the LDS-resident FIFO update (150 KiB)");
+    GD_CHECK_ARG(lds <= GD_LT_LDS_MAX, "row_loss_finish: T*H and B too large for the LDS-resident FIFO update (150 KiB)");
     static bool attr_set = false;
     if (!gd_allow_big_lds(row_loss_finish_kernel, lds, &attr_set, "row_loss_finish")) return GDMCF_E_HIP;
     hipLaunchKernelGGL(row_loss_finish_kernel, dim3(1), dim3(256), lds, (hipStream_t)stream, rowsum, rowdiv, alpha,
@@ -194,7 +132,7 @@
     GD_CHECK_SHAPE(B > 0 && T > 0 && H > 0, "lt_history_update: bad shape");
     GD_CHECK_ARG(ts && loss_unscaled && Lt_history && Lt_count, "lt_history_update: null pointer");
     const size_t lds = lt_lds_bytes(T, H, B);
-    GD_CHECK_ARG(lds <= 150 * 1024, "lt_history_update: T*H and B too large for the LDS-resident FIFO update (150 KiB)");
+    GD_CHECK_ARG(lds <= GD_LT_LDS_MAX, "lt_history_update: T*H and B too large for the LDS-resident FIFO update (150 KiB)");
     static bool attr_set = false;
     if (!gd_allow_big_lds(lt_history_update_kernel, lds, &attr_set, "lt_history_update")) return GDMCF_E_HIP;
     hipLaunchKernelGGL(lt_history_update_kernel, dim3(1), dim3(256), lds, (hipStream_t)stream, ts, loss_unscaled, B, T,
diff --git a/gdmcf_amd/csrc/reduce.hip b/gdmcf_amd/csrc/reduce.hip
--- a/gdmcf_amd/csrc/reduce.hip
+++ b/gdmcf_amd/csrc/reduce.hip
@@ -1,4 +1,4 @@
-#include "common.h"
+#include "tail_job.h"
 
 namespace {
 
@@ -55,24 +55,7 @@
                                                        const float* __restrict__ rs, int M, int K,
                                                        float* __restrict__ out, int64_t ldo,
                                                        unsigned short* __restrict__ out16, int64_t ldo16, int bias_col) {
-    const int m = blockIdx.y, k = (blockIdx.x * 256 + threadIdx.x) * 4;
-    if (bias_col && blockIdx.x == 0 && threadIdx.x == 0) out[(int64_t)m * ldo + K] = rs[m];
-    if (k >= K) return;
-    const float r = rs[m];
-    const float* a = A + (int64_t)m * lda + k;
-    float* o = out + (int64_t)m * ldo + k;
-    float v[4];
-    if (k + 3 < K) {
-        const f32x4 t = *reinterpret_cast<const f32x4_u4*>(a);
-        v[0] = t.x * r; v[1] = t.y * r; v[2] = t.z * r; v[3] = t.w * r;
-        *reinterpret_cast<f32x4_u4*>(o) = f32x4{v[0], v[1], v[2], v[3]};
-    } else {
-        for (int j = 0; j < 4; ++j)
-            if (k + j < K) o[j] = v[j] = a[j] * r;
-    }
-    if (out16)
-        for (int j = 0; j < 4; ++j)
-            if (k + j < K) out16[(int64_t)m * ldo16 + k + j] = gd_bf16_bits(v[j]);
+    gd_rowscale_rows<1>(A, lda, rs, M, K, out, ldo, out16, ldo16, bias_col, blockIdx.x, gridDim.x, blockIdx.y, gridDim.y);
 }
 
 __global__ __launch_bounds__(256) void colsum_kernel(const float* __restrict__ dZ, int64_t ld,
@@ -99,12 +82,7 @@
 
 __global__ __launch_bounds__(256) void rowpart_reduce_kernel(const float* __restrict__ rowpart, int ld, int M, int nt,
                                                              float* __restrict__ rowsum) {
-    const int m = blockIdx.x * 4 + (threadIdx.x >> 6), lane = threadIdx.x & 63;
-    if (m >= M) return;
-    float s = 0.f;
-    for (int j = lane; j < nt; j += 64) s += rowpart[(int64_t)m * ld + j];
-    for (int o = 32; o > 0; o >>= 1) s += __shfl_xor(s, o);
-    if (lane == 0) rowsum[m] = s;
+    gd_rowpart_reduce_rows<1>(rowpart, ld, M, nt, rowsum, blockIdx.x, gridDim.x);
 }
 
 typedef __bf16 gd_bf16x2 __attribute__((ext_vector_type(2)));
diff --git a/gdmcf_amd/csrc/tail_job.h b/gdmcf_amd/csrc/tail_job.h
--- /dev/null
+++ b/gdmcf_amd/csrc/tail_job.h
@@ -0,0 +1,190 @@
+#pragma once
+
+#include "common.h"
+
+namespace {
+
+template <int U>
+__device__ __forceinline__ void gd_rowpart_reduce_rows(const float* __restrict__ rowpart, int ld, int M, int nt,
+                                                       float* __restrict__ rowsum, int blk, int nblk) {
+    const int lane = threadIdx.x & 63, step = nblk * 4;
+    for (int m0 = blk * 4 + (int)(threadIdx.x >> 6); m0 < M; m0 += step * U) {
+        float s[U];
+#pragma unroll
+        for (int u = 0; u < U; ++u) s[u] = 0.f;
+        for (int j = lane; j < nt; j += 64) {
+#pragma unroll
+            for (int u = 0; u < U; ++u) s[u] += rowpart[(int64_t)min(m0 + u * step, M - 1) * ld + j];
+        }
+#pragma unroll
+        for (int u = 0; u < U; ++u) {
+            for (int o = 32; o > 0; o >>= 1) s[u] += __shfl_xor(s[u], o);
+            if (lane == 0 && m0 + u * step < M) rowsum[m0 + u * step] = s[u];
+        }
+    }
+}
+
+template <int U>
+__device__ __forceinline__ void gd_rowscale_rows(const float* __restrict__ A, int64_t lda, const float* __restrict__ rs, int M, int K,
+                                                 float* __restrict__ out, int64_t ldo, unsigned short* __restrict__ out16,
+                                                 int64_t ldo16, int bias_col, int bx, int nbx, int by, int nby) {
+    for (int kb = bx; kb * 1024 < K; kb += nbx) {
+        const int k = (kb * 256 + (int)threadIdx.x) * 4;
+        for (int m0 = by; m0 < M; m0 += nby * U) {
+            float r[U];
+            f32x4 t[U];
+#pragma unroll
+            for (int u = 0; u < U; ++u) {
+                const int m = min(m0 + u * nby, M - 1);
+                r[u] = rs[m];
+                const float* a = A + (int64_t)m * lda + k;
+                if (k + 3 < K) {
+                    t[u] = *reinterpret_cast<const f32x4_u4*>(a);
+                } else {
+                    for (int j = 0; j < 4; ++j) t[u][j] = k + j < K ? a[j] : 0.f;
+                }
+            }
+#pragma unroll
+            for (int u = 0; u < U; ++u) {
+                const int m = m0 + u * nby;
+                if (m >= M) break;
+                if (bias_col && kb == 0 && threadIdx.x == 0) out[(int64_t)m * ldo + K] = r[u];
+                if (k >= K) continue;
+                float* o = out + (int64_t)m * ldo + k;
+                const float v[4] = {t[u].x * r[u], t[u].y * r[u], t[u].z * r[u], t[u].w * r[u]};
+                if (k + 3 < K) {
+                    *reinterpret_cast<f32x4_u4*>(o) = f32x4{v[0], v[1], v[2], v[3]};
+                } else {
+                    for (int j = 0; j < 4; ++j)
+                        if (k + j < K) o[j] = v[j];
+                }
+                if (out16)
+                    for (int j = 0; j < 4; ++j)
+                        if (k + j < K) out16[(int64_t)m * ldo16 + k + j] = gd_bf16_bits(v[j]);
+            }
+        }
+    }
+}
+
+__device__ __forceinline__ void lt_history_parallel(const int64_t* __restrict__ ts, const double* __restrict__ lu, int B, int T, int H,
+                                                    double* hist, int64_t* cnt, unsigned char* lds_raw) {
+    double* old = reinterpret_cast<double*>(lds_raw);
+    int* n_t = reinterpret_cast<int*>(old + (size_t)T * H);
+    int* c0 = n_t + T;
+    int* tsl = c0 + T;
+    const int tid = threadIdx.x, nth = blockDim.x;
+    for (int i = tid; i < T * H; i += nth) old[i] = hist[i];
+    for (int t = tid; t < T; t += nth) {
+        n_t[t] = 0;
+        c0[t] = (int)cnt[t];
+    }
+    for (int b = tid; b < B; b += nth) tsl[b] = (int)ts[b];
+    __syncthreads();
+    for (int b = tid; b < B; b += nth) atomicAdd(&n_t[tsl[b]], 1);
+    __syncthreads();
+    for (int i = tid; i < T * H; i += nth) {
+        const int t = i / H, j = i % H;
+        const int drop = max(0, c0[t] + n_t[t] - H);
+        if (j < c0[t] && j - drop >= 0) hist[(int64_t)t * H + (j - drop)] = old[i];
+    }
+    for (int b = tid; b < B; b += nth) {
+        const int t = tsl[b];
+        int rank = 0;
+        for (int p = 0; p < b; ++p) rank += (tsl[p] == t);
+        const int drop = max(0, c0[t] + n_t[t] - H);
+        const int pos = c0[t] + rank - drop;
+        if (pos >= 0) hist[(int64_t)t * H + pos] = lu[b];
+    }
+    for (int t = tid; t < T; t += nth) cnt[t] = (int64_t)min(H, c0[t] + n_t[t]);
+}
+
+__device__ __forceinline__ void gd_row_loss_finish_block(const float* __restrict__ rowsum, const float* __restrict__ rowdiv,
+                                                         const float* __restrict__ alpha, float* __restrict__ gradcoef,
+                                                         const int64_t* __restrict__ ts, const double* __restrict__ weight_t,
+                                                         const double* __restrict__ pt, int B, int T, int H, double* hist,
+                                                         int64_t* cnt, int update, double* __restrict__ lu, double* __restrict__ loss,
+                                                         double* __restrict__ loss_mean, float* __restrict__ rowscale_mean,
+                                                         float inv_b, unsigned char* fin_lds) {
+    double part = 0.0;
+    for (int b = threadIdx.x; b < B; b += 256) {
+        const float mse = rowsum[b] / rowdiv[b];
+        const double l = weight_t[ts[b]] * (double)mse;
+        lu[b] = l;
+        const double lb = l / pt[b];
+        loss[b] = lb;
+        part += lb;
+        if (gradcoef) {
+            const float gc = (float)(2.0 * (alpha ? (double)alpha[b] : 1.0) * weight_t[ts[b]] / (pt[b] * (double)rowdiv[b]));
+            gradcoef[b] = gc;
+            if (rowscale_mean) rowscale_mean[b] = gc * inv_b;
+        }
+    }
+    if (loss_mean) {
+        double* s_part = reinterpret_cast<double*>(fin_lds);
+        for (int o = 32; o > 0; o >>= 1) part += __shfl_xor(part, o);
+        if ((threadIdx.x & 63) == 0) s_part[threadIdx.x >> 6] = part;
+        __syncthreads();
+        if (threadIdx.x == 0) *loss_mean = (((s_part[0] + s_part[1]) + s_part[2]) + s_part[3]) / (double)B;
+    }
+    __syncthreads();
+    if (update) lt_history_parallel(ts, lu, B, T, H, hist, cnt, fin_lds);
+}
+
+}
+
+struct GdTailJob {
+    int on;
+    int B;
+    const float* rowpart;
+    int ld_rowpart, nt;
+    float* rowsum;
+    const float* rowdiv;
+    const float* alpha;
+    float* gradcoef;
+    const int64_t* ts;
+    const double* weight_t;
+    const double* pt;
+    int T, H, update;
+    double* hist;
+    int64_t* cnt;
+    double* lu;
+    double* loss;
+    double* loss_mean;
+    float* rowscale_mean;
+    float inv_b;
+    int K;
+    const float* A;
+    int64_t lda;
+    const float* rs;
+    float* out;
+    int64_t ldo;
+    unsigned short* out16;
+    int64_t ldo16;
+    int bias_col;
+};
+
+namespace {
+
+__device__ __forceinline__ void gd_tail_job_run(const GdTailJob& j, unsigned char* lds) {
+    gd_rowpart_reduce_rows<8>(j.rowpart, j.ld_rowpart, j.B, j.nt, j.rowsum, 0, 1);
+    __syncthreads();
+    gd_row_loss_finish_block(j.rowsum, j.rowdiv, j.alpha, j.gradcoef, j.ts, j.weight_t, j.pt, j.B, j.T, j.H, j.hist, j.cnt, j.update,
+                             j.lu, j.loss, j.loss_mean, j.rowscale_mean, j.inv_b, lds);
+    __syncthreads();
+    gd_rowscale_rows<8>(j.A, j.lda, j.rs, j.B, j.K, j.out, j.ldo, j.out16, j.ldo16, j.bias_col, 0, 1, 0, 1);
+}
+
+inline size_t lt_lds_bytes(int T, int H, int B) { return (size_t)T * H * 8 + (size_t)T * 8 + (size_t)B * 4 + 16; }
+constexpr size_t GD_LT_LDS_MAX = 150 * 1024;
+
+template <class K>
+bool gd_allow_big_lds(K* kernel, size_t lds, bool* done, const char* who) {
+    if (*done || lds <= 48 * 1024) return true;
+    *done = hipFuncSetAttribute(reinterpret_cast<const void*>(kernel), hipFuncAttributeMaxDynamicSharedMemorySize, 160 * 1024) == hipSuccess;
+    if (!*done) gdmcf_set_error("%s: hipFuncSetAttribute failed", who);
+    return *done;
+}
+
+}
+
+int gd_dr_kn_launch_tail(GdGemm& g, const GdTailJob& job, hipStream_t s);
diff --git a/gdmcf_amd/engine.py b/gdmcf_amd/engine.py
--- a/gdmcf_amd/engine.py
+++ b/gdmcf_amd/engine.py
@@ -21,6 +21,8 @@
         self._side2 = None
         self._side2_used = False
         self._wt_on = os.environ.get("GDMCF_FWD_WT", "1") == "1"
+        self.defer_tail = False
+        self._pending_tail = None
 
     def _grad_like(self, p):
         if not self.static_grads:
@@ -40,8 +42,22 @@
                 rec[1] = w._version
 
     def flush_weight_waiters(self):
+        self._flush_tail()
         while self.weight_waiters:
             self.weight_waiters.popitem()[1]()
+
+    def _defers_tail(self, spec, layers, B):
+        if not self.defer_tail or type(self) is not DenoiserEngine or self.gemm_dtype != "f32" or spec["eps_mode"]:
+            return False
+        if (self.grad_sink is not None and not self.input_grad_first) or len(layers) < 2:
+            return False
+        n, k = layers[-1][0].shape
+        return bool(self.lib.gdmcf_debug_kn_tail_rides(B, k, n))
+
+    def _flush_tail(self):
+        pend, self._pending_tail = self._pending_tail, None
+        if pend is not None:
+            core.tail_job_run(self.lib, pend[0], pend[1], _lib.stream_ptr())
 
     def _shadows_on(self, bufs, layers):
         if self.gemm_dtype != "bf16":
@@ -149,6 +165,7 @@
 
     @with_precision
     def train_forward(self, spec):
+        self._flush_tail()
         x0, ts = spec["x_start"], spec["ts"]
         csr = spec.get("csr")
         B, dev = (csr.shape[0], csr.device) if csr is not None else (x0.shape[0], x0.device)
@@ -178,12 +195,19 @@
         w, bias, _ = layers[-1]
         N, K = w.shape
         self._use_weight(w)
+        defer = self._defers_tail(spec, layers, B)
         if csr is not None:
-            core.loss_layer_bits(lib, bufs, A, w, bias, bufs.x0bits, None, B, N, K, st)
-        else:
-            core.loss_layer(lib, bufs, A, w, bias, target, alpha, B, N, K, st)
-        loss, self.last_loss_mean = core.loss_tail(lib, bufs, spec, B, rowdiv, alpha, st, mean=True)
-        self._saved = dict(kind="train", B=B, bufs=bufs, layers=layers, keepalive=(keepalive, target, alpha, rowdiv, spec["pt"]))
+            nt = core.loss_layer_bits(lib, bufs, A, w, bias, bufs.x0bits, None, B, N, K, st, reduce=not defer)
+        else:
+            nt = core.loss_layer(lib, bufs, A, w, bias, target, alpha, B, N, K, st, reduce=not defer)
+        tail = None
+        if defer:
+            loss, self.last_loss_mean, tail = core.loss_tail_job(lib, bufs, spec, B, rowdiv, alpha, nt, A, K)
+            self._pending_tail = (tail, B)
+        else:
+            loss, self.last_loss_mean = core.loss_tail(lib, bufs, spec, B, rowdiv, alpha, st, mean=True)
+        self._saved = dict(kind="train", B=B, bufs=bufs, layers=layers, tail=tail,
+                           keepalive=(keepalive, target, alpha, rowdiv, spec["pt"]))
         return loss
 
     @with_precision
@@ -192,6 +216,12 @@
         if sv is None or sv.get("kind") != "train":
             raise RuntimeError("gdmcf_amd: train_backward without a preceding training_losses")
         bufs = sv["bufs"]
+        tail = sv.get("tail")
+        if tail is not None and self._pending_tail is not None and self._pending_tail[0] is tail:
+            if isinstance(gloss, float) and gloss == 1.0 / sv["B"]:
+                self._pending_tail = None
+                return self._backward(sv, bufs.diff, bufs.rowscale_mean, tail=tail)
+            self._flush_tail()
         if isinstance(gloss, float) and gloss == 1.0 / sv["B"] and getattr(bufs, "rowscale_mean", None) is not None:
             rowscale = bufs.rowscale_mean
         else:
@@ -225,7 +255,7 @@
             g = g.contiguous()
         return self._backward(sv, g, None)
 
-    def _backward(self, sv, dz_last, rowscale):
+    def _backward(self, sv, dz_last, rowscale, tail=None):
         lib, st = self.lib, _lib.stream_ptr()
         bufs, layers, B = sv["bufs"], sv["layers"], sv["B"]
         m = self.model
@@ -242,7 +272,10 @@
             N, K = w.shape
             if li > 0:
                 dprev = bufs.dzs[li - 1]
-                self._input_grad(bufs, B, w, N, K, dz, rs, A_prev, layers[li - 1][2], dprev, st)
+                if tail is not None and li == L - 1:
+                    core.linear_bwd_input_tail(lib, bufs, dz, w, rs, A_prev, layers[li - 1][2], B, N, K, dprev, tail, st)
+                else:
+                    self._input_grad(bufs, B, w, N, K, dz, rs, A_prev, layers[li - 1][2], dprev, st)
                 return dprev
             dWe = self._grad_like(m.emb_layer.weight)
             dbe = self._grad_like(m.emb_layer.bias)
@@ -252,7 +285,10 @@
         def weight_grad(li, w, bias, A_prev):
             db = self._grad_like(bias)
             scol = int(rs is None and li == 0 and getattr(bufs, "xin_ones", False) and A_prev.stride(0) > w.shape[1])
-            A_use, scol = self._row_scaled(bufs, B, w.shape[1], A_prev, rs, scol, st)
+            if tail is not None and li == L - 1:
+                A_use, scol = bufs.hs, int(bufs.hs.stride(0) > w.shape[1])
+            else:
+                A_use, scol = self._row_scaled(bufs, B, w.shape[1], A_prev, rs, scol, st)
             fs = fused.fused_state(w) if fused is not None else None
             dW = self._grad_like(w) if fs is None else None
             if fs is None and self._gemm_side and self.grad_sink is None and li == L - 1 and L > 1:
@@ -273,7 +309,7 @@
         for li in range(L - 1, -1, -1):
             w, bias, _ = layers[li]
             A_prev = bufs.acts[li - 1] if li > 0 else bufs.xin
-            if fused is not None or self.input_grad_first:
+            if fused is not None or self.input_grad_first or (tail is not None and li == L - 1):
                 nxt = input_grad(li, w, A_prev)
                 weight_grad(li, w, bias, A_prev)
             else:
diff --git a/gdmcf_amd/engine_core.py b/gdmcf_amd/engine_core.py
--- a/gdmcf_amd/engine_core.py
+++ b/gdmcf_amd/engine_core.py
@@ -1,4 +1,5 @@
 import collections
+import ctypes
 import functools
 
 import torch
@@ -249,18 +250,20 @@
                                      dWe.data_ptr(), dbe.data_ptr(), st))
 
 
-def loss_layer(lib, bufs, A, W, bias, target, alpha, B, N, K, st):
+def loss_layer(lib, bufs, A, W, bias, target, alpha, B, N, K, st, reduce=True):
     (a, lda), (w, ldw) = _pl(A), _pl(W)
     _lib.check(lib.gdmcf_linear_loss_fwd_f32(a, lda, w, ldw, _lib.ptr(bias), target.data_ptr(), target.stride(0),
                                              _lib.ptr(alpha), B, N, K, None, 0, bufs.diff.data_ptr(), bufs.ldi,
-                                             bufs.rowpart.data_ptr(), bufs.rowsum.data_ptr(), st))
-
-
-def loss_layer_bits(lib, bufs, A, W, bias, x0bits, alpha, B, N, K, st):
+                                             bufs.rowpart.data_ptr(), bufs.rowsum.data_ptr() if reduce else None, st))
+    return int(lib.gdmcf_loss_parts_last())
+
+
+def loss_layer_bits(lib, bufs, A, W, bias, x0bits, alpha, B, N, K, st, reduce=True):
     (a, lda), (w, ldw) = _pl(A), _pl(W)
     _lib.check(lib.gdmcf_linear_loss_fwd_bits_f32(a, lda, w, ldw, _lib.ptr(bias), x0bits.data_ptr(), x0bits.stride(0),
                                                   _lib.ptr(alpha), B, N, K, None, 0, bufs.diff.data_ptr(), bufs.ldi,
-                                                  bufs.rowpart.data_ptr(), bufs.rowsum.data_ptr(), st))
+                                                  bufs.rowpart.data_ptr(), bufs.rowsum.data_ptr() if reduce else None, st))
+    return int(lib.gdmcf_loss_parts_last())
 
 
 def loss_tail(lib, bufs, spec, B, rowdiv, alpha, st, mean=False):
@@ -277,6 +280,33 @@
         bufs.rowscale_mean = torch.zeros(B, dtype=torch.float32, device=ts.device)
     _lib.check(lib.gdmcf_row_loss_finish_mean_f64(*args, loss_mean.data_ptr(), bufs.rowscale_mean.data_ptr(), st))
     return loss, loss_mean
+
+
+def loss_tail_job(lib, bufs, spec, B, rowdiv, alpha, nt, A, K):
+    ts = spec["ts"]
+    loss = torch.empty(B, dtype=torch.float64, device=ts.device)
+    loss_mean = torch.empty((), dtype=torch.float64, device=ts.device)
+    if getattr(bufs, "rowscale_mean", None) is None:
+        bufs.rowscale_mean = torch.zeros(B, dtype=torch.float32, device=ts.device)
+    (a, lda) = _pl(A)
+    job = _lib.GdKnTail(bufs.rowpart.data_ptr(), bufs.rowpart.stride(0), nt, bufs.rowsum.data_ptr(), rowdiv.data_ptr(),
+                        _lib.ptr(alpha), ts.data_ptr(), spec["weight_t"].data_ptr(), spec["pt"].data_ptr(), spec["T"], spec["H"],
+                        spec["Lt_history"].data_ptr(), spec["Lt_count"].data_ptr(), int(spec["update_history"]),
+                        bufs.lu.data_ptr(), loss.data_ptr(), bufs.gradcoef.data_ptr(), loss_mean.data_ptr(),
+                        bufs.rowscale_mean.data_ptr(), a, lda, bufs.rowscale_mean.data_ptr(), K, bufs.hs.data_ptr(),
+                        bufs.hs.stride(0))
+    job.refs = (loss, loss_mean, rowdiv, alpha, ts, spec["weight_t"], spec["pt"], spec["Lt_history"], spec["Lt_count"], A)
+    return loss, loss_mean, job
+
+
+def tail_job_run(lib, job, B, st):
+    _lib.check(lib.gdmcf_kn_tail_run(ctypes.byref(job), B, st))
+
+
+def linear_bwd_input_tail(lib, bufs, dz, W, rs, A_prev, act_prev, B, N, K, d_prev, job, st):
+    (z, ldz), (w, ldw), (a, lda), (d, ldd) = _pl(dz), _pl(W), _pl(A_prev), _pl(d_prev)
+    _lib.check(lib.gdmcf_linear_bwd_input_tail_f32(z, ldz, w, ldw, _lib.ptr(rs), a, lda, act_prev, B, N, K, d, ldd,
+                                                   bufs.ws.data_ptr(), bufs.ws_bytes, ctypes.byref(job), st))
 
 
 def posterior_fwd(lib, A, W, bias, x_t, c1, c2, r1, r2, sigma, z, B, N, K, x_next, pred, st):
diff --git a/gdmcf_amd/graph.py b/gdmcf_amd/graph.py
--- a/gdmcf_amd/graph.py
+++ b/gdmcf_amd/graph.py
@@ -129,6 +129,8 @@
     def close(self):
         if self._state is None:
             return
+        if hasattr(self.eng, "_flush_tail"):
+            self.eng._flush_tail()
         prep, ts, step = self._read_state()
         self.eng.offset = prep
         if self.reweight:
diff --git a/gdmcf_amd/parallel.py b/gdmcf_amd/parallel.py
--- a/gdmcf_amd/parallel.py
+++ b/gdmcf_amd/parallel.py
@@ -248,8 +248,15 @@
         self.optimizer.zero_grad()
         eng = getattr(self.model, "engine", None)
         if self.direct_backward and eng is not None:
-            with torch.no_grad():
-                losses = self.diffusion.training_losses(self.model, batch, reweight, **rand)
+            defers = hasattr(eng, "defer_tail")
+            if defers:
+                eng.defer_tail = True
+            try:
+                with torch.no_grad():
+                    losses = self.diffusion.training_losses(self.model, batch, reweight, **rand)
+            finally:
+                if defers:
+                    eng.defer_tail = False
             loss = getattr(eng, "last_loss_mean", None)
             if loss is None:
                 loss = losses["loss"].mean()
diff --git a/include/gdmcf_hip.h b/include/gdmcf_hip.h
--- a/include/gdmcf_hip.h
+++ b/include/gdmcf_hip.h
@@ -119,6 +119,37 @@
                                const float* rowscale, const float* Aact, int64_t ldact, int act,
                                int M, int N, int K, float* dA, int64_t ldda, void* ws,
                                size_t ws_bytes, void* stream);
+typedef struct GdKnTail {
+    const float* rowpart;
+    int ld_rowpart, nt;
+    float* rowsum;
+    const float* rowdiv;
+    const float* alpha;
+    const int64_t* ts;
+    const double* weight_t;
+    const double* pt;
+    int T, H;
+    double* Lt_history;
+    int64_t* Lt_count;
+    int update_history;
+    double* loss_unscaled;
+    double* loss;
+    float* gradcoef;
+    double* loss_mean;
+    float* rowscale_mean;
+    const float* A;
+    int64_t lda;
+    const float* rowscale;
+    int Ka;
+    float* out;
+    int64_t ldo;
+} GdKnTail;
+int gdmcf_linear_bwd_input_tail_f32(const float* dZ, int64_t lddz, const float* W, int64_t ldw, const float* rowscale,
+                                    const float* Aact, int64_t ldact, int act, int M, int N, int K, float* dA, int64_t ldda,
+                                    void* ws, size_t ws_bytes, const GdKnTail* tail, void* stream);
+int gdmcf_kn_tail_run(const GdKnTail* tail, int M, void* stream);
+int gdmcf_loss_parts_last(void);
+int gdmcf_debug_kn_tail_rides(int M, int N, int K);
 int gdmcf_linear_bwd_weight_f32(const float* dZ, int64_t lddz, const float* A, int64_t lda,
                                 const float* rowscale, int a_scale_col, int M, int N, int K,
                                 float* dW, int64_t lddw, float* db, int accumulate, void* stream);
```

Measured after the change: 327,600 users/s, median of 6. 1.01x the previous value.
